# ligengen/EgoGen

Hardware: AMD Instinct MI355X
Metric: PPO env-steps/sec (512 parallel SMPL-X agents) (higher is better)
Workload: dtype f32 (blend GEMM: shape/template columns as 2-term bf16 splits, pose correctives as one fp16 product, fp32 accumulate); PPO update products on 2-term bf16 splits; rollout policy layers on 2-term bf16 splits

## Files before the change

egogen_amd/_lib.py:

```python
from __future__ import annotations

import ctypes as C
import os

_HERE = os.path.dirname(os.path.abspath(__file__))
LIB_PATH = os.path.join(_HERE, "libegogen_hip.so")

c_float_p = C.POINTER(C.c_float)
c_int_p = C.POINTER(C.c_int32)


class EgxError(RuntimeError):
    pass


class BodyModelHost(C.Structure):
    _fields_ = [
        ("num_verts", C.c_int),
        ("v_template_host", C.c_void_p), ("shapedirs_host", C.c_void_p), ("posedirs_host", C.c_void_p),
        ("J_regressor_host", C.c_void_p), ("parents_host", C.c_void_p), ("lbs_weights_host", C.c_void_p),
        ("hand_comps_l_host", C.c_void_p), ("hand_comps_r_host", C.c_void_p),
        ("hand_mean_l_host", C.c_void_p), ("hand_mean_r_host", C.c_void_p),
        ("extra_vids_host", C.c_void_p), ("lmk_vids_host", C.c_void_p), ("lmk_bary_host", C.c_void_p),
        ("num_markers", C.c_int), ("marker_vids_host", C.c_void_p),
        ("num_feet", C.c_int), ("feet_vids_host", C.c_void_p),
    ]


class SdfGrid(C.Structure):
    _fields_ = [("grid", C.c_void_p), ("d0", C.c_int), ("d1", C.c_int), ("d2", C.c_int),
                ("center", C.c_float * 3), ("scale", C.c_float), ("coarse_minmax", C.c_void_p)]


class LinearDesc(C.Structure):
    _fields_ = [("num_rows", C.c_int), ("out_features", C.c_int), ("num_segments", C.c_int),
                ("seg_ptr", C.c_void_p * 4), ("seg_width", C.c_int * 4), ("seg_ld", C.c_int * 4),
                ("weight", C.c_void_p), ("weight_ld", C.c_int), ("bias", C.c_void_p),
                ("residual", C.c_void_p), ("residual_ld", C.c_int),
                ("out", C.c_void_p), ("out_ld", C.c_int), ("activation", C.c_int), ("leaky_slope", C.c_float)]


class PriorPacked3(C.Structure):
    _fields_ = [("x_enc_w_ih", C.c_void_p), ("x_enc_w_hh", C.c_void_p), ("drnn_w", C.c_void_p * 3), ("d_rnn_w_hz", C.c_void_p),
                ("d_rnn_w_y", C.c_void_p), ("d_rnn_w_hh", C.c_void_p), ("d_comb_w", C.c_void_p), ("d_mlp_w", C.c_void_p * 2),
                ("d_out_w", C.c_void_p), ("reg_in_m", C.c_void_p), ("reg_in_xb", C.c_void_p), ("reg_in_betas", C.c_void_p),
                ("reg_blk", C.c_void_p), ("reg_out", C.c_void_p), ("reg_blk_b", C.c_void_p)]


class PriorWeights(C.Structure):
    _fields_ = [(n, C.c_void_p) for n in ("x_enc_w_ih", "x_enc_w_hh", "x_enc_b_ih", "x_enc_b_hh")] + \
               [("drnn_w", C.c_void_p * 3), ("drnn_b", C.c_void_p * 3)] + \
               [(n, C.c_void_p) for n in ("d_rnn_w_ih", "d_rnn_w_hh", "d_rnn_b_ih", "d_rnn_b_hh")] + \
               [("d_mlp_w", C.c_void_p * 2), ("d_mlp_b", C.c_void_p * 2), ("d_out_w", C.c_void_p), ("d_out_b", C.c_void_p),
                ("reg_in_w", C.c_void_p), ("reg_in_b", C.c_void_p), ("reg_blk_w", C.c_void_p * 20), ("reg_blk_b", C.c_void_p * 20),
                ("reg_out_w", C.c_void_p), ("reg_out_b", C.c_void_p), ("d_comb_w", C.c_void_p), ("d_comb_b", C.c_void_p),
                ("packed3", C.POINTER(PriorPacked3))]


class PolicyPacked3(C.Structure):
    _fields_ = [(n, C.c_void_p) for n in ("x_enc_w_ih", "x_enc_w_hh", "ego_enc_w_ih", "ego_enc_w_hh")] + \
               [("actor_w", C.c_void_p * 4), ("actor_out_w", C.c_void_p), ("critic_w", C.c_void_p * 4), ("critic_out_w", C.c_void_p)]


class PolicyWeights(C.Structure):
    _fields_ = [(n, C.c_void_p) for n in ("x_enc_w_ih", "x_enc_w_hh", "x_enc_b_ih", "x_enc_b_hh",
                                          "ego_enc_w_ih", "ego_enc_w_hh", "ego_enc_b_ih", "ego_enc_b_hh")] + \
               [("actor_w", C.c_void_p * 4), ("actor_b", C.c_void_p * 4), ("actor_out_w", C.c_void_p), ("actor_out_b", C.c_void_p),
                ("critic_w", C.c_void_p * 4), ("critic_b", C.c_void_p * 4), ("critic_out_w", C.c_void_p), ("critic_out_b", C.c_void_p),
                ("packed3", C.POINTER(PolicyPacked3))]


class PolicyGrads(C.Structure):
    _fields_ = [(n, C.c_void_p) for n in ("x_enc_w_ih", "x_enc_w_hh", "x_enc_b_ih", "x_enc_b_hh",
                                          "ego_enc_w_ih", "ego_enc_w_hh", "ego_enc_b_ih", "ego_enc_b_hh")] + \
               [("actor_w", C.c_void_p * 4), ("actor_b", C.c_void_p * 4), ("actor_out_w", C.c_void_p), ("actor_out_b", C.c_void_p),
                ("critic_w", C.c_void_p * 4), ("critic_b", C.c_void_p * 4), ("critic_out_w", C.c_void_p), ("critic_out_b", C.c_void_p)]


class VposerWeights(C.Structure):
    _fields_ = [(n, C.c_void_p) for n in ("fc1_w", "fc1_b", "fc2_w", "fc2_b", "mu_w", "mu_b", "fc1_w3", "fc2_w3", "mu_w3")]


class EnvConfig(C.Structure):
    _fields_ = [(n, C.c_float) for n in ("reproj_factor", "goal_thresh", "pene_thres", "weight_skate", "weight_floor",
                                         "weight_face_target", "weight_look_target", "weight_success", "weight_target_dist",
                                         "weight_pene", "weight_vp")] + \
               [(n, C.c_int) for n in ("max_depth", "scene_kind", "terminate_on_penetration", "pene_type_body")] + \
               [("ray_len", C.c_float), ("vp_thresh", C.c_float), ("no_goal_termination", C.c_int)]


class EnvScenes(C.Structure):
    _fields_ = [("edges", C.c_void_p), ("edge_off", C.c_void_p), ("tris", C.c_void_p), ("tri_off", C.c_void_p),
                ("floor_height", C.c_void_p), ("map_lin", C.c_void_p), ("map_res", C.c_int),
                ("crowd_bbox", C.c_void_p), ("crowd_group", C.c_int), ("crowd_scenes", C.c_int), ("crowd_member", C.c_int),
                ("crowd_floor_half", C.c_float), ("crowd_polygon", C.c_int), ("crowd_static", C.c_int)]


class EnvState(C.Structure):
    _fields_ = [(n, C.c_void_p) for n in ("state", "seed", "R0", "T0", "dist", "steps", "wpath", "scene_idx")]


class EnvStepIO(C.Structure):
    _fields_ = [(n, C.c_void_p) for n in ("Y_gen", "pred_params", "joints", "markers_proj", "pene_count", "vp_emb",
                                          "feet_marker_idx", "reward", "terminated", "reward_terms", "obs_ego", "obs_dist",
                                          "obs_time", "out_marker_b", "out_prev_frame", "nonfinite_count", "invalid_flags")]


class EnvResetIO(C.Structure):
    _fields_ = [("num_candidates", C.c_int)] + \
               [(n, C.c_void_p) for n in ("mask", "cand_pairs", "cand_yaw", "cand_variant", "cand_scene", "cand_valid", "tab_joints",
                                          "tab_markers", "tab_glorot", "tab_transl", "tab_pose", "obs_ego", "obs_dist",
                                          "obs_time", "out_choice", "out_pending", "forced_count")]


SIGNATURES = {
    "egx_last_error": (C.c_char_p, []),
    "egx_version": (C.c_int, []),
    "egx_body_model_create": (C.c_int, [C.POINTER(BodyModelHost), C.POINTER(C.c_void_p)]),
    "egx_body_model_destroy": (None, [C.c_void_p]),
    "egx_body_model_num_verts": (C.c_int, [C.c_void_p]),
    "egx_body_model_nnz": (C.c_int, [C.c_void_p]),
    "egx_body_model_lbs_vertices": (C.c_int, [C.c_void_p, C.c_int]),
    "egx_lbs_workspace_bytes": (C.c_size_t, [C.c_void_p, C.c_int]),
    "egx_body_model_culls": (C.c_int, [C.c_void_p, C.POINTER(C.c_float)]),
    "egx_lbs_set_culling": (C.c_int, [C.c_int]),
    "egx_lbs_get_culling": (C.c_int, []),
    "egx_lbs_cull_stats": (C.c_int, [C.c_void_p, C.c_void_p, C.c_int, C.POINTER(C.c_int32), C.POINTER(C.c_int32)]),
    "egx_lbs_forward": (C.c_int, [C.c_void_p, C.c_void_p, C.c_void_p, C.c_int, C.c_int, C.c_void_p, C.c_void_p,
                                  C.c_void_p, C.POINTER(SdfGrid), C.c_void_p, C.c_void_p, C.c_void_p,
                                  C.c_void_p, C.c_size_t, C.c_void_p]),
    "egx_sdf_scene_set_create": (C.c_int, [C.POINTER(SdfGrid), C.c_int, C.POINTER(C.c_void_p)]),
    "egx_sdf_scene_set_destroy": (None, [C.c_void_p]),
    "egx_sdf_scene_set_size": (C.c_int, [C.c_void_p]),
    "egx_lbs_forward_scenes": (C.c_int, [C.c_void_p, C.c_void_p, C.c_void_p, C.c_int, C.c_int, C.c_void_p, C.c_void_p,
                                         C.c_void_p, C.c_void_p, C.c_void_p, C.c_void_p, C.c_void_p, C.c_void_p,
                                         C.c_void_p, C.c_size_t, C.c_void_p]),
    "egx_point_set_create": (C.c_int, [C.POINTER(BodyModelHost), C.c_void_p, C.c_int, C.POINTER(C.c_void_p)]),
    "egx_point_set_destroy": (None, [C.c_void_p]),
    "egx_point_set_size": (C.c_int, [C.c_void_p]),
    "egx_points_forward": (C.c_int, [C.c_void_p, C.c_void_p, C.c_void_p, C.c_int, C.c_int, C.c_void_p, C.c_void_p, C.c_void_p]),
    "egx_points_backward": (C.c_int, [C.c_void_p, C.c_void_p, C.c_void_p, C.c_int, C.c_int, C.c_void_p, C.c_void_p, C.c_void_p,
                                      C.c_void_p, C.c_void_p]),
    "egx_lbs_joints": (C.c_int, [C.c_void_p, C.c_void_p, C.c_void_p, C.c_int, C.c_int, C.c_void_p, C.c_void_p, C.c_size_t, C.c_void_p]),
    "egx_canonical_frame": (C.c_int, [C.c_void_p, C.c_int, C.c_int, C.c_void_p, C.c_void_p, C.c_void_p]),
    "egx_update_transl_glorot": (C.c_int, [C.c_void_p, C.c_void_p, C.c_int, C.c_void_p, C.c_void_p, C.c_int, C.c_void_p, C.c_void_p]),
    "egx_sdf_sample": (C.c_int, [C.POINTER(SdfGrid), C.c_void_p, C.c_int64, C.c_void_p, C.c_void_p]),
    "egx_mesh_sdf": (C.c_int, [C.c_void_p, C.c_int, C.POINTER(C.c_float), C.c_float, C.c_int, C.c_int, C.c_int, C.c_int, C.c_void_p, C.c_void_p]),
    "egx_sdf_boxes": (C.c_int, [C.c_void_p, C.POINTER(C.c_float), C.POINTER(C.c_float), C.c_int, C.POINTER(C.c_float), C.c_float,
                                C.c_int, C.c_int, C.c_int, C.c_void_p, C.c_void_p]),
    "egx_scan_sdf": (C.c_int, [C.c_void_p, C.c_int, C.c_void_p, C.c_void_p, C.c_int, C.c_int, C.POINTER(C.c_float), C.c_float,
                               C.c_int, C.c_int, C.c_int, C.c_void_p, C.c_void_p]),
    "egx_walkable_raster": (C.c_int, [C.c_void_p, C.c_int, C.c_float, C.c_float, C.c_float, C.c_int, C.c_int] + [C.c_float] * 5 +
                            [C.c_void_p, C.c_void_p, C.c_void_p]),
    "egx_sdf_coarse_bytes": (C.c_size_t, [C.c_int, C.c_int, C.c_int]),
    "egx_sdf_build_coarse": (C.c_int, [C.POINTER(SdfGrid), C.c_void_p, C.c_void_p]),
    "egx_linear": (C.c_int, [C.POINTER(LinearDesc), C.c_void_p]),
    "egx_gru_pointwise": (C.c_int, [C.c_void_p, C.c_void_p, C.c_void_p, C.c_int, C.c_void_p, C.c_int, C.c_int, C.c_int, C.c_void_p]),
    "egx_cont6d_to_aa": (C.c_int, [C.c_void_p, C.c_int, C.c_void_p, C.c_int, C.c_void_p]),
    "egx_posenc": (C.c_int, [C.c_void_p, C.c_void_p, C.c_int, C.c_void_p, C.c_void_p]),
    "egx_sample_prior_workspace_bytes": (C.c_size_t, [C.c_int]),
    "egx_sample_prior": (C.c_int, [C.POINTER(PriorWeights), C.c_void_p, C.c_void_p, C.c_int, C.c_void_p, C.c_void_p, C.c_int,
                                   C.c_void_p, C.c_void_p, C.c_void_p, C.c_size_t, C.c_void_p]),
    "egx_policy_workspace_bytes": (C.c_size_t, [C.c_int]),
    "egx_policy_forward": (C.c_int, [C.POINTER(PolicyWeights), C.c_void_p, C.c_void_p, C.c_void_p, C.c_void_p, C.c_int,
                                     C.c_void_p, C.c_void_p, C.c_void_p, C.c_void_p, C.c_size_t, C.c_void_p]),
    "egx_assemble_params": (C.c_int, [C.c_void_p, C.c_void_p, C.c_int, C.c_void_p, C.c_void_p]),
    "egx_env_step_post": (C.c_int, [C.POINTER(EnvConfig), C.POINTER(EnvScenes), C.POINTER(EnvState), C.POINTER(EnvStepIO),
                                    C.c_int, C.c_void_p]),
    "egx_env_reset": (C.c_int, [C.POINTER(EnvConfig), C.POINTER(EnvScenes), C.POINTER(EnvState), C.POINTER(EnvResetIO),
                                C.c_int, C.c_void_p]),
    "egx_env_get_feature": (C.c_int, [C.c_void_p] * 5 + [C.c_int] * 4 + [C.c_void_p] * 3),
    "egx_env_get_map": (C.c_int, [C.c_void_p, C.c_int, C.c_float, C.c_void_p, C.c_int, C.c_void_p, C.c_void_p, C.c_int, C.c_void_p,
                                  C.c_void_p, C.c_void_p]),
    "egx_sample_action": (C.c_int, [C.c_void_p, C.c_void_p, C.c_void_p, C.c_float, C.c_float, C.c_int, C.c_int, C.c_void_p,
                                    C.c_void_p, C.c_void_p]),
    "egx_gae": (C.c_int, [C.c_void_p, C.c_void_p, C.c_void_p, C.c_int, C.c_int, C.c_double, C.c_double, C.c_void_p,
                          C.c_void_p, C.c_void_p]),
    "egx_ppo_loss": (C.c_int, [C.c_void_p] * 9 + [C.c_float] * 6 + [C.c_int] + [C.c_void_p] * 5),
    "egx_gru_pointwise_bwd": (C.c_int, [C.c_void_p, C.c_void_p, C.c_void_p, C.c_void_p, C.c_int, C.c_int, C.c_void_p, C.c_void_p,
                                        C.c_void_p, C.c_void_p]),
    "egx_ppo_loss_packed": (C.c_int, [C.c_void_p] * 8 + [C.c_float] * 6 + [C.c_int] + [C.c_void_p] * 4),
    "egx_lbs_set_blend_mode": (C.c_int, [C.c_int]),
    "egx_lbs_get_blend_mode": (C.c_int, []),
    "egx_lbs_set_wave_tile": (C.c_int, [C.c_int]),
    "egx_lbs_get_wave_tile": (C.c_int, []),
    "egx_lbs_set_fix_queue_capacity": (C.c_int, [C.c_int]),
    "egx_lbs_fix_stats": (C.c_int, [C.c_void_p, C.c_void_p, C.c_int, C.POINTER(C.c_int32)]),
    "egx_gather_rows": (C.c_int, [C.c_void_p, C.c_int, C.c_int, C.c_void_p, C.c_void_p, C.c_void_p, C.c_void_p]),
    "egx_adv_stats": (C.c_int, [C.c_void_p, C.c_int, C.c_void_p, C.c_void_p]),
    "egx_track_episode": (C.c_int, [C.c_void_p, C.c_void_p, C.c_int, C.c_void_p, C.c_void_p, C.c_void_p, C.c_void_p]),
    "egx_rollout_store": (C.c_int, [C.c_void_p] * 6 + [C.c_int] + [C.c_void_p] * 10),
    "egx_adamw_workspace_floats": (C.c_size_t, []),
    "egx_adamw_clip_step": (C.c_int, [C.c_void_p, C.c_void_p, C.c_void_p, C.c_void_p, C.c_size_t, C.c_size_t, C.c_float] + [C.c_double] * 5 +
                            [C.c_void_p, C.c_void_p, C.c_void_p]),
    "egx_policy_set_precision": (C.c_int, [C.c_int]),
    "egx_policy_get_precision": (C.c_int, []),
    "egx_act_fwd": (C.c_int, [C.c_void_p, C.c_void_p, C.c_void_p, C.c_int, C.c_int, C.c_int, C.c_float, C.c_void_p]),
    "egx_act_bwd_colsum": (C.c_int, [C.c_void_p, C.c_void_p, C.c_void_p, C.c_void_p, C.c_int, C.c_int, C.c_int, C.c_float,
                                     C.c_void_p]),
    "egx_profile_next_lbs": (C.c_int, [C.c_void_p, C.c_void_p]),
    "egx_event_create": (C.c_int, [C.POINTER(C.c_void_p)]),
    "egx_event_destroy": (C.c_int, [C.c_void_p]),
    "egx_event_elapsed_ms": (C.c_int, [C.c_void_p, C.c_void_p, C.POINTER(C.c_float)]),
    "egx_policy_train_create": (C.c_int, [C.POINTER(PolicyWeights), C.POINTER(PolicyGrads), C.c_int, C.POINTER(C.c_void_p)]),
    "egx_policy_train_destroy": (None, [C.c_void_p]),
    "egx_policy_train_refresh": (C.c_int, [C.c_void_p, C.c_void_p]),
    "egx_policy_train_packed": (C.c_int, [C.c_void_p, C.POINTER(PolicyPacked3)]),
    "egx_policy_train_bind": (C.c_int, [C.c_void_p, C.c_void_p, C.c_void_p]),
    "egx_policy_train_step": (C.c_int, [C.c_void_p] * 9 + [C.c_float] * 6 + [C.c_void_p, C.c_void_p]),
    "egx_policy_train_step_heads": (C.c_int, [C.c_void_p] * 9 + [C.c_float] * 6 + [C.c_void_p, C.c_void_p]),
    "egx_policy_train_step_encoders": (C.c_int, [C.c_void_p, C.c_void_p]),
    "egx_policy_train_set_precision": (C.c_int, [C.c_void_p, C.c_int]),
    "egx_pack3_bytes": (C.c_size_t, [C.c_int, C.c_int]),
    "egx_pack3": (C.c_int, [C.c_void_p, C.c_int, C.c_int, C.c_int, C.c_int, C.c_void_p, C.c_int, C.c_int, C.c_void_p]),
    "egx_gemm3_workspace_bytes": (C.c_size_t, [C.c_int, C.c_int, C.c_int]),
    "egx_gemm3": (C.c_int, [C.c_void_p, C.c_int, C.c_int, C.c_void_p, C.c_int, C.c_int, C.c_int, C.c_int, C.c_int, C.c_void_p, C.c_int,
                            C.c_float, C.c_void_p, C.c_int, C.c_void_p, C.c_int, C.c_void_p, C.c_int, C.c_void_p, C.c_size_t, C.c_void_p]),
    "egx_vposer_workspace_bytes": (C.c_size_t, [C.c_int]),
    "egx_vposer_encode": (C.c_int, [C.POINTER(VposerWeights), C.c_void_p, C.c_int, C.c_int, C.c_void_p, C.c_void_p,
                                    C.c_size_t, C.c_void_p]),
}

_lib = None


def load():
    global _lib
    if _lib is not None:
        return _lib
    if not os.path.exists(LIB_PATH):
        raise EgxError(f"{LIB_PATH} not found - build it with `python -c 'import __graft_entry__ as g; g.build()'` "
                       f"or `make -C egogen_amd/csrc`; there is no CPU fallback")
    lib = C.CDLL(LIB_PATH)
    for name, (res, args) in SIGNATURES.items():
        fn = getattr(lib, name)
        fn.restype = res
        fn.argtypes = args
    _lib = lib
    return lib


def check(rc: int, what: str):
    if rc != 0:
        msg = load().egx_last_error()
        raise EgxError(f"{what} failed (code {rc}): {msg.decode() if msg else ''}")


def ptr(t):
    if t is None:
        return None
    assert t.is_contiguous(), "tensor must be contiguous"
    return C.c_void_p(t.data_ptr())


def current_stream_ptr():
    import torch
    return C.c_void_p(torch.cuda.current_stream().cuda_stream)
```

egogen_amd/csrc/dense3.hip:

```cpp
#include <cstddef>
#include <cstdlib>
#include <mutex>
#include "egx_nets.h"

namespace {

typedef __bf16 bf16v8 __attribute__((ext_vector_type(8)));
typedef float f32x4a1 __attribute__((ext_vector_type(4), aligned(4)));

__host__ __device__ constexpr int d3_planes(int prec) { return prec == 0 ? 3 : (prec == 2 ? 2 : 1); }

template <int NP = 3>
__device__ __forceinline__ void d3_split(const float (&x)[8], bf16x8 (&pl)[NP]) {
  float r[8];
#pragma unroll
  for (int p = 0; p < NP; ++p) {
    bf16v8 h;
#pragma unroll
    for (int e = 0; e < 8; ++e) {
      const float v = (p == 0) ? x[e] : r[e];
      h[e] = (__bf16)v;
      r[e] = v - (float)h[e];
    }
    pl[p] = __builtin_bit_cast(bf16x8, h);
// ... 314 lines not shown
struct D3Gru2 {
  D3Gru g0, g1;
  int blocks0;
  int rowmap;
};
static_assert(offsetof(D3Gru2, g0) == 0 && offsetof(D3Gru2, g1) == sizeof(D3Gru), "layout");
template <int TRIP, int NPL>
__global__ __launch_bounds__(512) void egx_gru3_kernel(D3Gru2 two) {
  const bool second = (int)blockIdx.x >= two.blocks0;
  const D3Gru a = d3_kernarg<D3Gru>(second ? 1 : 0);
  const int gru_bid = second ? (int)blockIdx.x - two.blocks0 : (int)blockIdx.x;
  extern __shared__ __attribute__((aligned(16))) float gsm[];
  float* red = gsm;
  float* tile = gsm + 8 * 24 * 64;
  const int lane = threadIdx.x & 63, wave = threadIdx.x >> 6;
  const int MT = (a.M + 31) >> 5, CT = a.H >> 4;
  int mt, ct;
  if (!d3_tile(gru_bid, MT, CT, mt, ct, d3_rowmap(two.rowmap, a.M, 3 * a.H))) return;
  const int sd = wave >> 2, w4 = wave & 3;
  constexpr bool EARLY = NPL == 3;
  const int e_mi = wave >> 2, e_r = wave & 3;
  const int e_col = lane & 15, e_c = ct * 16 + e_col;
  const int e_row = 16 * e_mi + 4 * (lane >> 4) + e_r, e_m = mt * 32 + e_row;
  float pre_gi[3] = {0.f, 0.f, 0.f}, pre_bi[3] = {0.f, 0.f, 0.f}, pre_bh[3] = {0.f, 0.f, 0.f}, pre_hp = 0.f;
  auto prefetch = [&]() __attribute__((always_inline)) {
    if (e_m >= a.M) return;
#pragma unroll
    for (int g = 0; g < 3; ++g) {
      const int n = g * a.H + e_c;
      if (a.gi_in) pre_gi[g] = d3_g(a.gi_in)[(size_t)e_m * 3 * a.H + n];
      if (a.bias_i) pre_bi[g] = d3_g(a.bias_i)[n];
      pre_bh[g] = d3_g(a.bias_h)[n];
    }
    if (a.h_prev) pre_hp = d3_g(a.h_prev)[(size_t)e_m * a.ldh + e_c];
  };
  if (EARLY) prefetch();
  f32x4 acc[2][3];
#pragma unroll
  for (int mi = 0; mi < 2; ++mi)
#pragma unroll
    for (int g = 0; g < 3; ++g) acc[mi][g] = f32x4{0.f, 0.f, 0.f, 0.f};
  {
    const D3_GLOBAL bf16x8* A = d3_g(sd ? a.Ah : a.Ai);
    const D3_GLOBAL bf16x8* B = d3_g(sd ? a.Bh : a.Bi);
    const int S = A ? (sd ? a.Sh : a.Si) : 0, SA = sd ? a.SAh : a.SAi, sa0 = sd ? a.sah0 : a.sai0;
    const int per = (S + 3) >> 2;
    const int s_lo = w4 * per, s_hi = min(S, s_lo + per);
    const D3_GLOBAL bf16x8* pa[2];
    const D3_GLOBAL bf16x8* pb[3];
#pragma unroll
    for (int mi = 0; mi < 2; ++mi) pa[mi] = A + ((size_t)(2 * mt + mi) * SA + sa0) * 3 * 64 + lane;
#pragma unroll
    for (int g = 0; g < 3; ++g) pb[g] = B + (size_t)(g * CT + ct) * S * 3 * 64 + lane;
    for (int s = s_lo; s < s_hi; s += TRIP) {
      bf16x8 fa[TRIP][2][NPL], fb[TRIP][3][NPL];
#pragma unroll
      for (int u = 0; u < TRIP; ++u) {
        const int su = min(s + u, s_hi - 1);
#pragma unroll
        for (int p = 0; p < NPL; ++p) {
#pragma unroll
          for (int mi = 0; mi < 2; ++mi) fa[u][mi][p] = pa[mi][(size_t)(su * 3 + p) * 64];
#pragma unroll
          for (int g = 0; g < 3; ++g) fb[u][g][p] = pb[g][(size_t)(su * 3 + p) * 64];
        }
      }
      __builtin_amdgcn_sched_barrier(0);
      asm volatile("s_waitcnt vmcnt(0)" ::: "memory");
      __builtin_amdgcn_sched_barrier(0);
#pragma unroll
      for (int u = 0; u < TRIP; ++u) {
        if (s + u >= s_hi) break;
        d3_mma_tiles<2, 3, NPL>(fa[u], fb[u], acc);
      }
      __builtin_amdgcn_sched_barrier(0);
    }
  }
#pragma unroll
  for (int g = 0; g < 3; ++g)
#pragma unroll
    for (int mi = 0; mi < 2; ++mi)
#pragma unroll
      for (int r = 0; r < 4; ++r) red[(wave * 24 + (g * 2 + mi) * 4 + r) * 64 + lane] = acc[mi][g][r];
  if (!EARLY) prefetch();
  __syncthreads();
  {
    const int mi = e_mi, r = e_r, col = e_col, c = e_c, row = e_row, m = e_m;
    float gv[2][3];
#pragma unroll
    for (int s2 = 0; s2 < 2; ++s2)
#pragma unroll
      for (int g = 0; g < 3; ++g) {
        const int q = (g * 2 + mi) * 4 + r;
        gv[s2][g] = ((red[((s2 * 4 + 0) * 24 + q) * 64 + lane] + red[((s2 * 4 + 1) * 24 + q) * 64 + lane]) +
                     red[((s2 * 4 + 2) * 24 + q) * 64 + lane]) + red[((s2 * 4 + 3) * 24 + q) * 64 + lane];
      }
    float hv = 0.f;
    if (m < a.M) {
      float gi[3], gh[3];
#pragma unroll
      for (int g = 0; g < 3; ++g) {
        gi[g] = pre_gi[g] + gv[0][g] + pre_bi[g];
        gh[g] = gv[1][g] + pre_bh[g];
      }
      const float rg = 1.f / (1.f + expf(-(gi[0] + gh[0])));
      const float zg = 1.f / (1.f + expf(-(gi[1] + gh[1])));
      const float ng = tanhf(gi[2] + rg * gh[2]);
      const float hp = pre_hp;
      {
#pragma clang fp contract(off)
        const float keep = (1.f - zg) * ng, carry = zg * hp;
        hv = keep + carry;
      }
#pragma unroll
      for (int g = 0; g < 3; ++g) {
        const int n = g * a.H + c;
        if (a.gi_out) d3_g(a.gi_out)[(size_t)m * 3 * a.H + n] = gi[g];
        if (a.gh_out) d3_g(a.gh_out)[(size_t)m * 3 * a.H + n] = gh[g];
      }
      if (a.h_out) d3_g(a.h_out)[(size_t)m * a.ldo + c] = hv;
    }
    tile[row * 20 + col] = hv;
  }
  if (a.h_out3 || a.h_out3T) __syncthreads();
  if (a.h_out3T && wave == 2) {
    const int c = lane & 15, kg = lane >> 4;
    float x[8];
#pragma unroll
    for (int e = 0; e < 8; ++e) x[e] = tile[(8 * kg + e) * 20 + c];
    bf16x8 pl[NPL];
    d3_split<NPL>(x, pl);
    D3_GLOBAL bf16x8* o = d3_g(a.h_out3T) + ((size_t)((a.col0T >> 4) + ct) * a.S3T + a.s3T0 + mt) * 3 * 64 + lane;
#pragma unroll
    for (int p = 0; p < NPL; ++p) o[p * 64] = pl[p];
  }
  if (a.h_out3) {
    if (wave < 2 && lane < 32) {
      const int row = 16 * wave + (lane & 15), g = lane >> 4;
      const f32x4 x0 = *reinterpret_cast<const f32x4*>(&tile[row * 20 + 8 * g]), x1 = *reinterpret_cast<const f32x4*>(&tile[row * 20 + 8 * g + 4]);
      const float x[8] = {x0[0], x0[1], x0[2], x0[3], x1[0], x1[1], x1[2], x1[3]};
      bf16x8 pl[NPL];
      d3_split<NPL>(x, pl);
      D3_GLOBAL bf16x8* o = d3_g(a.h_out3) + ((size_t)(2 * mt + wave) * a.S3 + a.s30 + (ct >> 1)) * 3 * 64 + 32 * (ct & 1) + lane;
#pragma unroll
      for (int p = 0; p < NPL; ++p) o[p * 64] = pl[p];
    }
  }
}

__global__ __launch_bounds__(256) void egx_posenc3_kernel(const float* __restrict__ dist, const float* __restrict__ time, int n,
                                                          float* __restrict__ out, int ld, bf16x8* __restrict__ out3, int S3, int s0,
                                                          bf16x8* __restrict__ out3T, int S3T, int col0T, float* __restrict__ zero6) {
  if (zero6 && blockIdx.x == 0 && threadIdx.x < 6) zero6[threadIdx.x] = 0.f;
  int frag = blockIdx.x * 4 + (threadIdx.x >> 6);
  const int lane = threadIdx.x & 63;
  const int RT = 2 * ((n + 31) >> 5);
  if (frag >= RT * 4) {
    frag -= RT * 4;
    const int Sn = (n + 31) >> 5;
    if (!out3T || frag >= 8 * Sn) return;
    const int t = frag / Sn, s = frag % Sn;
    const int c = 16 * t + (lane & 15), m0 = 32 * s + 8 * (lane >> 4);
    float x[8];
#pragma unroll
    for (int e = 0; e < 8; ++e) {
      const int m = m0 + e;
      float v = 0.f;
      if (m < n) {
        const float f = ((c < 64) ? dist[m] : time[m]) * exp2f((float)((c & 63) >> 1));
        v = (c & 1) ? cosf(f) : sinf(f);
      }
      x[e] = v;
    }
    bf16x8 pl[3];
    d3_split(x, pl);
    bf16x8* o = out3T + ((size_t)((col0T >> 4) + t) * S3T + s) * 3 * 64 + lane;
#pragma unroll
    for (int p = 0; p < 3; ++p) o[p * 64] = pl[p];
    return;
  }
  const int rt = frag >> 2, s = frag & 3;
  const int row = rt * 16 + (lane & 15), c0 = s * 32 + 8 * (lane >> 4);
  float x[8];
#pragma unroll
  for (int e = 0; e < 8; ++e) {
    const int c = c0 + e;
    float v = 0.f;
    if (row < n) {
      const float f = ((c < 64) ? dist[row] : time[row]) * exp2f((float)((c & 63) >> 1));
      v = (c & 1) ? cosf(f) : sinf(f);
      out[(size_t)row * ld + c] = v;
    }
    x[e] = v;
  }
  bf16x8 pl[3];
  d3_split(x, pl);
  bf16x8* o = out3 + ((size_t)rt * S3 + s0 + s) * 3 * 64 + lane;
#pragma unroll
  for (int p = 0; p < 3; ++p) o[p * 64] = pl[p];
}
void egx_launch_posenc3(hipStream_t st, const float* dist, const float* time, int n, float* out, int ld, void* out3, int S3, int s0,
                        void* out3T, int S3T, int col0T, float* zero6) {
  const int frags = 2 * egx_ceil_div(n, 32) * 4 + (out3T ? 8 * egx_ceil_div(n, 32) : 0);
  hipLaunchKernelGGL(egx_posenc3_kernel, dim3(egx_ceil_div(frags, 4)), dim3(256), 0, st, dist, time, n, out, ld,
                     static_cast<bf16x8*>(out3), S3, s0, static_cast<bf16x8*>(out3T), S3T, col0T, zero6);
}

namespace {
constexpr int R3_XBP = 164, R3_NOUT = 159;
constexpr int r3_act_frags(int nrt) { return nrt * 4 * 3 * 64; }
constexpr size_t r3_lds(int nrt) { return (size_t)16 * nrt * R3_XBP * 4 + 2 * (size_t)r3_act_frags(nrt) * 16; }

__device__ __forceinline__ void r3_load_w(const bf16x8* P, int tile, int S, int lane, bf16x8 (&wf)[4][3]) {
  const bf16x8* p = P + (size_t)tile * S * 3 * 64 + lane;
#pragma unroll
  for (int s = 0; s < 4; ++s)
#pragma unroll
    for (int pl = 0; pl < 3; ++pl) wf[s][pl] = p[(s * 3 + pl) * 64];
}
template <int NRT>
__device__ __forceinline__ void r3_mma3(const bf16x8 (&a)[NRT][3], const bf16x8 (&wf)[3], f32x4 (&acc)[NRT]) {
#pragma unroll
  for (int pr = 0; pr < 6; ++pr) {
    const int pa = (pr == 0) ? 1 : (pr == 1) ? 0 : (pr == 2) ? 2 : (pr == 3) ? 0 : (pr == 4) ? 1 : 0;
    const int pb = (pr == 0) ? 1 : (pr == 1) ? 2 : (pr == 2) ? 0 : (pr == 3) ? 1 : (pr == 4) ? 0 : 0;
#pragma unroll
    for (int rt = 0; rt < NRT; ++rt) acc[rt] = __builtin_amdgcn_mfma_f32_16x16x32_bf16(wf[pb], a[rt][pa], acc[rt], 0, 0, 0);
  }
}
template <int NRT>
__device__ __forceinline__ void r3_mma128(const bf16x8* act, int lane, const bf16x8 (&wf)[4][3], f32x4 (&acc)[NRT]) {
#pragma unroll
  for (int s = 0; s < 4; ++s) {
    bf16x8 a[NRT][3];
#pragma unroll
    for (int rt = 0; rt < NRT; ++rt)
#pragma unroll
      for (int pl = 0; pl < 3; ++pl) a[rt][pl] = act[((rt * 4 + s) * 3 + pl) * 64 + lane];
    r3_mma3<NRT>(a, wf[s], acc);
  }
}
template <int NRT>
__device__ __forceinline__ void r3_store_packed(const float (&v)[NRT][4], bf16x8* dst, int wave, int lane) {
  typedef __bf16 bf16v4 __attribute__((ext_vector_type(4)));
  const int g = lane >> 4;
  char* o = reinterpret_cast<char*>(dst + (size_t)((wave >> 1) * 3) * 64 + 16 * (2 * (wave & 1) + (g >> 1)) + (lane & 15)) + 8 * (g & 1);
#pragma unroll
  for (int rt = 0; rt < NRT; ++rt) {
    float r[4];
#pragma unroll
    for (int p = 0; p < 3; ++p) {
      bf16v4 h;
#pragma unroll
      for (int e = 0; e < 4; ++e) {
        const float x = (p == 0) ? v[rt][e] : r[e];
        h[e] = (__bf16)x;
        r[e] = x - (float)h[e];
      }
      *reinterpret_cast<bf16v4*>(o + (size_t)((rt * 4) * 3 + p) * 64 * sizeof(bf16x8)) = h;
    }
  }
}
}

template <int NRT>
__global__ __launch_bounds__(512) void egx_regressor3_kernel(RegWeights3 w, const float* __restrict__ Y,
                                                                const float* __restrict__ betas, int A, int M,
                                                                float* __restrict__ out_Yb) {
  constexpr int ROWS = 16 * NRT;
  extern __shared__ __attribute__((aligned(16))) char r3_smem[];
  float* xb = reinterpret_cast<float*>(r3_smem);
  bf16x8* hb3 = reinterpret_cast<bf16x8*>(r3_smem + (size_t)ROWS * R3_XBP * 4);
  bf16x8* tb3 = hb3 + r3_act_frags(NRT);
  const int tid = threadIdx.x, lane = tid & 63, wave = tid >> 6;
  const int m0 = blockIdx.x * ROWS;
  const int col4 = 16 * wave + 4 * (lane >> 4);
  for (int i = tid; i < ROWS * R3_XBP; i += 512) xb[i] = 0.f;
  bf16x8* in3 = hb3;
  for (int f = wave; f < NRT * 8; f += 8) {
    const int rt = f >> 3, s = f & 7;
    const int row = min(m0 + 16 * rt + (lane & 15), M - 1), k0 = 8 * (lane >> 4);
    float x[8];
#pragma unroll
    for (int e = 0; e < 8; ++e) {
      const int k = 32 * s + k0 + e;
      x[e] = (s < 7) ? (k < 201 ? Y[(size_t)row * 201 + k] : 0.f) : (k0 + e < 10 ? betas[(size_t)(row % A) * 10 + k0 + e] : 0.f);
    }
    bf16x8 pl[3];
    d3_split(x, pl);
#pragma unroll
    for (int p = 0; p < 3; ++p) in3[((rt * 8 + s) * 3 + p) * 64 + lane] = pl[p];
  }
  __syncthreads();
  f32x4 base[NRT];
  {
    const f32x4 b = *reinterpret_cast<const f32x4a1*>(w.in_b + col4);
#pragma unroll
    for (int rt = 0; rt < NRT; ++rt) base[rt] = b;
    for (int s = 0; s < 8; ++s) {
      bf16x8 wf[3];
      const bf16x8* pw = (s < 7) ? w.in_m + ((size_t)(wave * 7 + s) * 3) * 64 + lane : w.in_b3 + ((size_t)wave * 3) * 64 + lane;
#pragma unroll
      for (int pl = 0; pl < 3; ++pl) wf[pl] = pw[pl * 64];
      bf16x8 a[NRT][3];
#pragma unroll
      for (int rt = 0; rt < NRT; ++rt)
#pragma unroll
        for (int pl = 0; pl < 3; ++pl) a[rt][pl] = in3[((rt * 8 + s) * 3 + pl) * 64 + lane];
      r3_mma3<NRT>(a, wf, base);
    }
  }
  __syncthreads();
  bf16x8 wA[4][3], wB[4][3];
  float hres[NRT][4];
  f32x4 acc[NRT];
  auto layer = [&](int l, const bf16x8 (&cur)[4][3], bf16x8 (&nxt)[4][3]) __attribute__((always_inline)) {
    const bf16x8* src = (l & 1) ? tb3 : hb3;
    const f32x4 b = *reinterpret_cast<const f32x4a1*>(w.blk_b + l * 128 + col4);
    if (l + 1 < 20) r3_load_w(w.blk + (size_t)(l + 1) * 8 * 4 * 3 * 64, wave, 4, lane, nxt);
    else r3_load_w(w.out, wave, 4, lane, nxt);
#pragma unroll
    for (int rt = 0; rt < NRT; ++rt) acc[rt] = f32x4{0.f, 0.f, 0.f, 0.f};
    __builtin_amdgcn_sched_barrier(0);
    r3_mma128<NRT>(src, lane, cur, acc);
    __builtin_amdgcn_sched_barrier(0);
    float v[NRT][4];
#pragma unroll
    for (int rt = 0; rt < NRT; ++rt)
#pragma unroll
      for (int r = 0; r < 4; ++r) {
        float y = fmaxf(acc[rt][r] + b[r], 0.f);
        if (l & 1) { y += hres[rt][r]; hres[rt][r] = y; }
        v[rt][r] = y;
      }
    r3_store_packed<NRT>(v, (l & 1) ? hb3 : tb3, wave, lane);
    __syncthreads();
  };
  r3_load_w(w.blk, wave, 4, lane, wA);
  for (int rc = 0; rc < 3; ++rc) {
#pragma unroll
    for (int rt = 0; rt < NRT; ++rt) acc[rt] = base[rt];
    if (rc > 0) {
      bf16x8* xb3 = hb3;
      for (int f = wave; f < NRT * 5; f += 8) {
        const int rt = f / 5, s = f % 5;
        const float* sp = xb + (16 * rt + (lane & 15)) * R3_XBP + 32 * s + 8 * (lane >> 4);
        const f32x4 x0 = *reinterpret_cast<const f32x4*>(sp), x1 = *reinterpret_cast<const f32x4*>(sp + 4);
        const float x[8] = {x0[0], x0[1], x0[2], x0[3], x1[0], x1[1], x1[2], x1[3]};
        bf16x8 pl[3];
        d3_split(x, pl);
#pragma unroll
        for (int p = 0; p < 3; ++p) xb3[((rt * 5 + s) * 3 + p) * 64 + lane] = pl[p];
// ... 446 lines not shown
```

egogen_amd/csrc/egx_nets.h:

```cpp
#pragma once
#include "egx_common.h"

struct EgxSeg {
  const float* p;
  int w, ld;
};

int egx_launch_linear(hipStream_t st, int M, int N, const EgxSeg* segs, int nseg, const float* W, const float* b,
                      int act, float slope, const float* res, int ldr, float* out, int ldo);
int egx_launch_gru_pointwise(hipStream_t st, const float* gi, const float* gh, const float* hprev, int ldh, float* hout,
                             int ldo, int M, int H);
int egx_launch_cont6d_to_aa(hipStream_t st, const float* xb6, int n, float* out, int ldo);
int egx_launch_posenc(hipStream_t st, const float* dist, const float* time, int A, float* out);

void egx_launch_frame_scan(hipStream_t st, float* y, const float* x_last, int x_ld, int A, int width, int T);

struct D3Pack {
  const float* src;
  int R, K, ld, col0;
  void* dst;
  int S_total, s0;
  int transpose = 0;
};
void egx_launch_pack3(hipStream_t st, const D3Pack* jobs, int njobs);

struct D3Plain {
  const bf16x8* A = nullptr;
  int SA = 0, sa0 = 0;
  const bf16x8* B = nullptr;
  int S = 0;
  const float* bias = nullptr;
  const float* res = nullptr;
  int ldr = 0;
  float* out = nullptr;
  int ldo = 0;
  bf16x8* out3 = nullptr;
  int S3 = 0, s30 = 0;
  int M = 0, N = 0, act = 0;
  float slope = 0.f;
  int batches = 1;
  size_t batch_strideA = 0, batch_stride3 = 0;
  int batch_rows_out = 0;
  int prec = 0;
  float* out_act = nullptr;
  int ldact = 0;
  const float* dact = nullptr;
  int lddact = 0, dact_code = 0;
  float dact_slope = 0.f;
  bf16x8* out3T = nullptr;
  int S3T = 0, s3T0 = 0;
  float* bias_out = nullptr;
  int n_split = 0;
};
void egx_launch_dense3_n(hipStream_t st, const D3Plain* ps, int n);
void egx_launch_dense3(hipStream_t st, const D3Plain& p);
void egx_launch_dense3_pair(hipStream_t st, const D3Plain& p, const D3Plain& q);
void egx_launch_dense3_triple(hipStream_t st, const D3Plain& p, const D3Plain& q, const D3Plain& r);
int egx_ppo_loss_packed_precleared(const float* zp, const float* value, const float* act, const float* adv, const float* ret,
                                   const float* logp_old, const float* adv_stats, const float* scale, float adv_eps, float min_logvar,
                                   float max_logvar, float eps_clip, float vf_coef, float ent_coef, int num_rows, float* g_zp,
                                   float* g_value, float* out_terms, void* stream_);
void egx_launch_posenc3(hipStream_t st, const float* dist, const float* time, int n, float* out, int ld, void* out3, int S3, int s0,
                        void* out3T = nullptr, int S3T = 0, int col0T = 0, float* zero6 = nullptr );

struct D3Gru {
  const bf16x8* Ai = nullptr;
  int SAi = 0, sai0 = 0;
  const bf16x8* Bi = nullptr;
  int Si = 0;
  const float* bias_i = nullptr;
  const float* gi_in = nullptr;
  float* gi_out = nullptr;
  const bf16x8* Ah = nullptr;
  int SAh = 0, sah0 = 0;
  const bf16x8* Bh = nullptr;
  int Sh = 0;
  const float* bias_h = nullptr;
  const float* h_prev = nullptr;
  int ldh = 0;
  float* h_out = nullptr;
  int ldo = 0;
  bf16x8* h_out3 = nullptr;
  int S3 = 0, s30 = 0;
  int M = 0, H = 0;
  int prec = 0;
  float* gh_out = nullptr;
  bf16x8* h_out3T = nullptr;
  int S3T = 0, s3T0 = 0, col0T = 0;
};
int egx_launch_gru3(hipStream_t st, const D3Gru& g);
int egx_launch_gru3_pair(hipStream_t st, const D3Gru& g0, const D3Gru& g1);

struct RegWeights3 {
  const bf16x8 *in_m, *in_xb, *in_b3;
  const float* in_b;
  const bf16x8* blk;
  const float* blk_b;
  const bf16x8* out;
  const float* out_b;
};
int egx_launch_regressor3(hipStream_t st, const RegWeights3& w, const float* Y, const float* betas, int A, int M, float* out_Yb);

struct VpWeights3 {
  const bf16x8 *fc1, *fc2, *mu;
  const float *b1, *b2, *bmu;
};
int egx_launch_vposer3(hipStream_t st, const VpWeights3& w, const float* x, int x_ld, int n, float* out);

__device__ __forceinline__ void egx_cont6d_item(const float* src, float* dst, int j) {
  if (j == 22) {
    dst[0] = src[0]; dst[1] = src[1]; dst[2] = src[2];
    for (int e = 0; e < 24; ++e) dst[69 + e] = src[135 + e];
    return;
  }
  const float* a = src + 3 + 6 * j;
  float b1[3] = {a[0], a[2], a[4]}, a2[3] = {a[1], a[3], a[5]};
  const float n1 = fmaxf(sqrtf(b1[0] * b1[0] + b1[1] * b1[1] + b1[2] * b1[2]), 1e-12f);
  b1[0] /= n1; b1[1] /= n1; b1[2] /= n1;
  const float d = b1[0] * a2[0] + b1[1] * a2[1] + b1[2] * a2[2];
  float b2[3] = {a2[0] - d * b1[0], a2[1] - d * b1[1], a2[2] - d * b1[2]};
  const float n2 = fmaxf(sqrtf(b2[0] * b2[0] + b2[1] * b2[1] + b2[2] * b2[2]), 1e-12f);
  b2[0] /= n2; b2[1] /= n2; b2[2] /= n2;
  const float b3[3] = {b1[1] * b2[2] - b1[2] * b2[1], b1[2] * b2[0] - b1[0] * b2[2], b1[0] * b2[1] - b1[1] * b2[0]};
  const float R[9] = {b1[0], b2[0], b3[0], b1[1], b2[1], b3[1], b1[2], b2[2], b3[2]};
  float aa[3];
  egx_tgm_rotmat_to_aa(R, aa);
  dst[3 + 3 * j + 0] = aa[0]; dst[3 + 3 * j + 1] = aa[1]; dst[3 + 3 * j + 2] = aa[2];
}
```

egogen_amd/csrc/ppo.hip:

```cpp
#include <algorithm>
#include <cstring>
#include "egx_common.h"

namespace {
constexpr float LOG_SQRT_2PI = 0.91893853320467274178f;

}

__device__ __forceinline__ float egx_wave_sum(float v) {
#pragma unroll
  for (int o = 32; o > 0; o >>= 1) v += __shfl_xor(v, o);
  return v;
}

__global__ __launch_bounds__(256) void egx_ppo_loss_kernel(const float* __restrict__ mu, const float* __restrict__ logvar,
                                                          const float* __restrict__ value, const float* __restrict__ act,
                                                          const float* __restrict__ adv, const float* __restrict__ ret,
                                                          const float* __restrict__ logp_old, const float* __restrict__ adv_stats,
                                                          const float* __restrict__ scale_ptr, float adv_eps, float min_lv,
                                                          float max_lv, float eps_clip, float vf_coef, float ent_coef, int n,
                                                          int stride ,
                                                          float* __restrict__ g_mu, float* __restrict__ g_logvar,
                                                          float* __restrict__ g_value, float* __restrict__ out_terms) {
  __shared__ float sh[4][6];
  const int lane = threadIdx.x & 63, wave = threadIdx.x >> 6;
  const float scale = scale_ptr[0];
  float acc[6] = {0.f, 0.f, 0.f, 0.f, 0.f, 0.f};
  for (int row = blockIdx.x * 4 + wave; row < n; row += gridDim.x * 4) {
    float lv[2], inv_var[2], diff[2], lp_d = 0.f, ent_d = 0.f, musq_d = 0.f;
    bool pass[2];
#pragma unroll
    for (int h = 0; h < 2; ++h) {
      const int d = lane + 64 * h;
      const size_t i = (size_t)row * stride + d;
      const float lv_raw = logvar[i], m = mu[i];
      lv[h] = fminf(fmaxf(lv_raw, min_lv), max_lv);
      pass[h] = (lv_raw >= min_lv) && (lv_raw <= max_lv);
      inv_var[h] = expf(-lv[h]);
      diff[h] = act[(size_t)row * 128 + d] - m;
      lp_d += -0.5f * diff[h] * diff[h] * inv_var[h] - 0.5f * lv[h] - LOG_SQRT_2PI;
      ent_d += 0.5f + LOG_SQRT_2PI + 0.5f * lv[h];
      musq_d += m * m;
    }
    const float lp = egx_wave_sum(lp_d), ent = egx_wave_sum(ent_d), musq = egx_wave_sum(musq_d);
    float A = adv[row];
    if (adv_stats) A = (A - adv_stats[0]) / (adv_stats[1] + adv_eps);
    const float ratio = expf(lp - logp_old[row]);
    const float s1 = ratio * A;
    const float rc = fminf(fmaxf(ratio, 1.f - eps_clip), 1.f + eps_clip);
    const float s2 = rc * A;
    const bool in_range = (ratio >= 1.f - eps_clip) && (ratio <= 1.f + eps_clip);
    float dclip_dlp;
    if (s1 < s2) dclip_dlp = -A * ratio;
    else if (s1 > s2) dclip_dlp = in_range ? -A * ratio : 0.f;
    else dclip_dlp = in_range ? -A * ratio : -0.5f * A * ratio;
    const float v = value[row];
    const float dv = ret[row] - v;
#pragma unroll
    for (int h = 0; h < 2; ++h) {
      const size_t i = (size_t)row * stride + lane + 64 * h;
      g_mu[i] = scale * dclip_dlp * (diff[h] * inv_var[h]);
      const float dlp_dlv = 0.5f * (diff[h] * diff[h] * inv_var[h] - 1.f);
      g_logvar[i] = pass[h] ? scale * (dclip_dlp * dlp_dlv - ent_coef * 0.5f) : 0.f;
    }
    if (lane == 0) g_value[row] = scale * vf_coef * (-2.f) * dv;
    const float clip_l = -fminf(s1, s2), vf_l = dv * dv;
    acc[0] += scale * (clip_l + vf_coef * vf_l - ent_coef * ent);
    acc[1] += scale * clip_l;
    acc[2] += scale * vf_l;
    acc[3] += scale * ent;
    acc[4] += scale * 0.5f * musq / 128.f;
    acc[5] += scale * (logp_old[row] - lp);
  }
  if (lane == 0) {
#pragma unroll
    for (int k = 0; k < 6; ++k) sh[wave][k] = acc[k];
  }
  __syncthreads();
  if (threadIdx.x < 6) atomicAdd(out_terms + threadIdx.x, (sh[0][threadIdx.x] + sh[1][threadIdx.x]) + (sh[2][threadIdx.x] + sh[3][threadIdx.x]));
}

__global__ void egx_gru_pointwise_bwd_kernel(const float* __restrict__ gi, const float* __restrict__ gh,
                                             const float* __restrict__ hprev, const float* __restrict__ dh, int M, int H,
                                             float* __restrict__ dgi, float* __restrict__ dgh, float* __restrict__ dhprev) {
  const int idx = blockIdx.x * blockDim.x + threadIdx.x;
  if (idx >= M * H) return;
  const int m = idx / H, c = idx % H;
  const size_t b3 = (size_t)m * 3 * H;
  const float r = 1.f / (1.f + expf(-(gi[b3 + c] + gh[b3 + c])));
  const float z = 1.f / (1.f + expf(-(gi[b3 + H + c] + gh[b3 + H + c])));
  const float ghn = gh[b3 + 2 * H + c];
  const float nn = tanhf(gi[b3 + 2 * H + c] + r * ghn);
  const float hp = hprev ? hprev[idx] : 0.f;
  const float g = dh[idx];
  const float dn = g * (1.f - z), dz = g * (hp - nn);
  const float dan = dn * (1.f - nn * nn);
  const float dar = dan * ghn * r * (1.f - r);
  const float daz = dz * z * (1.f - z);
  dgi[b3 + c] = dar; dgh[b3 + c] = dar;
  dgi[b3 + H + c] = daz; dgh[b3 + H + c] = daz;
  dgi[b3 + 2 * H + c] = dan; dgh[b3 + 2 * H + c] = dan * r;
  if (dhprev) dhprev[idx] = g * z;
}

__global__ void egx_act_fwd_kernel(float* __restrict__ z, const float* __restrict__ res, float* __restrict__ out, size_t n4,
                                   int act, float slope) {
  const size_t i = (size_t)blockIdx.x * blockDim.x + threadIdx.x;
  if (i >= n4) return;
  float4 v = reinterpret_cast<float4*>(z)[i];
  float* e = reinterpret_cast<float*>(&v);
#pragma unroll
  for (int k = 0; k < 4; ++k) {
    const float x = e[k];
    e[k] = (act == 1) ? tanhf(x) : (act == 2) ? fmaxf(x, 0.f) : (act == 3) ? (x > 0.f ? x : x * slope) : x;
  }
  reinterpret_cast<float4*>(z)[i] = v;
  if (res) {
    const float4 r = reinterpret_cast<const float4*>(res)[i];
    reinterpret_cast<float4*>(out)[i] = make_float4(v.x + r.x, v.y + r.y, v.z + r.z, v.w + r.w);
  }
}

__global__ __launch_bounds__(256) void egx_act_bwd_colsum_kernel(const float* __restrict__ dy, const float* __restrict__ a,
                                                                 float* __restrict__ g, float* __restrict__ db, int M, int N,
                                                                 int rows_per_block, int act, float slope) {
  __shared__ float part[4][64];
  const int tx = threadIdx.x & 63, ty = threadIdx.x >> 6;
  const int n = blockIdx.x * 64 + tx;
  const int m0 = blockIdx.y * rows_per_block, m1 = min(M, m0 + rows_per_block);
  float s = 0.f;
  if (n < N) {
    for (int m = m0 + ty; m < m1; m += 4) {
      const size_t idx = (size_t)m * N + n;
      float v = dy[idx];
      if (act != 0) {
        const float y = a[idx];
        v *= (act == 1) ? (1.f - y * y) : (act == 2) ? (y > 0.f ? 1.f : 0.f) : (y > 0.f ? 1.f : slope);
      }
      if (g) g[idx] = v;
      s += v;
    }
  }
  part[ty][tx] = s;
  __syncthreads();
  if (ty == 0 && n < N && db) atomicAdd(db + n, part[0][tx] + part[1][tx] + part[2][tx] + part[3][tx]);
}

struct GatherArgs {
  const float *s0, *s1, *s2, *s3, *s4, *s5, *s6, *s7;
  float *d0, *d1, *d2, *d3, *d4, *d5, *d6, *d7;
  int w0, w1, w2, w3, w4, w5, w6, w7;
  const long long* idx;
  int n;
};
__device__ __forceinline__ void gather_seg(const float* __restrict__ s, float* __restrict__ d, int w, long long src_row, int dst_row) {
  if (!s || w <= 0) return;
  const float* sr = s + (size_t)src_row * w;
  float* dr = d + (size_t)dst_row * w;
  for (int c = threadIdx.x; c < w; c += blockDim.x) dr[c] = sr[c];
}
__global__ __launch_bounds__(256) void egx_gather_rows_kernel(GatherArgs a) {
  const int r = blockIdx.x;
  const long long src = a.idx[r];
  gather_seg(a.s0, a.d0, a.w0, src, r); gather_seg(a.s1, a.d1, a.w1, src, r);
  gather_seg(a.s2, a.d2, a.w2, src, r); gather_seg(a.s3, a.d3, a.w3, src, r);
  gather_seg(a.s4, a.d4, a.w4, src, r); gather_seg(a.s5, a.d5, a.w5, src, r);
  gather_seg(a.s6, a.d6, a.w6, src, r); gather_seg(a.s7, a.d7, a.w7, src, r);
}

__global__ __launch_bounds__(256) void egx_adv_stats_kernel(const float* __restrict__ adv, int n, float* __restrict__ out) {
  __shared__ double red[256];
  __shared__ double s_mean;
  double a = 0.0;
  for (int i = threadIdx.x; i < n; i += 256) a += adv[i];
  red[threadIdx.x] = a;
  __syncthreads();
  for (int st = 128; st > 0; st >>= 1) {
    if (threadIdx.x < st) red[threadIdx.x] += red[threadIdx.x + st];
    __syncthreads();
  }
  if (threadIdx.x == 0) s_mean = red[0] / n;
  __syncthreads();
  const double mean = s_mean;
  double b = 0.0;
  for (int i = threadIdx.x; i < n; i += 256) { const double d = adv[i] - mean; b += d * d; }
  red[threadIdx.x] = b;
  __syncthreads();
  for (int st = 128; st > 0; st >>= 1) {
    if (threadIdx.x < st) red[threadIdx.x] += red[threadIdx.x + st];
    __syncthreads();
  }
  if (threadIdx.x == 0) {
    out[0] = (float)mean;
    out[1] = (n > 1) ? (float)sqrt(red[0] / (n - 1)) : nanf("");
  }
}

__global__ __launch_bounds__(256) void egx_track_episode_kernel(const float* __restrict__ rew, const int* __restrict__ term, int A,
                                                                float* __restrict__ ep_ret, float* __restrict__ ep_len,
                                                                float* __restrict__ done_sums ) {
  __shared__ float s[3][256];
  float a = 0.f, b = 0.f, c = 0.f;
  for (int i = threadIdx.x; i < A; i += 256) {
    const float r = ep_ret[i] + rew[i], l = ep_len[i] + 1.f;
    const bool d = term[i] != 0;
    if (d) { a += r; b += l; c += 1.f; }
    ep_ret[i] = d ? 0.f : r;
    ep_len[i] = d ? 0.f : l;
  }
  s[0][threadIdx.x] = a; s[1][threadIdx.x] = b; s[2][threadIdx.x] = c;
  __syncthreads();
  for (int st = 128; st > 0; st >>= 1) {
    if (threadIdx.x < st)
      for (int k = 0; k < 3; ++k) s[k][threadIdx.x] += s[k][threadIdx.x + st];
    __syncthreads();
  }
  if (threadIdx.x < 3) done_sums[threadIdx.x] += s[threadIdx.x][0];
}

__global__ __launch_bounds__(256) void egx_rollout_store_kernel(const float* __restrict__ state, const float* __restrict__ ego,
                                                                const float* __restrict__ dist, const float* __restrict__ time,
                                                                const float* __restrict__ rew, const int* __restrict__ term, int A,
                                                                float* __restrict__ state_dst, float* __restrict__ ego_dst,
                                                                float* __restrict__ dist_dst, float* __restrict__ time_dst,
                                                                float* __restrict__ rew_dst, int* __restrict__ term_dst,
                                                                float* __restrict__ ep_ret, float* __restrict__ ep_len,
                                                                float* __restrict__ done_sums) {
  const int a = blockIdx.x;
  if (a < A) {
    const f32x4* s4 = reinterpret_cast<const f32x4*>(state + (size_t)a * 804);
    f32x4* d4 = reinterpret_cast<f32x4*>(state_dst + (size_t)a * 804);
    if (threadIdx.x < 201) d4[threadIdx.x] = s4[threadIdx.x];
    else if (threadIdx.x < 217) {
      const int e = threadIdx.x - 201;
      reinterpret_cast<f32x4*>(ego_dst + (size_t)a * 64)[e] = reinterpret_cast<const f32x4*>(ego + (size_t)a * 64)[e];
    } else if (threadIdx.x == 217) {
      dist_dst[a] = dist[a];
      time_dst[a] = time[a];
      if (rew_dst) { rew_dst[a] = rew[a]; term_dst[a] = term[a]; }
    }
    return;
  }
  if (!ep_ret) return;
  __shared__ float s[3][256];
  float x = 0.f, y = 0.f, c = 0.f;
  for (int i = threadIdx.x; i < A; i += 256) {
    const float r = ep_ret[i] + rew[i], l = ep_len[i] + 1.f;
    const bool d = term[i] != 0;
    if (d) { x += r; y += l; c += 1.f; }
    ep_ret[i] = d ? 0.f : r;
    ep_len[i] = d ? 0.f : l;
  }
  s[0][threadIdx.x] = x; s[1][threadIdx.x] = y; s[2][threadIdx.x] = c;
  __syncthreads();
  for (int st = 128; st > 0; st >>= 1) {
    if (threadIdx.x < st)
      for (int k = 0; k < 3; ++k) s[k][threadIdx.x] += s[k][threadIdx.x + st];
    __syncthreads();
  }
  if (threadIdx.x < 3) done_sums[threadIdx.x] += s[threadIdx.x][0];
}

__global__ __launch_bounds__(256) void egx_sumsq_partial_kernel(const float* __restrict__ g, size_t n, float* __restrict__ partials,
                                                                float* __restrict__ step) {
  __shared__ double red[256];
  double a = 0.0;
  const size_t stride = (size_t)gridDim.x * 256 * 4;
  for (size_t i = ((size_t)blockIdx.x * 256 + threadIdx.x) * 4; i + 3 < n; i += stride) {
    const float4 v = *reinterpret_cast<const float4*>(g + i);
    a += (double)v.x * v.x + (double)v.y * v.y + (double)v.z * v.z + (double)v.w * v.w;
  }
  if (blockIdx.x == 0 && threadIdx.x == 0) {
    for (size_t i = n & ~(size_t)3; i < n; ++i) a += (double)g[i] * g[i];
    *step += 1.f;
  }
  red[threadIdx.x] = a;
  __syncthreads();
  for (int st = 128; st > 0; st >>= 1) {
    if (threadIdx.x < st) red[threadIdx.x] += red[threadIdx.x + st];
    __syncthreads();
  }
  if (threadIdx.x == 0) partials[blockIdx.x] = (float)red[0];
}

__global__ __launch_bounds__(256) void egx_adamw_consts_kernel(const float* __restrict__ partials, int n_partials, int do_clip,
                                                               float max_norm, double lr, double b1, double b2,
                                                               const float* __restrict__ step, float* __restrict__ consts) {
  __shared__ double red[256];
  double a = 0.0;
  for (int i = threadIdx.x; i < n_partials; i += 256) a += partials[i];
  red[threadIdx.x] = a;
  __syncthreads();
  for (int st = 128; st > 0; st >>= 1) {
    if (threadIdx.x < st) red[threadIdx.x] += red[threadIdx.x + st];
    __syncthreads();
  }
  if (threadIdx.x == 0) {
    const double t = (double)*step;
    const float bc1 = (float)(1.0 - pow(b1, t)), bc2 = (float)(1.0 - pow(b2, t));
    float coef = 1.f;
    if (do_clip) coef = fminf(max_norm / ((float)sqrt(red[0]) + 1e-6f), 1.f);
    consts[0] = coef;
    consts[1] = (float)(lr / bc1);
    consts[2] = sqrtf(bc2);
  }
}

__global__ __launch_bounds__(256) void egx_adamw_flat_kernel(float* __restrict__ p, const float* __restrict__ g, float* __restrict__ m,
                                                             float* __restrict__ v, size_t n, size_t n_clip,
                                                             const float* __restrict__ consts ,
                                                             double lr, double b1, double b2, double eps, double wd) {
  const float coef = consts[0], step_size = consts[1], bc2s = consts[2];
  const size_t i0 = ((size_t)blockIdx.x * 256 + threadIdx.x) * 4;
  if (i0 >= n) return;
  const int cnt = (int)((n - i0 < 4) ? (n - i0) : 4);
  float gr[4], pv[4], mv[4], vv[4];
  if (cnt == 4) {
    *reinterpret_cast<float4*>(gr) = *reinterpret_cast<const float4*>(g + i0);
    *reinterpret_cast<float4*>(pv) = *reinterpret_cast<const float4*>(p + i0);
    *reinterpret_cast<float4*>(mv) = *reinterpret_cast<const float4*>(m + i0);
    *reinterpret_cast<float4*>(vv) = *reinterpret_cast<const float4*>(v + i0);
  } else {
    for (int e = 0; e < cnt; ++e) { gr[e] = g[i0 + e]; pv[e] = p[i0 + e]; mv[e] = m[i0 + e]; vv[e] = v[i0 + e]; }
  }
  const double omb1 = 1.0 - b1, omb2 = 1.0 - b2, lrwd = lr * wd;
#pragma unroll
  for (int e = 0; e < 4; ++e) {
    if (e < cnt) {
      float gg = gr[e];
      if (i0 + e < n_clip) gg *= coef;
      pv[e] = (float)((double)pv[e] - lrwd * (double)pv[e]);
      mv[e] = (float)((double)mv[e] + omb1 * ((double)gg - (double)mv[e]));
      vv[e] = (float)(b2 * (double)vv[e] + omb2 * (double)gg * (double)gg);
      const float denom = (float)((double)(sqrtf(vv[e]) / bc2s) + eps);
      pv[e] -= step_size * mv[e] / denom;
    }
  }
  if (cnt == 4) {
    *reinterpret_cast<float4*>(p + i0) = *reinterpret_cast<const float4*>(pv);
    *reinterpret_cast<float4*>(m + i0) = *reinterpret_cast<const float4*>(mv);
    *reinterpret_cast<float4*>(v + i0) = *reinterpret_cast<const float4*>(vv);
  } else {
    for (int e = 0; e < cnt; ++e) { p[i0 + e] = pv[e]; m[i0 + e] = mv[e]; v[i0 + e] = vv[e]; }
  }
}

__global__ void egx_zero_terms_kernel(float* __restrict__ t) {
  if (threadIdx.x < 6) t[threadIdx.x] = 0.f;
}

static int ppo_loss_blocks(int num_rows) { return std::max(1, std::min(256, egx_ceil_div(num_rows, 8))); }

extern "C" int egx_ppo_loss(const float* mu, const float* logvar, const float* value, const float* act, const float* adv,
                            const float* ret, const float* logp_old, const float* adv_stats, const float* scale,
                            float adv_eps, float min_logvar, float max_logvar, float eps_clip, float vf_coef, float ent_coef,
                            int num_rows, float* g_mu, float* g_logvar, float* g_value, float* out_terms, void* stream_) {
  EGX_REQUIRE(mu && logvar && value && act && adv && ret && logp_old && scale && g_mu && g_logvar && g_value && out_terms &&
                  num_rows > 0, "bad arguments");
  hipStream_t st = static_cast<hipStream_t>(stream_);
  hipLaunchKernelGGL(egx_zero_terms_kernel, dim3(1), dim3(64), 0, st, out_terms);
  hipLaunchKernelGGL(egx_ppo_loss_kernel, dim3(ppo_loss_blocks(num_rows)), dim3(256), 0, st, mu, logvar, value, act, adv, ret, logp_old,
                     adv_stats, scale, adv_eps, min_logvar, max_logvar, eps_clip, vf_coef, ent_coef, num_rows, 128, g_mu, g_logvar,
                     g_value, out_terms);
  EGX_HIP_CHECK(hipGetLastError());
  return EGX_OK;
}

int egx_ppo_loss_packed_precleared(const float* zp, const float* value, const float* act, const float* adv, const float* ret,
                                   const float* logp_old, const float* adv_stats, const float* scale, float adv_eps, float min_logvar,
                                   float max_logvar, float eps_clip, float vf_coef, float ent_coef, int num_rows, float* g_zp,
                                   float* g_value, float* out_terms, void* stream_) {
  EGX_REQUIRE(zp && value && act && adv && ret && logp_old && scale && g_zp && g_value && out_terms && num_rows > 0, "bad arguments");
  hipStream_t st = static_cast<hipStream_t>(stream_);
  hipLaunchKernelGGL(egx_ppo_loss_kernel, dim3(ppo_loss_blocks(num_rows)), dim3(256), 0, st, zp, zp + 128, value, act, adv, ret, logp_old, adv_stats,
                     scale, adv_eps, min_logvar, max_logvar, eps_clip, vf_coef, ent_coef, num_rows, 256, g_zp, g_zp + 128, g_value,
                     out_terms);
  EGX_HIP_CHECK(hipGetLastError());
  return EGX_OK;
}

extern "C" int egx_ppo_loss_packed(const float* zp, const float* value, const float* act, const float* adv, const float* ret,
                                   const float* logp_old, const float* adv_stats, const float* scale, float adv_eps, float min_logvar,
                                   float max_logvar, float eps_clip, float vf_coef, float ent_coef, int num_rows, float* g_zp,
                                   float* g_value, float* out_terms, void* stream_) {
  EGX_REQUIRE(zp && value && act && adv && ret && logp_old && scale && g_zp && g_value && out_terms && num_rows > 0, "bad arguments");
  hipStream_t st = static_cast<hipStream_t>(stream_);
  hipLaunchKernelGGL(egx_zero_terms_kernel, dim3(1), dim3(64), 0, st, out_terms);
  hipLaunchKernelGGL(egx_ppo_loss_kernel, dim3(ppo_loss_blocks(num_rows)), dim3(256), 0, st, zp, zp + 128, value, act, adv, ret, logp_old, adv_stats,
                     scale, adv_eps, min_logvar, max_logvar, eps_clip, vf_coef, ent_coef, num_rows, 256, g_zp, g_zp + 128, g_value,
                     out_terms);
  EGX_HIP_CHECK(hipGetLastError());
  return EGX_OK;
}

extern "C" int egx_gru_pointwise_bwd(const float* gi, const float* gh, const float* h_prev, const float* dh, int num_rows,
                                     int hidden, float* dgi, float* dgh, float* dh_prev, void* stream_) {
  EGX_REQUIRE(gi && gh && dh && dgi && dgh && num_rows > 0 && hidden > 0, "bad arguments");
  const int n = num_rows * hidden;
  hipLaunchKernelGGL(egx_gru_pointwise_bwd_kernel, dim3(egx_ceil_div(n, 256)), dim3(256), 0, static_cast<hipStream_t>(stream_),
                     gi, gh, h_prev, dh, num_rows, hidden, dgi, dgh, dh_prev);
  EGX_HIP_CHECK(hipGetLastError());
  return EGX_OK;
}

extern "C" int egx_act_fwd(float* z, const float* res, float* out, int num_rows, int width, int act, float slope, void* stream_) {
  EGX_REQUIRE(z && num_rows > 0 && width > 0 && (!res || out), "bad arguments");
  EGX_REQUIRE(((size_t)num_rows * width) % 4 == 0, "rows x width must be a multiple of 4");
  EGX_REQUIRE(act >= 0 && act <= 3, "unknown activation");
  const size_t n4 = (size_t)num_rows * width / 4;
  hipLaunchKernelGGL(egx_act_fwd_kernel, dim3((unsigned)((n4 + 255) / 256)), dim3(256), 0, static_cast<hipStream_t>(stream_), z,
                     res, out, n4, act, slope);
  EGX_HIP_CHECK(hipGetLastError());
  return EGX_OK;
}

extern "C" int egx_act_bwd_colsum(const float* dy, const float* a, float* g, float* db_accum, int num_rows, int width, int act,
                                  float slope, void* stream_) {
  EGX_REQUIRE(dy && num_rows > 0 && width > 0 && (act == 0 || a) && (g || db_accum), "bad arguments");
  EGX_REQUIRE(act >= 0 && act <= 3, "unknown activation");
  const int strips = egx_ceil_div(width, 64);
  int splits = std::max(1, std::min(egx_ceil_div(num_rows, 32), 512 / strips));
  const int rpb = egx_ceil_div(num_rows, splits);
  splits = egx_ceil_div(num_rows, rpb);
  hipLaunchKernelGGL(egx_act_bwd_colsum_kernel, dim3(strips, splits), dim3(256), 0, static_cast<hipStream_t>(stream_), dy, a, g,
                     db_accum, num_rows, width, rpb, act, slope);
  EGX_HIP_CHECK(hipGetLastError());
  return EGX_OK;
}

extern "C" int egx_gather_rows(const int64_t* idx, int num_rows, int num_tensors, const float* const* src, const int* width,
                               float* const* dst, void* stream_) {
  EGX_REQUIRE(idx && src && width && dst && num_rows > 0 && num_tensors > 0 && num_tensors <= 8, "bad arguments");
  GatherArgs a;
  std::memset(&a, 0, sizeof(a));
  const float** sp[8] = {&a.s0, &a.s1, &a.s2, &a.s3, &a.s4, &a.s5, &a.s6, &a.s7};
  float** dp[8] = {&a.d0, &a.d1, &a.d2, &a.d3, &a.d4, &a.d5, &a.d6, &a.d7};
  int* wp[8] = {&a.w0, &a.w1, &a.w2, &a.w3, &a.w4, &a.w5, &a.w6, &a.w7};
  for (int t = 0; t < num_tensors; ++t) {
    EGX_REQUIRE(src[t] && dst[t] && width[t] > 0, "null tensor or non-positive width");
    *sp[t] = src[t]; *dp[t] = dst[t]; *wp[t] = width[t];
  }
  a.idx = reinterpret_cast<const long long*>(idx);
  a.n = num_rows;
  hipLaunchKernelGGL(egx_gather_rows_kernel, dim3(num_rows), dim3(256), 0, static_cast<hipStream_t>(stream_), a);
  EGX_HIP_CHECK(hipGetLastError());
  return EGX_OK;
}

extern "C" int egx_adv_stats(const float* adv, int n, float* out_mean_std, void* stream_) {
  EGX_REQUIRE(adv && out_mean_std && n > 0, "bad arguments");
  hipLaunchKernelGGL(egx_adv_stats_kernel, dim3(1), dim3(256), 0, static_cast<hipStream_t>(stream_), adv, n, out_mean_std);
  EGX_HIP_CHECK(hipGetLastError());
  return EGX_OK;
}

extern "C" int egx_track_episode(const float* rew, const int32_t* term, int num_agents, float* ep_ret, float* ep_len,
                                 float* done_sums, void* stream_) {
  EGX_REQUIRE(rew && term && ep_ret && ep_len && done_sums && num_agents > 0, "bad arguments");
  hipLaunchKernelGGL(egx_track_episode_kernel, dim3(1), dim3(256), 0, static_cast<hipStream_t>(stream_), rew, term, num_agents,
                     ep_ret, ep_len, done_sums);
  EGX_HIP_CHECK(hipGetLastError());
  return EGX_OK;
}

extern "C" int egx_rollout_store(const float* state, const float* egosensing, const float* dist, const float* time, const float* rew,
                                 const int32_t* term, int num_agents, float* state_dst, float* ego_dst, float* dist_dst, float* time_dst,
                                 float* rew_dst, int32_t* term_dst, float* ep_ret, float* ep_len, float* done_sums, void* stream_) {
  EGX_REQUIRE(state && egosensing && dist && time && state_dst && ego_dst && dist_dst && time_dst && num_agents > 0, "bad arguments");
  EGX_REQUIRE((!rew_dst && !term_dst && !ep_ret) || (rew && term && rew_dst && term_dst), "reward / termination source or slot missing");
  EGX_REQUIRE(!ep_ret || (ep_len && done_sums && rew && term), "episode bookkeeping needs ep_len, done_sums, rew, term");
  hipLaunchKernelGGL(egx_rollout_store_kernel, dim3(num_agents + (ep_ret ? 1 : 0)), dim3(256), 0, static_cast<hipStream_t>(stream_), state,
                     egosensing, dist, time, rew, term, num_agents, state_dst, ego_dst, dist_dst, time_dst, rew_dst, term_dst, ep_ret, ep_len,
                     done_sums);
  EGX_HIP_CHECK(hipGetLastError());
  return EGX_OK;
}

extern "C" size_t egx_adamw_workspace_floats(void) { return 1024 + 8; }

extern "C" int egx_adamw_clip_step(float* param, const float* grad, float* exp_avg, float* exp_avg_sq, size_t n, size_t n_clip,
                                   float max_norm, double lr, double beta1, double beta2, double eps, double weight_decay,
                                   float* step, float* workspace, void* stream_) {
  EGX_REQUIRE(param && grad && exp_avg && exp_avg_sq && step && workspace && n > 0 && n_clip <= n, "bad arguments");
  hipStream_t st = static_cast<hipStream_t>(stream_);
  const int nb = 1024;
  const bool do_clip = max_norm > 0.f && n_clip > 0;
  hipLaunchKernelGGL(egx_sumsq_partial_kernel, dim3(nb), dim3(256), 0, st, grad, do_clip ? n_clip : (size_t)0, workspace, step);
  hipLaunchKernelGGL(egx_adamw_consts_kernel, dim3(1), dim3(256), 0, st, workspace, nb, do_clip ? 1 : 0, max_norm, lr, beta1, beta2,
                     step, workspace + nb);
  const size_t blocks = (n + 1023) / 1024;
  hipLaunchKernelGGL(egx_adamw_flat_kernel, dim3((unsigned)blocks), dim3(256), 0, st, param, grad, exp_avg, exp_avg_sq, n, n_clip,
                     workspace + nb, lr, beta1, beta2, eps, weight_decay);
  EGX_HIP_CHECK(hipGetLastError());
  return EGX_OK;
}
```

egogen_amd/csrc/update3.hip:

```cpp
#include <algorithm>
#include <cstring>
#include <vector>
#include "egx_nets.h"

namespace {

typedef __bf16 bf16v8 __attribute__((ext_vector_type(8)));
__device__ __forceinline__ void u3_split(const float (&x)[8], bf16x8 (&pl)[3]) {
  float r[8];
#pragma unroll
  for (int p = 0; p < 3; ++p) {
    bf16v8 h;
#pragma unroll
    for (int e = 0; e < 8; ++e) {
      const float v = (p == 0) ? x[e] : r[e];
      h[e] = (__bf16)v;
      r[e] = v - (float)h[e];
    }
    pl[p] = __builtin_bit_cast(bf16x8, h);
  }
}

struct PackEntry {
  const float* src;
  int red, cols, ld, col0;
  bf16x8* dst;
  int S_total, s0;
  int transpose;
  int ones_row;
  int frag_end;
  bf16x8* dst2;
  int S_total2;
};

__global__ __launch_bounds__(256) void egx_pack3_table_kernel(const PackEntry* __restrict__ tab, int n, int nplanes) {
  int frag = blockIdx.x * 4 + (threadIdx.x >> 6);
  const int lane = threadIdx.x & 63;
  if (n <= 0 || frag >= tab[n - 1].frag_end) return;
  int lo = 0, hi = n - 1;
  while (lo < hi) {
    const int mid = (lo + hi) >> 1;
    if (frag >= tab[mid].frag_end) lo = mid + 1; else hi = mid;
  }
  const PackEntry e = tab[lo];
  frag -= lo > 0 ? tab[lo - 1].frag_end : 0;
  float x[8];
  int rt, s;
  if (e.transpose == 2) {
    __shared__ float sblk[4][32][33];
    float (*sb)[33] = sblk[threadIdx.x >> 6];
    const int BJ = (e.cols + 31) >> 5;
    const int bi = frag / BJ, bj = frag % BJ;
    const int r = lane & 15, kg = lane >> 4;
#pragma unroll
    for (int t = 0; t < 2; ++t) {
      const int row = 32 * bi + 16 * t + r, k0 = 32 * bj + 8 * kg;
      const float* sp = e.src + (size_t)row * e.ld + e.col0 + k0;
      if (row < e.red && k0 + 7 < e.cols && (reinterpret_cast<uintptr_t>(sp) & 15) == 0) {
        const f32x4 x0 = *reinterpret_cast<const f32x4*>(sp), x1 = *reinterpret_cast<const f32x4*>(sp + 4);
        x[0] = x0[0]; x[1] = x0[1]; x[2] = x0[2]; x[3] = x0[3]; x[4] = x1[0]; x[5] = x1[1]; x[6] = x1[2]; x[7] = x1[3];
      } else {
#pragma unroll
        for (int q = 0; q < 8; ++q) x[q] = (row < e.red && k0 + q < e.cols) ? sp[q] : 0.f;
      }
#pragma unroll
      for (int q = 0; q < 8; ++q) sb[16 * t + r][8 * kg + q] = x[q];
      bf16x8 pl[3];
      u3_split(x, pl);
      bf16x8* o = e.dst + ((size_t)(2 * bi + t) * e.S_total + e.s0 + bj) * 3 * 64 + lane;
#pragma unroll
      for (int p = 0; p < 3; ++p)
        if (p < nplanes) o[p * 64] = pl[p];
    }
    __builtin_amdgcn_wave_barrier();
#pragma unroll
    for (int t = 0; t < 2; ++t) {
#pragma unroll
      for (int q = 0; q < 8; ++q) x[q] = sb[8 * kg + q][16 * t + r];
      bf16x8 pl[3];
      u3_split(x, pl);
      bf16x8* o = e.dst2 + ((size_t)(2 * bj + t) * e.S_total2 + bi) * 3 * 64 + lane;
#pragma unroll
      for (int p = 0; p < 3; ++p)
        if (p < nplanes) o[p * 64] = pl[p];
    }
    return;
  }
  if (!e.transpose) {
    const int S = (e.cols + 31) >> 5;
    rt = frag / S; s = frag % S;
    const int row = rt * 16 + (lane & 15), k0 = s * 32 + 8 * (lane >> 4);
#pragma unroll
    for (int q = 0; q < 8; ++q) x[q] = (row < e.red && k0 + q < e.cols) ? e.src[(size_t)row * e.ld + e.col0 + k0 + q] : 0.f;
  } else {
    const int S = (e.red + 31) >> 5;
    rt = frag / S; s = frag % S;
    const int irow = rt * 16 + (lane & 15), k0 = s * 32 + 8 * (lane >> 4);
#pragma unroll
    for (int q = 0; q < 8; ++q) {
      float v = 0.f;
      if (k0 + q < e.red) {
        if (irow < e.cols) v = e.src[(size_t)(k0 + q) * e.ld + e.col0 + irow];
        else if (irow == e.ones_row) v = 1.f;
      }
      x[q] = v;
    }
  }
  bf16x8 pl[3];
  u3_split(x, pl);
  bf16x8* o = e.dst + ((size_t)rt * e.S_total + e.s0 + s) * 3 * 64 + lane;
#pragma unroll
  for (int p = 0; p < 3; ++p)
    if (p < nplanes) o[p * 64] = pl[p];
}

inline int img_tiles(int rows) { return 2 * egx_ceil_div(rows, 32); }
inline size_t img_frags(int rows, int red) { return (size_t)img_tiles(rows) * egx_ceil_div(red, 32); }
constexpr size_t FRAG_BYTES = 3 * 64 * 16;

struct GruBwd {
  const float* gi;
  const float* gh;
  const float* bias_h;
  const float* h_prev;
  const float* dh0;
  const float* dh1;
  int ld0, ld1;
  bf16x8* dgiT;
  bf16x8* dghT;
  int ST, s0T;
  bf16x8* dgh_r;
  float* dhp;
  int M, H;
};
struct GruBwd2 {
  GruBwd a, b;
  int blocks0;
};

__global__ __launch_bounds__(256) void egx_gru_bwd3_kernel(GruBwd2 two) {
  const bool second = (int)blockIdx.x >= two.blocks0;
  const GruBwd& a = second ? two.b : two.a;
  const int bid = second ? (int)blockIdx.x - two.blocks0 : (int)blockIdx.x;
  __shared__ __attribute__((aligned(16))) float tile[6][32 * 36];
  const int CT = a.H >> 5;
  const int mt = bid / CT, ct = bid % CT;
  const int lane = threadIdx.x & 63, wave = threadIdx.x >> 6;
  const int H = a.H;
  const int cl = threadIdx.x & 31, c = ct * 32 + cl;
#pragma unroll
  for (int j = 0; j < 4; ++j) {
    const int rl = (threadIdx.x >> 5) + 8 * j, m = mt * 32 + rl;
    float o[6] = {0.f, 0.f, 0.f, 0.f, 0.f, 0.f};
    if (m < a.M) {
      const float* gim = a.gi + (size_t)m * 3 * H;
      const float* ghm = a.gh ? a.gh + (size_t)m * 3 * H : a.bias_h;
      const float ghn = ghm[2 * H + c];
      const float r = 1.f / (1.f + expf(-(gim[c] + ghm[c])));
      const float z = 1.f / (1.f + expf(-(gim[H + c] + ghm[H + c])));
      const float nn = tanhf(gim[2 * H + c] + r * ghn);
      const float hp = a.h_prev ? a.h_prev[(size_t)m * H + c] : 0.f;
      float dh = a.dh0[(size_t)m * a.ld0 + c];
      if (a.dh1) dh += a.dh1[(size_t)m * a.ld1 + c];
      const float dnn = dh * (1.f - z), dz = dh * (hp - nn);
      const float dpn = dnn * (1.f - nn * nn);
      const float dpr = dpn * ghn * r * (1.f - r), dpz = dz * z * (1.f - z);
      o[0] = dpr; o[1] = dpz; o[2] = dpn; o[3] = dpr; o[4] = dpz; o[5] = dpn * r;
      if (a.dhp) a.dhp[(size_t)m * H + c] = dh * z;
    }
#pragma unroll
    for (int q = 0; q < 6; ++q) tile[q][rl * 36 + cl] = o[q];
  }
  __syncthreads();
  const int ntask = 12 + (a.dgh_r ? 6 : 0);
  for (int task = wave; task < ntask; task += 4) {
    float x[8];
    bf16x8* o;
    if (task < 12) {
      const int q = task >> 1, half = task & 1;
      const int cc = 16 * half + (lane & 15), kg = lane >> 4;
#pragma unroll
      for (int e = 0; e < 8; ++e) x[e] = tile[q][(8 * kg + e) * 36 + cc];
      bf16x8* img = q < 3 ? a.dgiT : a.dghT;
      const int row_tile = ((q % 3) * H + ct * 32) / 16 + half;
      o = img + ((size_t)row_tile * a.ST + a.s0T + mt) * 3 * 64 + lane;
    } else {
      const int g = (task - 12) >> 1, half = (task - 12) & 1;
      const int row = 16 * half + (lane & 15), kg = lane >> 4;
      const f32x4 x0 = *reinterpret_cast<const f32x4*>(&tile[3 + g][row * 36 + 8 * kg]), x1 = *reinterpret_cast<const f32x4*>(&tile[3 + g][row * 36 + 8 * kg + 4]);
      x[0] = x0[0]; x[1] = x0[1]; x[2] = x0[2]; x[3] = x0[3]; x[4] = x1[0]; x[5] = x1[1]; x[6] = x1[2]; x[7] = x1[3];
      const int S = (3 * H) >> 5;
      o = a.dgh_r + ((size_t)(2 * mt + half) * S + (g * H) / 32 + ct) * 3 * 64 + lane;
    }
    bf16x8 pl[3];
    u3_split(x, pl);
#pragma unroll
    for (int p = 0; p < 3; ++p) o[p * 64] = pl[p];
  }
}

struct Arena {
  char* base = nullptr;
  size_t off = 0, cap = 0;
  void* take(size_t bytes) {
    void* p = base ? base + off : nullptr;
    off = egx_align_up(off + bytes, 256);
    return p;
  }
};

constexpr int HD = 512, CAT = 1152, ZP = 256, ST_DIM = 402, EGO_DIM = 32;

struct Branch {
  const float* W[4]; const float* b[4]; const float* Wout; const float* bout;
  float* gW[4]; float* gb[4]; float* gWout; float* gbout;
  int nout;
  bf16x8 *W_r[4], *W_t[4], *Wout_r, *Wout_t;
  float *a[4], *u1f, *du2, *du1, *dhx;
  bf16x8 *a1_r, *u1_r, *a3_r, *u2_r, *a1T, *u1T, *a3T, *u2T;
  bf16x8 *g_r[4], *gT[4];
  float* head;
  float* ghead;
  bf16x8 *ghead_r, *gheadT;
};
struct Encoder {
  const float *Wih, *Whh, *bih, *bhh;
  float *gWih, *gWhh, *gbih, *gbhh;
  int in_dim, cat_off;
  bf16x8 *Wih_r, *Whh_r, *Whh_t;
  bf16x8 *x0_r, *x1_r, *xT;
  float *gi1, *gi2, *gh2, *h1f;
  bf16x8 *h1_r, *hprevT;
  bf16x8 *dgiT, *dghT, *dgh_r;
  float *dhp, *dh1;
};

}

struct egx_policy_train {
  int n = 0, Sn = 0;
  Arena ar;
  Encoder enc[2];
  Branch br[2];
  float* catf = nullptr;
  bf16x8 *cat_r = nullptr, *catT = nullptr;
  PackEntry* tab_weights = nullptr; int n_weights = 0, frags_weights = 0;
  PackEntry* tab_inputs = nullptr; int n_inputs = 0, frags_inputs = 0;
  PackEntry* tab_loss = nullptr; int n_loss = 0, frags_loss = 0;
  std::vector<PackEntry> h_inputs;
  const float* bound_state = nullptr; const float* bound_ego = nullptr;
  int prec = 0;
};

namespace {

int upload_table(std::vector<PackEntry>& v, PackEntry** dev, int* frags) {
  int run = 0;
  for (PackEntry& e : v) {
    if (e.transpose == 2) {
      run += egx_ceil_div(e.red, 32) * egx_ceil_div(e.cols, 32);
    } else {
      const int rows = e.transpose ? e.cols + (e.ones_row >= 0 ? 1 : 0) : e.red;
      const int red = e.transpose ? e.red : e.cols;
      run += (int)img_frags(rows, red);
    }
    e.frag_end = run;
  }
  *frags = run;
  if (!*dev) EGX_HIP_CHECK(hipMalloc(reinterpret_cast<void**>(dev), v.size() * sizeof(PackEntry)));
  EGX_HIP_CHECK(hipMemcpy(*dev, v.data(), v.size() * sizeof(PackEntry), hipMemcpyHostToDevice));
  return EGX_OK;
}
void run_table(hipStream_t st, const PackEntry* tab, int n, int frags, int nplanes = 3) {
  hipLaunchKernelGGL(egx_pack3_table_kernel, dim3(egx_ceil_div(frags, 4)), dim3(256), 0, st, tab, n, nplanes);
}
inline int planes_of(int prec) { return prec == 0 ? 3 : (prec == 2 ? 2 : 1); }

void layout(egx_policy_train* h) {
  const int n = h->n, Sn = h->Sn;
  Arena& ar = h->ar;
  ar.off = 0;
  auto img = [&](int rows, int red) { return static_cast<bf16x8*>(ar.take(img_frags(rows, red) * FRAG_BYTES)); };
  auto f32 = [&](size_t count) { return static_cast<float*>(ar.take(count * sizeof(float))); };
  for (int e = 0; e < 2; ++e) {
    Encoder& E = h->enc[e];
    E.Wih_r = img(3 * HD, E.in_dim); E.Whh_r = img(3 * HD, HD); E.Whh_t = img(HD, 3 * HD);
    E.x0_r = img(n, E.in_dim); E.x1_r = img(n, E.in_dim); E.xT = img(E.in_dim + 1, 2 * n);
    E.gi1 = f32((size_t)n * 3 * HD); E.gi2 = f32((size_t)n * 3 * HD); E.gh2 = f32((size_t)n * 3 * HD); E.h1f = f32((size_t)n * HD);
    E.h1_r = img(n, HD); E.hprevT = img(HD + 1, 2 * n);
    E.dgiT = img(3 * HD, 2 * n); E.dghT = img(3 * HD, 2 * n); E.dgh_r = img(n, 3 * HD);
    E.dhp = f32((size_t)n * HD); E.dh1 = f32((size_t)n * HD);
  }
  h->catf = f32((size_t)n * CAT); h->cat_r = img(n, CAT); h->catT = img(CAT + 1, n);
  for (int b = 0; b < 2; ++b) {
    Branch& B = h->br[b];
    for (int l = 0; l < 4; ++l) { B.W_r[l] = img(CAT, CAT); B.W_t[l] = img(CAT, CAT); B.a[l] = f32((size_t)n * CAT); }
    B.Wout_r = img(B.nout, CAT); B.Wout_t = img(CAT, B.nout);
    B.u1f = f32((size_t)n * CAT); B.du2 = f32((size_t)n * CAT); B.du1 = f32((size_t)n * CAT); B.dhx = f32((size_t)n * CAT);
    B.a1_r = img(n, CAT); B.u1_r = img(n, CAT); B.a3_r = img(n, CAT); B.u2_r = img(n, CAT);
    B.a1T = img(CAT + 1, n); B.u1T = img(CAT + 1, n); B.a3T = img(CAT + 1, n); B.u2T = img(CAT + 1, n);
    for (int l = 0; l < 4; ++l) { B.g_r[l] = img(n, CAT); B.gT[l] = img(CAT, n); }
    B.head = f32((size_t)n * B.nout); B.ghead = f32((size_t)n * B.nout);
    B.ghead_r = img(n, B.nout); B.gheadT = img(B.nout, n);
  }
  (void)Sn;
}

__global__ void egx_ones_row_kernel(bf16x8* img, int row, int S_total, int s_lo, int s_hi) {
  const int s = s_lo + blockIdx.x, kg = threadIdx.x;
  if (s >= s_hi) return;
  const int lane = (row & 15) + 16 * kg;
  bf16x8 one;
#pragma unroll
  for (int e = 0; e < 8; ++e) one[e] = (short)0x3F80;
  img[((size_t)(row >> 4) * S_total + s) * 3 * 64 + lane] = one;
}

}

extern "C" int egx_policy_train_create(const egx_policy_weights* w, const egx_policy_grads* g, int num_rows, egx_policy_train** out) {
  EGX_REQUIRE(w && g && out, "null argument");
  EGX_REQUIRE(num_rows > 0 && num_rows % 32 == 0, "the minibatch must be a multiple of 32 rows");
  auto* h = new egx_policy_train();
  h->n = num_rows; h->Sn = num_rows / 32;
  Encoder& X = h->enc[0];
  X.Wih = w->x_enc_w_ih; X.Whh = w->x_enc_w_hh; X.bih = w->x_enc_b_ih; X.bhh = w->x_enc_b_hh;
  X.gWih = g->x_enc_w_ih; X.gWhh = g->x_enc_w_hh; X.gbih = g->x_enc_b_ih; X.gbhh = g->x_enc_b_hh;
  X.in_dim = ST_DIM; X.cat_off = 0;
  Encoder& E = h->enc[1];
  E.Wih = w->ego_enc_w_ih; E.Whh = w->ego_enc_w_hh; E.bih = w->ego_enc_b_ih; E.bhh = w->ego_enc_b_hh;
  E.gWih = g->ego_enc_w_ih; E.gWhh = g->ego_enc_w_hh; E.gbih = g->ego_enc_b_ih; E.gbhh = g->ego_enc_b_hh;
  E.in_dim = EGO_DIM; E.cat_off = HD;
  for (int l = 0; l < 4; ++l) {
    h->br[0].W[l] = w->actor_w[l]; h->br[0].b[l] = w->actor_b[l]; h->br[0].gW[l] = g->actor_w[l]; h->br[0].gb[l] = g->actor_b[l];
    h->br[1].W[l] = w->critic_w[l]; h->br[1].b[l] = w->critic_b[l]; h->br[1].gW[l] = g->critic_w[l]; h->br[1].gb[l] = g->critic_b[l];
  }
  h->br[0].Wout = w->actor_out_w; h->br[0].bout = w->actor_out_b; h->br[0].gWout = g->actor_out_w; h->br[0].gbout = g->actor_out_b;
  h->br[0].nout = ZP;
  h->br[1].Wout = w->critic_out_w; h->br[1].bout = w->critic_out_b; h->br[1].gWout = g->critic_out_w; h->br[1].gbout = g->critic_out_b;
  h->br[1].nout = 1;
  layout(h);
  h->ar.cap = h->ar.off;
  if (hipMalloc(reinterpret_cast<void**>(&h->ar.base), h->ar.cap) != hipSuccess) {
    delete h;
    egx_set_error("egx_policy_train_create: device allocation failed");
    return EGX_ERR_HIP;
  }
  auto fail = [&](int rc_) { egx_policy_train_destroy(h); return rc_; };
#define U3_CHECK(expr) do { hipError_t e_ = (expr); if (e_ != hipSuccess) { egx_set_error(std::string("egx_policy_train_create: ") + hipGetErrorString(e_)); return fail(EGX_ERR_HIP); } } while (0)
  U3_CHECK(hipMemset(h->ar.base, 0, h->ar.cap));
  layout(h);
  const int n = h->n, Sn = h->Sn;
  auto ones = [&](bf16x8* img, int row, int S_total, int s_lo, int s_hi) {
    hipLaunchKernelGGL(egx_ones_row_kernel, dim3(s_hi - s_lo), dim3(4), 0, nullptr, img, row, S_total, s_lo, s_hi);
  };
  for (int e = 0; e < 2; ++e) ones(h->enc[e].hprevT, HD, 2 * Sn, 0, 2 * Sn);
  ones(h->catT, CAT, Sn, 0, Sn);
  for (int b = 0; b < 2; ++b)
    for (bf16x8* img : {h->br[b].a1T, h->br[b].u1T, h->br[b].a3T, h->br[b].u2T}) ones(img, CAT, Sn, 0, Sn);
  U3_CHECK(hipGetLastError());
  std::vector<PackEntry> tw;
  auto add = [](std::vector<PackEntry>& v, const float* src, int red, int cols, int ld, int col0, bf16x8* dst, int S_total, int s0,
                int transpose, int ones_row) {
    PackEntry e;
    e.src = src; e.red = red; e.cols = cols; e.ld = ld; e.col0 = col0; e.dst = dst; e.S_total = S_total; e.s0 = s0;
    e.transpose = transpose; e.ones_row = ones_row; e.frag_end = 0; e.dst2 = nullptr; e.S_total2 = 0;
    v.push_back(e);
  };
  auto add_both = [](std::vector<PackEntry>& v, const float* src, int rows, int cols, bf16x8* img, bf16x8* imgT) {
    PackEntry e;
    e.src = src; e.red = rows; e.cols = cols; e.ld = cols; e.col0 = 0; e.dst = img; e.S_total = egx_ceil_div(cols, 32); e.s0 = 0;
    e.transpose = 2; e.ones_row = -1; e.frag_end = 0; e.dst2 = imgT; e.S_total2 = egx_ceil_div(rows, 32);
    v.push_back(e);
  };
  for (int e = 0; e < 2; ++e) {
    Encoder& En = h->enc[e];
    add(tw, En.Wih, 3 * HD, En.in_dim, En.in_dim, 0, En.Wih_r, egx_ceil_div(En.in_dim, 32), 0, 0, -1);
    add_both(tw, En.Whh, 3 * HD, HD, En.Whh_r, En.Whh_t);
  }
  for (int b = 0; b < 2; ++b) {
    Branch& B = h->br[b];
    for (int l = 0; l < 4; ++l) {
      add_both(tw, B.W[l], CAT, CAT, B.W_r[l], B.W_t[l]);
    }
    add_both(tw, B.Wout, B.nout, CAT, B.Wout_r, B.Wout_t);
  }
  h->n_weights = (int)tw.size();
  int rc = upload_table(tw, &h->tab_weights, &h->frags_weights);
  if (rc) return fail(rc);
  for (int e = 0; e < 2; ++e) {
    Encoder& En = h->enc[e];
    const int d = En.in_dim, S = egx_ceil_div(d, 32);
    add(h->h_inputs, nullptr, n, d, 2 * d, 0, En.x0_r, S, 0, 0, -1);
    add(h->h_inputs, nullptr, n, d, 2 * d, d, En.x1_r, S, 0, 0, -1);
    add(h->h_inputs, nullptr, n, d, 2 * d, 0, En.xT, 2 * Sn, 0, 1, d);
    add(h->h_inputs, nullptr, n, d, 2 * d, d, En.xT, 2 * Sn, Sn, 1, d);
  }
  h->n_inputs = (int)h->h_inputs.size();
  std::vector<PackEntry> tl;
  for (int b = 0; b < 2; ++b) {
    Branch& B = h->br[b];
    add(tl, B.ghead, n, B.nout, B.nout, 0, B.ghead_r, egx_ceil_div(B.nout, 32), 0, 0, -1);
    add(tl, B.ghead, n, B.nout, B.nout, 0, B.gheadT, Sn, 0, 1, -1);
  }
  h->n_loss = (int)tl.size();
  if ((rc = upload_table(tl, &h->tab_loss, &h->frags_loss))) return fail(rc);
  U3_CHECK(hipDeviceSynchronize());
#undef U3_CHECK
  *out = h;
  return EGX_OK;
}

extern "C" void egx_policy_train_destroy(egx_policy_train* h) {
  if (!h) return;
  (void)hipFree(h->ar.base); (void)hipFree(h->tab_weights); (void)hipFree(h->tab_inputs); (void)hipFree(h->tab_loss);
  delete h;
}

extern "C" int egx_policy_train_refresh(egx_policy_train* h, void* stream) {
  EGX_REQUIRE(h, "null handle");
  const int planes = std::max(planes_of(h->prec), planes_of(egx_policy_get_precision()));
  run_table(static_cast<hipStream_t>(stream), h->tab_weights, h->n_weights, h->frags_weights, planes);
  EGX_HIP_CHECK(hipGetLastError());
  return EGX_OK;
}

extern "C" int egx_policy_train_set_precision(egx_policy_train* h, int prec) {
  EGX_REQUIRE(h, "null handle");
  EGX_REQUIRE(prec == 0 || prec == 1 || prec == 2, "precision must be 0 (three bf16 planes: fp32-equivalent), 2 (two planes) or 1 (bf16)");
  h->prec = prec;
  return EGX_OK;
}

extern "C" int egx_policy_train_packed(const egx_policy_train* h, egx_policy_packed3* out) {
  EGX_REQUIRE(h && out, "null argument");
  out->x_enc_w_ih = h->enc[0].Wih_r; out->x_enc_w_hh = h->enc[0].Whh_r;
  out->ego_enc_w_ih = h->enc[1].Wih_r; out->ego_enc_w_hh = h->enc[1].Whh_r;
  for (int l = 0; l < 4; ++l) { out->actor_w[l] = h->br[0].W_r[l]; out->critic_w[l] = h->br[1].W_r[l]; }
  out->actor_out_w = h->br[0].Wout_r; out->critic_out_w = h->br[1].Wout_r;
  return EGX_OK;
}

extern "C" int egx_policy_train_bind(egx_policy_train* h, const float* state, const float* egosensing) {
  EGX_REQUIRE(h && state && egosensing, "null argument");
  if (h->bound_state == state && h->bound_ego == egosensing && h->tab_inputs) return EGX_OK;
  for (int i = 0; i < 4; ++i) h->h_inputs[i].src = state;
  for (int i = 4; i < 8; ++i) h->h_inputs[i].src = egosensing;
  int rc = upload_table(h->h_inputs, &h->tab_inputs, &h->frags_inputs);
  if (rc) return rc;
  h->bound_state = state; h->bound_ego = egosensing;
  return EGX_OK;
}

static int train_step_parts(egx_policy_train* h, const float* dist, const float* time, const float* act, const float* adv,
                            const float* ret, const float* logp_old, const float* adv_stats, const float* scale, float adv_eps,
                            float min_logvar, float max_logvar, float eps_clip, float vf_coef, float ent_coef, float* out_terms,
                            void* stream_, int parts);

extern "C" int egx_policy_train_step(egx_policy_train* h, const float* dist, const float* time, const float* act, const float* adv,
                                     const float* ret, const float* logp_old, const float* adv_stats, const float* scale,
                                     float adv_eps, float min_logvar, float max_logvar, float eps_clip, float vf_coef, float ent_coef,
                                     float* out_terms, void* stream_) {
  return train_step_parts(h, dist, time, act, adv, ret, logp_old, adv_stats, scale, adv_eps, min_logvar, max_logvar, eps_clip, vf_coef,
                          ent_coef, out_terms, stream_, 3);
}

extern "C" int egx_policy_train_step_heads(egx_policy_train* h, const float* dist, const float* time, const float* act, const float* adv,
                                           const float* ret, const float* logp_old, const float* adv_stats, const float* scale,
                                           float adv_eps, float min_logvar, float max_logvar, float eps_clip, float vf_coef,
                                           float ent_coef, float* out_terms, void* stream_) {
  return train_step_parts(h, dist, time, act, adv, ret, logp_old, adv_stats, scale, adv_eps, min_logvar, max_logvar, eps_clip, vf_coef,
                          ent_coef, out_terms, stream_, 1);
}
extern "C" int egx_policy_train_step_encoders(egx_policy_train* h, void* stream_) {
  EGX_REQUIRE(h, "null handle");
  return train_step_parts(h, nullptr, nullptr, nullptr, nullptr, nullptr, nullptr, nullptr, nullptr, 0.f, 0.f, 0.f, 0.f, 0.f, 0.f, nullptr,
                          stream_, 2);
}

static int train_step_parts(egx_policy_train* h, const float* dist, const float* time, const float* act, const float* adv,
                            const float* ret, const float* logp_old, const float* adv_stats, const float* scale, float adv_eps,
                            float min_logvar, float max_logvar, float eps_clip, float vf_coef, float ent_coef, float* out_terms,
                            void* stream_, int parts) {
  EGX_REQUIRE(h && (!(parts & 1) || (dist && time && act && adv && ret && logp_old && scale && out_terms)), "null argument");
  EGX_REQUIRE(h->tab_inputs, "egx_policy_train_bind has not been called");
  hipStream_t st = static_cast<hipStream_t>(stream_);
  const int n = h->n, Sn = h->Sn;
  constexpr int S_HD = HD / 32, S_CAT = CAT / 32, S_G = 3 * HD / 32;
  const float slope = 0.01f;
  const int prec = h->prec;
  auto launch_n = [prec](hipStream_t s_, D3Plain* ps, int cnt) {
    for (int i = 0; i < cnt; ++i) ps[i].prec = prec;
    egx_launch_dense3_n(s_, ps, cnt);
  };
  auto launch_gru = [prec](hipStream_t s_, D3Gru& g0, D3Gru& g1) {
    g0.prec = g1.prec = prec;
    return egx_launch_gru3_pair(s_, g0, g1);
  };

  int rc = EGX_OK;
  if (parts & 1) {
  run_table(st, h->tab_inputs, h->n_inputs, h->frags_inputs, planes_of(h->prec));
  egx_launch_posenc3(st, dist, time, n, h->catf + 2 * HD, CAT, h->cat_r, S_CAT, 2 * S_HD, h->catT, Sn, 2 * HD, out_terms);
  {
    D3Gru g[2];
    for (int e = 0; e < 2; ++e) {
      Encoder& E = h->enc[e];
      const int Sx = egx_ceil_div(E.in_dim, 32);
      D3Gru& q = g[e];
      q.M = n; q.H = HD;
      q.Ai = E.x0_r; q.SAi = Sx; q.Bi = E.Wih_r; q.Si = Sx; q.bias_i = E.bih; q.bias_h = E.bhh;
      q.gi_out = E.gi1; q.h_out = E.h1f; q.ldo = HD; q.h_out3 = E.h1_r; q.S3 = S_HD;
      q.h_out3T = E.hprevT; q.S3T = 2 * Sn; q.s3T0 = Sn; q.col0T = 0;
    }
    launch_gru(st, g[0], g[1]);
    for (int e = 0; e < 2; ++e) {
      Encoder& E = h->enc[e];
      D3Gru& q = g[e];
      q.Ai = E.x1_r; q.gi_out = E.gi2; q.gh_out = E.gh2;
      q.Ah = E.h1_r; q.SAh = S_HD; q.Bh = E.Whh_r; q.Sh = S_HD; q.h_prev = E.h1f; q.ldh = HD;
      q.h_out = h->catf + E.cat_off; q.ldo = CAT; q.h_out3 = h->cat_r; q.S3 = S_CAT; q.s30 = E.cat_off / 32;
      q.h_out3T = h->catT; q.S3T = Sn; q.s3T0 = 0; q.col0T = E.cat_off;
    }
    launch_gru(st, g[0], g[1]);
  }
  {
    D3Plain L[2];
    auto fwd = [&](int l, const bf16x8* in_a, const bf16x8* in_c, const float* res_a, const float* res_c, float* outf_a, float* outf_c,
                   bf16x8* o3_a, bf16x8* o3_c, bf16x8* o3T_a, bf16x8* o3T_c) {
      const bf16x8* in[2] = {in_a, in_c};
      const float* res[2] = {res_a, res_c};
      float* outf[2] = {outf_a, outf_c};
      bf16x8* o3[2] = {o3_a, o3_c};
      bf16x8* o3T[2] = {o3T_a, o3T_c};
      for (int b = 0; b < 2; ++b) {
        Branch& B = h->br[b];
        D3Plain& q = L[b];
        q = D3Plain();
        q.M = n; q.N = CAT; q.A = in[b]; q.SA = S_CAT; q.S = S_CAT; q.B = B.W_r[l]; q.bias = B.b[l]; q.act = 3; q.slope = slope;
        q.out_act = B.a[l]; q.ldact = CAT;
        q.res = res[b]; q.ldr = CAT; q.out = outf[b]; q.ldo = CAT;
        q.out3 = o3[b]; q.S3 = S_CAT; q.out3T = o3T[b]; q.S3T = Sn;
      }
      launch_n(st, L, 2);
    };
    Branch &Ba = h->br[0], &Bc = h->br[1];
    fwd(0, h->cat_r, h->cat_r, nullptr, nullptr, nullptr, nullptr, Ba.a1_r, Bc.a1_r, Ba.a1T, Bc.a1T);
    fwd(1, Ba.a1_r, Bc.a1_r, h->catf, h->catf, Ba.u1f, Bc.u1f, Ba.u1_r, Bc.u1_r, Ba.u1T, Bc.u1T);
    fwd(2, Ba.u1_r, Bc.u1_r, nullptr, nullptr, nullptr, nullptr, Ba.a3_r, Bc.a3_r, Ba.a3T, Bc.a3T);
    fwd(3, Ba.a3_r, Bc.a3_r, Ba.u1f, Bc.u1f, nullptr, nullptr, Ba.u2_r, Bc.u2_r, Ba.u2T, Bc.u2T);
    for (int b = 0; b < 2; ++b) {
      Branch& B = h->br[b];
      D3Plain& q = L[b];
      q = D3Plain();
      q.M = n; q.N = B.nout; q.A = B.u2_r; q.SA = S_CAT; q.S = S_CAT; q.B = B.Wout_r; q.bias = B.bout; q.out = B.head; q.ldo = B.nout;
    }
    launch_n(st, L, 2);
  }
  rc = egx_ppo_loss_packed_precleared(h->br[0].head, h->br[1].head, act, adv, ret, logp_old, adv_stats, scale, adv_eps, min_logvar, max_logvar,
                               eps_clip, vf_coef, ent_coef, n, h->br[0].ghead, h->br[1].ghead, out_terms, st);
  if (rc) return rc;
  run_table(st, h->tab_loss, h->n_loss, h->frags_loss, planes_of(h->prec));
  hipStream_t sw = st;
  auto wgrad = [&](D3Plain& q, const bf16x8* gT, const bf16x8* xT, int rows, float* gW, float* gb) {
    q = D3Plain();
    q.M = rows; q.N = CAT + 1; q.A = gT; q.SA = Sn; q.S = Sn; q.B = xT; q.out = gW; q.ldo = CAT; q.n_split = CAT; q.bias_out = gb;
  };
  Branch &Ba = h->br[0], &Bc = h->br[1];
  D3Plain W[4], D[2];
  for (int b = 0; b < 2; ++b) wgrad(W[b], h->br[b].gheadT, h->br[b].u2T, h->br[b].nout, h->br[b].gWout, h->br[b].gbout);
  launch_n(sw, W, 2);
  auto dgrad = [&](const bf16x8* const (&gin)[2], const int (&S_in)[2], const bf16x8* const (&Wt)[2], float* const (&res)[2],
                   float* const (&outf)[2], int gate, int lout) {
    for (int b = 0; b < 2; ++b) {
      Branch& B = h->br[b];
      D3Plain& d = D[b];
      d = D3Plain();
      d.M = n; d.N = CAT; d.A = gin[b]; d.SA = S_in[b]; d.S = S_in[b]; d.B = Wt[b];
      d.res = res[b]; d.ldr = CAT; d.out = outf[b]; d.ldo = CAT;
      if (gate >= 0) {
        d.dact = B.a[gate]; d.lddact = CAT; d.dact_code = 3; d.dact_slope = slope;
        d.out3 = B.g_r[lout]; d.S3 = S_CAT; d.out3T = B.gT[lout]; d.S3T = Sn;
      }
    }
    launch_n(st, D, 2);
  };
  const int S_head[2] = {egx_ceil_div(Ba.nout, 32), egx_ceil_div(Bc.nout, 32)}, S_full[2] = {S_CAT, S_CAT};
  float* const none[2] = {nullptr, nullptr};
  {
    const bf16x8* const gin[2] = {Ba.ghead_r, Bc.ghead_r};
    const bf16x8* const Wt[2] = {Ba.Wout_t, Bc.Wout_t};
    float* const outf[2] = {Ba.du2, Bc.du2};
    dgrad(gin, S_head, Wt, none, outf, 3, 3);
  }
  D3Plain WL[8];
  auto layer_bwd = [&](int l, bf16x8* const (&xT)[2], float* const (&res)[2], float* const (&outf)[2], int gate) {
    for (int b = 0; b < 2; ++b) wgrad(WL[2 * l + b], h->br[b].gT[l], xT[b], CAT, h->br[b].gW[l], h->br[b].gb[l]);
    const bf16x8* const gin[2] = {Ba.g_r[l], Bc.g_r[l]};
    const bf16x8* const Wt[2] = {Ba.W_t[l], Bc.W_t[l]};
    dgrad(gin, S_full, Wt, res, outf, gate, gate);
    return EGX_OK;
  };
  {
    bf16x8* const x3[2] = {Ba.a3T, Bc.a3T};
    if ((rc = layer_bwd(3, x3, none, none, 2))) return rc;
    bf16x8* const x2[2] = {Ba.u1T, Bc.u1T};
    float* const du2[2] = {Ba.du2, Bc.du2};
    float* const du1[2] = {Ba.du1, Bc.du1};
    if ((rc = layer_bwd(2, x2, du2, du1, 1))) return rc;
    bf16x8* const x1[2] = {Ba.a1T, Bc.a1T};
    if ((rc = layer_bwd(1, x1, none, none, 0))) return rc;
    bf16x8* const x0[2] = {h->catT, h->catT};
    float* const dhx[2] = {Ba.dhx, Bc.dhx};
    if ((rc = layer_bwd(0, x0, du1, dhx, -1))) return rc;
    launch_n(sw, WL, 4);
    launch_n(sw, WL + 4, 4);
  }
  }
  if (parts & 2) {
    hipStream_t sw = st;
    GruBwd2 two;
    const int blocks = (n / 32) * (HD / 32);
    two.blocks0 = blocks;
    GruBwd* gb[2] = {&two.a, &two.b};
    for (int e = 0; e < 2; ++e) {
      Encoder& E = h->enc[e];
      GruBwd& q = *gb[e];
      q.gi = E.gi2; q.gh = E.gh2; q.bias_h = E.bhh; q.h_prev = E.h1f;
      q.dh0 = h->br[0].dhx + E.cat_off; q.ld0 = CAT; q.dh1 = h->br[1].dhx + E.cat_off; q.ld1 = CAT;
      q.dgiT = E.dgiT; q.dghT = E.dghT; q.ST = 2 * Sn; q.s0T = Sn; q.dgh_r = E.dgh_r; q.dhp = E.dhp; q.M = n; q.H = HD;
    }
    hipLaunchKernelGGL(egx_gru_bwd3_kernel, dim3(2 * blocks), dim3(256), 0, st, two);
    D3Plain P[4];
    for (int e = 0; e < 2; ++e) {
      Encoder& E = h->enc[e];
      D3Plain& d = P[e];
      d = D3Plain();
      d.M = n; d.N = HD; d.A = E.dgh_r; d.SA = S_G; d.S = S_G; d.B = E.Whh_t; d.res = E.dhp; d.ldr = HD; d.out = E.dh1; d.ldo = HD;
    }
    launch_n(st, P, 2);
    for (int e = 0; e < 2; ++e) {
      Encoder& E = h->enc[e];
      GruBwd& q = *gb[e];
      q.gi = E.gi1; q.gh = nullptr; q.h_prev = nullptr; q.dh0 = E.dh1; q.ld0 = HD; q.dh1 = nullptr; q.ld1 = 0;
      q.s0T = 0; q.dgh_r = nullptr; q.dhp = nullptr;
    }
    hipLaunchKernelGGL(egx_gru_bwd3_kernel, dim3(2 * blocks), dim3(256), 0, st, two);
      for (int e = 0; e < 2; ++e) {
      Encoder& E = h->enc[e];
      D3Plain& a = P[2 * e];
      a = D3Plain();
      a.M = 3 * HD; a.N = E.in_dim + 1; a.A = E.dgiT; a.SA = 2 * Sn; a.S = 2 * Sn; a.B = E.xT; a.out = E.gWih; a.ldo = E.in_dim;
      a.n_split = E.in_dim; a.bias_out = E.gbih;
      D3Plain& c = P[2 * e + 1];
      c = D3Plain();
      c.M = 3 * HD; c.N = HD + 1; c.A = E.dghT; c.SA = 2 * Sn; c.S = 2 * Sn; c.B = E.hprevT; c.out = E.gWhh; c.ldo = HD;
      c.n_split = HD; c.bias_out = E.gbhh;
    }
    launch_n(sw, P, 4);
  }
  EGX_HIP_CHECK(hipGetLastError());
  return EGX_OK;
}
```

egogen_amd/ppo_policy.py:

```python
from __future__ import annotations

import ctypes as C
import math
import os
from typing import Dict, List, Optional

import numpy as np
import torch
import torch.distributed as dist
from torch import nn

from . import _lib
from .models import ActorCritic, GAMMAActor, GAMMACritic, GAMMAPolicyBase, PolicyHipRunner

_EPS = float(np.finfo(np.float32).eps)
_LOG_SQRT_2PI = math.log(math.sqrt(2 * math.pi))
_UPDATE_PREC = {"f32": 0, "bf16x2": 2, "bf16": 1}


class RunningMeanStd:

    def __init__(self):
        self.mean, self.var, self.count = 0.0, 1.0, 0

    def update(self, x) -> None:
        x = np.asarray(x, np.float64).reshape(-1)
        self.update_from_moments(float(x.mean()), float(x.var()), x.size)

    def update_from_moments(self, bm: float, bv: float, bc) -> None:
        delta = bm - self.mean
        tot = self.count + bc
        new_mean = self.mean + delta * bc / tot
        m2 = self.var * self.count + bv * bc + delta ** 2 * self.count * bc / tot
        self.mean, self.var, self.count = new_mean, m2 / tot, tot


class RolloutBatch:

    def __init__(self, n: int, A: int, device):
        f = dict(dtype=torch.float32, device=device)
        self.n, self.A = n, A
        self.state = torch.zeros(n + 1, A, 2, 402, **f)
        self.ego = torch.zeros(n + 1, A, 2, 32, **f)
        self.dist = torch.zeros(n + 1, A, **f)
        self.time = torch.zeros(n + 1, A, **f)
        self.act = torch.zeros(n, A, 128, **f)
        self.mu = torch.zeros(n, A, 128, **f)
        self.logvar = torch.zeros(n, A, 128, **f)
        self.logp_old = torch.zeros(n, A, **f)
        self.rew = torch.zeros(n, A, **f)
        self.term = torch.zeros(n, A, dtype=torch.int32, device=device)
        self.values = torch.zeros(n + 1, A, **f)
        self.returns = torch.zeros(n, A, **f)
        self.adv = torch.zeros(n, A, **f)

    def store_obs(self, t: int, obs: Dict[str, torch.Tensor]):
        self.state[t].copy_(obs["state"])
        self.ego[t].copy_(obs["egosensing"])
        self.dist[t].copy_(obs["dist"].reshape(-1))
        self.time[t].copy_(obs["time"].reshape(-1))

    def obs_flat(self, upto: Optional[int] = None) -> Dict[str, torch.Tensor]:
        k = self.n if upto is None else upto
        return {"state": self.state[:k].reshape(-1, 2, 402), "egosensing": self.ego[:k].reshape(-1, 2, 32),
                "dist": self.dist[:k].reshape(-1), "time": self.time[:k].reshape(-1)}


class GAMMAPPOPolicy(nn.Module):
    def __init__(self, actor: GAMMAActor, critic: GAMMACritic, shared_net: GAMMAPolicyBase, optim: torch.optim.Optimizer,
                 dist_fn=None, discount_factor: float = 0.99, gae_lambda: float = 0.95, max_grad_norm: Optional[float] = None,
                 vf_coef: float = 0.5, ent_coef: float = 0.01, weight_kld: float = 1.0, reward_normalization: bool = False,
                 eps_clip: float = 0.2, dual_clip: Optional[float] = None, value_clip: bool = False,
                 advantage_normalization: bool = True, recompute_advantage: bool = False,
                 deterministic_eval: bool = False, max_batchsize: int = 256, seed: int = 0, **_ignored):
        super().__init__()
        assert dual_clip is None or dual_clip > 1.0, "Dual-clip PPO parameter should greater than 1.0."
        self._dual_clip = dual_clip
        self._value_clip = bool(value_clip)
        self._rew_norm = bool(reward_normalization)
        self._recompute_adv = bool(recompute_advantage)
        self.ret_rms = RunningMeanStd()
        self.actor, self.critic, self.shared_net = actor, critic, shared_net
        self._actor_critic = ActorCritic(actor, critic)
        self.optim = optim
        self._gamma, self._lambda = discount_factor, gae_lambda
        self._grad_norm = max_grad_norm
        self._weight_vf, self._weight_ent, self._weight_kld = vf_coef, ent_coef, weight_kld
        self._eps_clip = eps_clip
        self._norm_adv = bool(advantage_normalization)
        self._deterministic_eval = deterministic_eval
        self._batch = max_batchsize
        self._runner = PolicyHipRunner(shared_net, actor, critic)
        self._noise_gen: Optional[torch.Generator] = None
        self._seed = seed
        self._perm_gen = torch.Generator().manual_seed(seed)
        self._flat_grad: Optional[torch.Tensor] = None
        self._after_minibatch = None
        self._layout = None
        self._graph_cache: dict = {}
        self.use_update_graph = bool(_ignored.get("use_update_graph", False))
        self.overlap_allreduce = os.environ.get("EGX_DP_OVERLAP", "0") == "1"
        self.use_fused_loss = bool(_ignored.get("use_fused_loss", True))
        self._scale_cache = {}
        self.use_train_step = bool(_ignored.get("use_train_step", os.environ.get("EGX_TRAIN_STEP", "1") != "0"))
        self._train_handles: dict = {}
        self.update_precision = str(_ignored.get("update_precision", os.environ.get("EGX_UPDATE_PREC", "f32")))
        if self.update_precision not in _UPDATE_PREC:
            raise ValueError(f"update_precision must be one of {sorted(_UPDATE_PREC)}, got {self.update_precision!r}")
        self.use_fused_linear = bool(_ignored.get("use_fused_linear", True))
        self.use_flat_optimizer = bool(_ignored.get("use_flat_optimizer", os.environ.get("EGX_FLAT_OPTIMIZER", "1") != "0"))
        self._flat_opt_state = None
        self.world_size = dist.get_world_size() if dist.is_available() and dist.is_initialized() else 1
        self._dp = self.world_size > 1 or (os.environ.get("EGX_FORCE_DP_PATH") == "1" and dist.is_available() and dist.is_initialized())
        self.update_paths: dict = {}
        self.allreduce_events: list = []
        self._allreduce_done: list = []

    @torch.no_grad()
    def forward(self, obs: Dict[str, torch.Tensor], noise: Optional[torch.Tensor] = None, out: Optional[dict] = None):
        lib = _lib.load()
        out = self._runner.forward(obs, want_actor=True, want_critic=True, out=out)
        n = out["mu"].shape[0]
        dev = out["mu"].device
        deterministic = self._deterministic_eval and not self.training
        if not deterministic and noise is None:
            if self._noise_gen is None:
                self._noise_gen = torch.Generator(device=dev)
                rank = dist.get_rank() if self.world_size > 1 else 0
                self._noise_gen.manual_seed(self._seed + 1 + 9973 * rank)
            noise = torch.randn(n, 128, generator=self._noise_gen, device=dev)
        if "act" not in out:
            out["act"] = torch.empty(n, 128, dtype=torch.float32, device=dev)
            out["logp"] = torch.empty(n, dtype=torch.float32, device=dev)
        rc = lib.egx_sample_action(_lib.ptr(out["mu"]), _lib.ptr(out["logvar"]), _lib.ptr(noise) if noise is not None else None,
                                   float(self.actor.min_logvar), float(self.actor.max_logvar), 1 if deterministic else 0, n,
                                   _lib.ptr(out["act"]), _lib.ptr(out["logp"]), _lib.current_stream_ptr())
        _lib.check(rc, "egx_sample_action")
        return out

    @torch.no_grad()
    def values(self, obs: Dict[str, torch.Tensor]) -> torch.Tensor:
        return self._runner.forward(obs, want_actor=False, want_critic=True)["value"]

    @torch.no_grad()
    def process_fn(self, batch: RolloutBatch):
        lib = _lib.load()
        n, A = batch.n, batch.A
        if getattr(batch, "rollout_values_valid", False) and not getattr(self, "_recomputing", False):
            last = {k: v[n * A:(n + 1) * A] for k, v in batch.obs_flat(n + 1).items()}
            batch.values[n].copy_(self.values(last))
        else:
            v = self.values(batch.obs_flat(n + 1))
            batch.values.copy_(v.reshape(n + 1, A))
        values = batch.values
        scale = 1.0
        if self._rew_norm:
            scale = float(np.sqrt(self.ret_rms.var + _EPS))
            values = (batch.values * scale).contiguous()
        rc = lib.egx_gae(_lib.ptr(values), _lib.ptr(batch.rew), _lib.ptr(batch.term), n, A, float(self._gamma),
                         float(self._lambda), _lib.ptr(batch.returns), _lib.ptr(batch.adv), _lib.current_stream_ptr())
        _lib.check(rc, "egx_gae")
        if self._rew_norm:
            unnorm = batch.returns.detach().double()
            batch.returns.div_(scale)
            if self._dp:
                mom = torch.stack([unnorm.sum(), (unnorm * unnorm).sum(), torch.tensor(float(unnorm.numel()), dtype=torch.float64,
                                                                                       device=unnorm.device)])
                dist.all_reduce(mom)
                s1, s2, cnt = (float(v) for v in mom.cpu())
                mean = s1 / cnt
                self.ret_rms.update_from_moments(mean, max(0.0, s2 / cnt - mean * mean), cnt)
            else:
                self.ret_rms.update(unnorm.cpu().numpy())
        return batch

    def _dist_params(self, obs):
        hx = self.shared_net(obs)
        (mu, logvar), _ = self.actor(hx)
        logvar = logvar.clamp(self.actor.min_logvar, self.actor.max_logvar)
        sigma = torch.exp(logvar) ** 0.5
        return hx, mu, sigma

    @staticmethod
    def log_prob(mu, sigma, act):
        return (-((act - mu) ** 2) / (2 * sigma ** 2) - torch.log(sigma) - _LOG_SQRT_2PI).sum(-1)

    @staticmethod
    def entropy(sigma):
        return (0.5 + _LOG_SQRT_2PI + torch.log(sigma)).sum(-1)

    def _flat_layout(self):
        if self._layout is None:
            params = [p for g in self.optim.param_groups for p in g["params"]]
            off, lay = 0, []
            for p in params:
                lay.append((p, off, p.numel()))
                off += (p.numel() + 63) // 64 * 64
            self._layout, self._layout_total = lay, off
        return self._layout

    def _ensure_flat_grads(self):
        lay = self._flat_layout()
        if self._flat_grad is None:
            self._flat_grad = torch.zeros(self._layout_total, dtype=torch.float32, device=lay[0][0].device)
        base = self._flat_grad.data_ptr()
        for p, off, n in lay:
            if p.grad is None or p.grad.data_ptr() != base + 4 * off:
                p.grad = self._flat_grad[off:off + n].view_as(p)

    def _loss_options(self) -> bool:
        return self._dual_clip is not None or self._value_clip

    def minibatch_loss(self, obs, act, adv, returns, logp_old, global_stats=None, v_s=None):
        n_local = adv.shape[0]
        if adv.is_cuda and self.use_fused_loss and not self._loss_options():
            return self._minibatch_loss_fused(obs, act, adv, returns, logp_old, global_stats)
        hx, mu, sigma = self._dist_params(obs)
        if self._norm_adv:
            if global_stats is None:
                mean, std = adv.mean(), adv.std()
            else:
                mean, std = global_stats[0], global_stats[1]
            adv = (adv - mean) / (std + _EPS)
        scale = 1.0 / n_local if global_stats is None else 1.0 / global_stats[2]
        lp = self.log_prob(mu, sigma, act)
        ratio = (lp - logp_old).exp().float()
        surr1 = ratio * adv
        surr2 = ratio.clamp(1.0 - self._eps_clip, 1.0 + self._eps_clip) * adv
        if self._dual_clip:
            clip1 = torch.min(surr1, surr2)
            clip2 = torch.max(clip1, self._dual_clip * adv)
            clip_loss = -torch.where(adv < 0, clip2, clip1).sum() * scale
        else:
            clip_loss = -torch.min(surr1, surr2).sum() * scale
        value = self.critic(hx).flatten()
        if self._value_clip:
            if v_s is None:
                raise ValueError("value_clip needs the old values v_s of the minibatch")
            v_clip = v_s + (value - v_s).clamp(-self._eps_clip, self._eps_clip)
            vf_loss = torch.max((returns - value).pow(2), (returns - v_clip).pow(2)).sum() * scale
        else:
            vf_loss = (returns - value).pow(2).sum() * scale
        ent_loss = self.entropy(sigma).sum() * scale
        kld_loss = 0.5 * mu.pow(2).sum() * scale / mu.shape[1]
        loss = clip_loss + self._weight_vf * vf_loss - self._weight_ent * ent_loss
        return loss, {"loss": loss, "loss/clip": clip_loss, "loss/vf": vf_loss, "loss/ent": ent_loss, "loss/kld": kld_loss,
                      "approx_kl": (logp_old - lp).sum() * scale}

    def _gather(self, batch: RolloutBatch, idx: torch.Tensor):
        N = batch.n * batch.A
        obs_all = batch.obs_flat()
        if idx.is_cuda and self.use_fused_loss and all(v.dtype == torch.float32 for v in obs_all.values()):
            from .fused_ops import gather_rows
            st, ego, di, ti, act, adv, ret, lpo = gather_rows(idx, [
                obs_all["state"].reshape(N, 804), obs_all["egosensing"].reshape(N, 64), obs_all["dist"].reshape(N, 1),
                obs_all["time"].reshape(N, 1), batch.act.reshape(N, 128), batch.adv.reshape(N, 1), batch.returns.reshape(N, 1),
                batch.logp_old.reshape(N, 1)])
            n = idx.shape[0]
            obs = {"state": st.reshape(n, 2, 402), "egosensing": ego.reshape(n, 2, 32), "dist": di.reshape(n), "time": ti.reshape(n)}
            return obs, act, adv.reshape(n), ret.reshape(n), lpo.reshape(n)
        obs = {k: v.index_select(0, idx) for k, v in obs_all.items()}
        return (obs, batch.act.reshape(N, 128).index_select(0, idx), batch.adv.reshape(N).index_select(0, idx),
                batch.returns.reshape(N).index_select(0, idx), batch.logp_old.reshape(N).index_select(0, idx))

    def _train_handle(self, n: int):
        if not (self.use_train_step and self.use_fused_loss and self.use_fused_linear and n % 32 == 0 and self.actor.z_dim == 128
                and self._flat_opt_state == "ready" and self._flat_grad is not None and self._flat_grad.is_cuda and self._norm_adv
                and self._chain_shapes_ok() and not self._loss_options()):
            return None
        hs = self._train_handles.get(n)
        if hs is not None:
            return hs
        if self._graph_cache:
            self._graph_cache.clear()
        lib = _lib.load()
        self._ensure_flat_grads()
        w = self._runner._weights()
        g = _lib.PolicyGrads()
        s, a, c = self.shared_net, self.actor.pnet, self.critic.vnet
        gp = lambda t: t.grad.data_ptr()
        g.x_enc_w_ih, g.x_enc_w_hh, g.x_enc_b_ih, g.x_enc_b_hh = gp(s.x_enc.weight_ih_l0), gp(s.x_enc.weight_hh_l0), gp(s.x_enc.bias_ih_l0), gp(s.x_enc.bias_hh_l0)
        g.ego_enc_w_ih, g.ego_enc_w_hh, g.ego_enc_b_ih, g.ego_enc_b_hh = (gp(s.ego_enc.weight_ih_l0), gp(s.ego_enc.weight_hh_l0),
                                                                            gp(s.ego_enc.bias_ih_l0), gp(s.ego_enc.bias_hh_l0))
        for b in range(2):
            for k in range(2):
                g.actor_w[2 * b + k], g.actor_b[2 * b + k] = gp(a.layers[b].layers[k].weight), gp(a.layers[b].layers[k].bias)
                g.critic_w[2 * b + k], g.critic_b[2 * b + k] = gp(c.layers[b].layers[k].weight), gp(c.layers[b].layers[k].bias)
        g.actor_out_w, g.actor_out_b = gp(a.out_fc.weight), gp(a.out_fc.bias)
        g.critic_out_w, g.critic_out_b = gp(c.out_fc.weight), gp(c.out_fc.bias)
        h = C.c_void_p()
        _lib.check(lib.egx_policy_train_create(C.byref(w), C.byref(g), int(n), C.byref(h)), "egx_policy_train_create")
        _lib.check(lib.egx_policy_train_set_precision(h, _UPDATE_PREC[self.update_precision]), "egx_policy_train_set_precision")
        dev = self._flat_grad.device
        f = dict(dtype=torch.float32, device=dev)
        bufs = [torch.empty(n, 804, **f), torch.empty(n, 64, **f), torch.empty(n, 1, **f), torch.empty(n, 1, **f),
                torch.empty(n, 128, **f), torch.empty(n, 1, **f), torch.empty(n, 1, **f), torch.empty(n, 1, **f)]
        _lib.check(lib.egx_policy_train_bind(h, _lib.ptr(bufs[0]), _lib.ptr(bufs[1])), "egx_policy_train_bind")
        packed = _lib.PolicyPacked3()
        _lib.check(lib.egx_policy_train_packed(h, C.byref(packed)), "egx_policy_train_packed")
        hs = {"h": h, "bufs": bufs, "stats": torch.zeros(2, **f), "key": (w.x_enc_w_ih, g.x_enc_w_ih), "packed": packed}
        self._train_handles[n] = hs
        if len(self._train_handles) == 1:
            self._runner.adopt_packed(packed, refresh=self._refresh_images)
            self._images_owner = n
        self._refresh_images()
        return hs

    def _chain_shapes_ok(self) -> bool:
        ok = getattr(self, "_chain_ok", None)
        if ok is None:
            a, c, s = self.actor.pnet, self.critic.vnet, self.shared_net
            def block_ok(blk, nout):
                return (blk.residual and len(blk.layers) == 2 and blk.out_fc.out_features == nout and blk.out_fc.in_features == 1152
                        and all(m.act_name == "lrelu" and len(m.layers) == 2 and
                                all(fc.in_features == 1152 and fc.out_features == 1152 for fc in m.layers) for m in blk.layers))
            ok = (s.h_dim == 512 and s.x_enc.input_size == 402 and s.ego_enc.input_size == 32 and block_ok(a, 256) and block_ok(c, 1))
            self._chain_ok = ok
        return ok

    def _drop_train_handles(self):
        lib = _lib.load() if self._train_handles else None
        for hs in self._train_handles.values():
            lib.egx_policy_train_destroy(hs["h"])
        self._train_handles = {}
        self._runner._wstruct = None

    def __del__(self):
        try:
            self._drop_train_handles()
        except Exception:
            pass

    def _refresh_images(self):
        if not self._train_handles:
            return
        lib, st = _lib.load(), _lib.current_stream_ptr()
        for hs in self._train_handles.values():
            _lib.check(lib.egx_policy_train_refresh(hs["h"], st), "egx_policy_train_refresh")

    def _fwd_bwd_train_step(self, hs, batch, idx, gstats, log_out, part: str = "all"):
        from .fused_ops import gather_rows
        lib, st = _lib.load(), _lib.current_stream_ptr()
        if part == "encoders":
            _lib.check(lib.egx_policy_train_step_encoders(hs["h"], st), "egx_policy_train_step_encoders")
            return
        N = batch.n * batch.A
        obs_all = batch.obs_flat()
        b = hs["bufs"]
        gather_rows(idx, [obs_all["state"].reshape(N, 804), obs_all["egosensing"].reshape(N, 64), obs_all["dist"].reshape(N, 1),
                          obs_all["time"].reshape(N, 1), batch.act.reshape(N, 128), batch.adv.reshape(N, 1), batch.returns.reshape(N, 1),
                          batch.logp_old.reshape(N, 1)], out=b)
        n = int(idx.shape[0])
        dev = b[0].device
        if gstats is None:
            _lib.check(lib.egx_adv_stats(_lib.ptr(b[5]), n, _lib.ptr(hs["stats"]), st), "egx_adv_stats")
            scale = self._scale_cache.get((n, dev))
            if scale is None:
                scale = torch.full((1,), 1.0 / n, dtype=torch.float32, device=dev)
                self._scale_cache[(n, dev)] = scale
        else:
            hs["stats"].copy_(torch.stack([gstats[0], gstats[1]]).float())
            scale = (1.0 / gstats[2]).reshape(1).float()
        fn = lib.egx_policy_train_step_heads if part == "heads" else lib.egx_policy_train_step
        rc = fn(hs["h"], _lib.ptr(b[2]), _lib.ptr(b[3]), _lib.ptr(b[4]), _lib.ptr(b[5]), _lib.ptr(b[6]), _lib.ptr(b[7]),
                _lib.ptr(hs["stats"]), _lib.ptr(scale), float(_EPS), float(self.actor.min_logvar),
                float(self.actor.max_logvar), float(self._eps_clip), float(self._weight_vf), float(self._weight_ent),
                _lib.ptr(log_out), st)
        _lib.check(rc, "egx_policy_train_step")

    def _fwd_bwd(self, batch, idx, gstats, log_out) -> str:
        hs = self._train_handle(int(idx.shape[0])) if idx.is_cuda else None
        if hs is not None:
            self._fwd_bwd_train_step(hs, batch, idx, gstats, log_out)
            return "chain"
        obs, act, adv, ret, lpo = self._gather(batch, idx)
        v_s = batch.values[:batch.n].reshape(-1).index_select(0, idx) if self._value_clip else None
        loss, terms = self.minibatch_loss(obs, act, adv, ret, lpo, gstats, v_s=v_s)
        self._flat_grad.zero_()
        loss.backward()
        if adv.is_cuda and self.use_fused_loss and self.use_fused_linear:
            from . import models as _m
            if _m._TWO_STREAM_UPDATE:
                torch.cuda.current_stream().wait_stream(_m._side_stream(adv.device))
        packed = terms.get("_packed")
        if packed is not None:
            log_out.copy_(packed)
        else:
            log_out.copy_(torch.stack([terms[k].detach() for k in ("loss", "loss/clip", "loss/vf", "loss/ent", "loss/kld", "approx_kl")]))
        return "autograd"

    def _clip_and_step(self):
        if self.use_flat_optimizer and self._flat_opt_state == "ready":
            g = self.optim.param_groups[0]
            lib = _lib.load()
            b1, b2 = g["betas"]
            rc = lib.egx_adamw_clip_step(_lib.ptr(self._flat_p), _lib.ptr(self._flat_grad), _lib.ptr(self._flat_m), _lib.ptr(self._flat_v),
                                         self._flat_p.numel(), self._n_clip, float(self._grad_norm or 0.0), float(g["lr"]), float(b1),
                                         float(b2), float(g["eps"]), float(g["weight_decay"]), _lib.ptr(self._step_t),
                                         _lib.ptr(self._adamw_ws), _lib.current_stream_ptr())
            _lib.check(rc, "egx_adamw_clip_step")
            self._runner.mark_dirty()
            self._refresh_images()
            return
        if self._grad_norm:
            nn.utils.clip_grad_norm_(self._actor_critic.parameters(), max_norm=self._grad_norm)
        self.optim.step()
        self._refresh_images()

    def _flat_optimizer_ready(self) -> bool:
        if self._flat_opt_state == "unsupported":
            return False
        opt = self.optim
        params = [p for g in opt.param_groups for p in g["params"]]
        if self._flat_opt_state is None:
            ok = (isinstance(opt, torch.optim.AdamW) and len(opt.param_groups) == 1 and not opt.param_groups[0].get("amsgrad", False)
                  and not opt.param_groups[0].get("maximize", False) and all(p.is_cuda and p.dtype == torch.float32 for p in params))
            clip = list(self._actor_critic.parameters())
            ok = ok and len(clip) <= len(params) and all(a is b for a, b in zip(clip, params))
            if not ok:
                self._flat_opt_state = "unsupported"
                return False
            dev = params[0].device
            lay = self._flat_layout()
            total = self._layout_total
            self._flat_p = torch.zeros(total, dtype=torch.float32, device=dev)
            self._flat_m = torch.zeros(total, dtype=torch.float32, device=dev)
            self._flat_v = torch.zeros(total, dtype=torch.float32, device=dev)
            self._step_t = torch.zeros((), dtype=torch.float32, device=dev)
            self._adamw_ws = torch.zeros(int(_lib.load().egx_adamw_workspace_floats()), dtype=torch.float32, device=dev)
            self._n_clip = lay[len(clip)][1] if len(clip) < len(lay) else total
            with torch.no_grad():
                for p, off, n in lay:
                    self._flat_p[off:off + n].copy_(p.detach().reshape(-1))
                    p.data = self._flat_p[off:off + n].view_as(p)
            self._flat_opt_state = "ready"
            self._graph_cache.clear()
            self._drop_train_handles()
        st0 = opt.state.get(params[0], {})
        if st0.get("exp_avg") is None or st0["exp_avg"].data_ptr() != self._flat_m.data_ptr():
            with torch.no_grad():
                for p, off, n in self._flat_layout():
                    st = opt.state[p]
                    mv, vv = self._flat_m[off:off + n].view_as(p), self._flat_v[off:off + n].view_as(p)
                    if torch.is_tensor(st.get("exp_avg")):
                        mv.copy_(st["exp_avg"]); vv.copy_(st["exp_avg_sq"])
                    else:
                        mv.zero_(); vv.zero_()
                    if "step" in st and p is params[0]:
                        self._step_t.fill_(float(st["step"]))
                    st["exp_avg"], st["exp_avg_sq"], st["step"] = mv, vv, self._step_t
            self._graph_cache.clear()
        return True

    def optim_state_dict(self) -> dict:
        sd = self.optim.state_dict()
        out_state = {}
        for k, st in sd["state"].items():
            ns = {}
            for name, v in st.items():
                if name == "step":
                    ns[name] = torch.tensor(float(v), dtype=torch.float32)
                elif torch.is_tensor(v):
                    ns[name] = v.detach().clone()
                else:
                    ns[name] = v
            out_state[k] = ns
        return {"state": out_state, "param_groups": sd["param_groups"]}

    def _global_adv_stats(self, batch: RolloutBatch, perm: torch.Tensor, spans) -> torch.Tensor:
        adv = batch.adv.reshape(-1).double()
        sizes = {e - s for s, e in spans}
        if len(sizes) == 1:
            a = adv.index_select(0, perm[spans[0][0]:spans[-1][1]]).reshape(len(spans), -1)
            mom = torch.stack([a.sum(1), (a * a).sum(1), torch.full_like(a[:, 0], float(a.shape[1]))], dim=1)
        else:
            rows = []
            for s, e in spans:
                a = adv.index_select(0, perm[s:e])
                rows.append(torch.stack([a.sum(), (a * a).sum(), torch.full_like(a[0], float(e - s))]))
            mom = torch.stack(rows)
        mom = mom.contiguous()
        dist.all_reduce(mom)
        ng = mom[:, 2]
        mean = mom[:, 0] / ng
        var = (mom[:, 1] - ng * mean * mean) / (ng - 1)
        return torch.stack([mean, var.clamp(min=0).sqrt(), ng], dim=1).float()

    def _grad_buckets(self):
        n = getattr(self, "_n_clip", None)
        g = self._flat_grad
        if n is None or n <= 0 or n >= g.numel():
            return [g]
        return [g[:n], g[n:]]

    def _all_reduce_grad(self, bucket=None):
        ev = self.allreduce_events.pop() if self.allreduce_events else None
        if ev is not None:
            ev[0].record()
        dist.all_reduce(self._flat_grad if bucket is None else bucket)
        if ev is not None:
            ev[1].record()
            self._allreduce_done.append(ev)

    def _comm_stream(self):
        s = getattr(self, "_comm_s", None)
        if s is None:
            s = self._comm_s = torch.cuda.Stream()
        return s

    def _graphs_for(self, batch: RolloutBatch, local_bs: int):
        key = (id(batch), local_bs)
        g = self._graph_cache.get(key)
        if g is not None:
            return g
        dev = batch.act.device
        st = {"idx": torch.zeros(local_bs, dtype=torch.long, device=dev), "log": torch.zeros(6, device=dev),
              "gstats": torch.tensor([0.0, 1.0, float(local_bs * self.world_size)], device=dev), "use_gstats": self._dp}
        gs = (lambda: (st["gstats"][0], st["gstats"][1], st["gstats"][2])) if st["use_gstats"] else (lambda: None)
        try:
            snap = {k: v.clone() for k, v in self.state_dict().items()}
            params = [p_ for g_ in self.optim.param_groups for p_ in g_["params"]]
            osnap = {id(p_): {k: v.clone() for k, v in self.optim.state.get(p_, {}).items() if torch.is_tensor(v)} for p_ in params}
            side = torch.cuda.Stream()
            side.wait_stream(torch.cuda.current_stream())
            with torch.cuda.stream(side):
                for _ in range(3):
                    self._fwd_bwd(batch, st["idx"], gs(), st["log"])
                    self._clip_and_step()
            torch.cuda.current_stream().wait_stream(side)
            torch.cuda.synchronize()
            g1 = torch.cuda.CUDAGraph()
            g2 = None
            if not self._dp:
                with torch.cuda.graph(g1):
                    st["path"] = self._fwd_bwd(batch, st["idx"], gs(), st["log"])
                    self._clip_and_step()
            else:
                hs = self._train_handle(local_bs) if st["idx"].is_cuda else None
                if hs is not None and len(self._grad_buckets()) == 2 and self.overlap_allreduce:
                    with torch.cuda.graph(g1):
                        self._fwd_bwd_train_step(hs, batch, st["idx"], gs(), st["log"], part="heads")
                    g1b = torch.cuda.CUDAGraph()
                    with torch.cuda.graph(g1b, pool=g1.pool()):
                        self._fwd_bwd_train_step(hs, batch, st["idx"], gs(), st["log"], part="encoders")
                    st["g1b"], st["path"] = g1b, "chain"
                else:
                    with torch.cuda.graph(g1):
                        st["path"] = self._fwd_bwd(batch, st["idx"], gs(), st["log"])
                g2 = torch.cuda.CUDAGraph()
                with torch.cuda.graph(g2, pool=g1.pool()):
                    self._clip_and_step()
            self.load_state_dict(snap)
            for p_ in params:
                for k, v in self.optim.state.get(p_, {}).items():
                    if torch.is_tensor(v):
                        old_v = osnap[id(p_)].get(k)
                        v.copy_(old_v) if old_v is not None else v.zero_()
            st["g1"], st["g2"] = g1, g2
            self._refresh_images()
        except Exception as e:
            import warnings
            warnings.warn(f"PPO update graph capture failed ({type(e).__name__}: {e}); running the update eagerly")
            st["g1"] = st["g2"] = None
            st["failed"] = True
        self._graph_cache[key] = st
        return st

    def _minibatch_loss_fused(self, obs, act, adv, returns, logp_old, global_stats):
        from .fused_ops import PPOLossFn, PPOLossPackedFn
        zp = None
        if self.use_fused_linear:
            from .models import fused_update_forward
            self._ensure_flat_grads()
            if self.actor.z_dim == 128:
                zp, value = fused_update_forward(self.shared_net, self.actor, self.critic, obs, packed=True)
            else:
                mu, logvar, value = fused_update_forward(self.shared_net, self.actor, self.critic, obs)
        else:
            hx = self.shared_net(obs)
            (mu, logvar), _ = self.actor(hx)
            value = self.critic(hx).flatten()
        n_local = adv.shape[0]
        dev = adv.device
        stats = None
        if self._norm_adv:
            if global_stats is None:
                from .fused_ops import adv_stats
                stats = adv_stats(adv)
            else:
                stats = torch.stack([global_stats[0], global_stats[1]]).float()
        if global_stats is None:
            scale = self._scale_cache.get((n_local, dev))
            if scale is None:
                scale = torch.full((1,), 1.0 / n_local, dtype=torch.float32, device=dev)
                self._scale_cache[(n_local, dev)] = scale
        else:
            scale = (1.0 / global_stats[2]).reshape(1).float()
        if zp is not None:
            loss, terms = PPOLossPackedFn.apply(zp, value, act, adv, returns, logp_old, stats, scale, _EPS, self.actor.min_logvar,
                                                self.actor.max_logvar, self._eps_clip, self._weight_vf, self._weight_ent)
        else:
            loss, terms = PPOLossFn.apply(mu, logvar, value, act, adv, returns, logp_old, stats, scale, _EPS, self.actor.min_logvar,
                                          self.actor.max_logvar, self._eps_clip, self._weight_vf, self._weight_ent)
        return loss, {"loss": terms[0], "loss/clip": terms[1], "loss/vf": terms[2], "loss/ent": terms[3], "loss/kld": terms[4],
                      "approx_kl": terms[5], "_packed": terms}

    def learn(self, batch: RolloutBatch, batch_size: int, repeat: int) -> Dict[str, List[float]]:
        self.train()
        self._ensure_flat_grads()
        if self.use_flat_optimizer and batch.act.is_cuda:
            self._flat_optimizer_ready()
        self._refresh_images()
        ws = self.world_size
        dp = self._dp
        N = batch.n * batch.A
        dev = batch.act.device
        local_bs = max(1, batch_size // ws)
        names = ("loss", "loss/clip", "loss/vf", "loss/ent", "loss/kld")
        stats = {k: [] for k in names}
        logs = []
        use_graph = self.use_update_graph and dev.type == "cuda"
        kld_rows = []
        for step in range(repeat):
            if self._recompute_adv and step > 0:
                self._recomputing = True
                try:
                    self._runner.mark_dirty()
                    self._refresh_images()
                    self.process_fn(batch)
                finally:
                    self._recomputing = False
            if getattr(self, "_perm_queue", None):
                perm = torch.as_tensor(self._perm_queue.pop(0), dtype=torch.long).to(dev)
            else:
                perm = torch.randperm(N, generator=self._perm_gen).to(dev)
            bounds = list(range(0, N, local_bs))
            if len(bounds) > 1 and N - bounds[-1] < local_bs:
                bounds.pop()
            last_log = None
            spans = [(s, bounds[i + 1] if i + 1 < len(bounds) else N) for i, s in enumerate(bounds)]
            gstats_all = self._global_adv_stats(batch, perm, spans) if dp else None
            for i, (s, e) in enumerate(spans):
                idx = perm[s:e]
                st = self._graphs_for(batch, local_bs) if (use_graph and e - s == local_bs) else None
                if st is not None and st.get("g1") is not None:
                    st["idx"].copy_(idx)
                    if dp:
                        st["gstats"].copy_(gstats_all[i])
                    st["g1"].replay()
                    if dp:
                        if st.get("g1b") is not None:
                            main, comm = torch.cuda.current_stream(), self._comm_stream()
                            b0, b1 = self._grad_buckets()
                            comm.wait_stream(main)
                            with torch.cuda.stream(comm):
                                self._all_reduce_grad(b0)
                            st["g1b"].replay()
                            comm.wait_stream(main)
                            with torch.cuda.stream(comm):
                                self._all_reduce_grad(b1)
                            main.wait_stream(comm)
                        else:
                            self._all_reduce_grad()
                        st["g2"].replay()
                    last_log = st["log"].clone()
                    self.update_paths[st["path"] + "+graph"] = self.update_paths.get(st["path"] + "+graph", 0) + 1
                else:
                    gstats = None
                    if dp:
                        gstats = (gstats_all[i, 0], gstats_all[i, 1], gstats_all[i, 2])
                    log = torch.zeros(6, device=dev)
                    path = self._fwd_bwd(batch, idx, gstats, log)
                    if dp:
                        self._all_reduce_grad()
                    self._clip_and_step()
                    last_log = log
                    self.update_paths[path] = self.update_paths.get(path, 0) + 1
                logs.append(last_log[:5])
                if self._after_minibatch is not None:
                    self._after_minibatch(len(logs) - 1)
                kld_rows.append(idx)
            if repeat > 1 and last_log is not None:
                kl = last_log[5].clone()
                if dp:
                    dist.all_reduce(kl)
                if float(kl.item()) >= 0.02:
                    break
        self._runner.mark_dirty()
        self._refresh_images()
        if logs:
            L = torch.stack(logs)
            mu2 = batch.mu.reshape(N, -1).pow(2).mean(1)
            if len({int(r.shape[0]) for r in kld_rows}) == 1:
                kld = 0.5 * mu2.index_select(0, torch.cat(kld_rows)).reshape(len(kld_rows), -1).mean(1)
            else:
                kld = torch.stack([0.5 * mu2.index_select(0, r).mean() for r in kld_rows])
            if dp:
                kld = kld / ws
            L[:, 4] = kld
            if dp:
                dist.all_reduce(L)
            for row in L.cpu().tolist():
                for k, v in zip(names, row):
                    stats[k].append(v)
        return stats
```

include/egogen_hip.h:

```cpp
#ifndef EGOGEN_HIP_H
#define EGOGEN_HIP_H

#include <stddef.h>
#include <stdint.h>

#ifdef __cplusplus
extern "C" {
#endif

#define EGX_OK 0
#define EGX_ERR_ARG (-1)
#define EGX_ERR_HIP (-2)
#define EGX_ERR_WORKSPACE (-3)

#define EGX_NUM_JOINTS 55
#define EGX_NUM_JOINTS_OUT 127
#define EGX_XB_DIM 93
#define EGX_NUM_BETAS 10
#define EGX_POSE_FEAT 486
#define EGX_BLEND_K 472

const char* egx_last_error(void);
int egx_version(void);

// ... 61 lines not shown
int egx_point_set_create(const egx_body_model_host* desc, const int32_t* vids_host, int num_points, egx_point_set** out);
void egx_point_set_destroy(egx_point_set* set);
int egx_point_set_size(const egx_point_set* set);
int egx_points_forward(const egx_point_set* set, const float* xb, const float* betas, int num_bodies, int frames_per_agent,
                       float* out_points, float* out_joints55, void* stream);
int egx_points_backward(const egx_point_set* set, const float* xb, const float* betas, int num_bodies, int frames_per_agent,
                        const float* grad_points, const float* grad_joints55, float* grad_xb, float* grad_betas_body, void* stream);

typedef struct egx_sdf_scene_set egx_sdf_scene_set;
int egx_sdf_scene_set_create(const egx_sdf_grid* scenes, int num_scenes, egx_sdf_scene_set** out);
void egx_sdf_scene_set_destroy(egx_sdf_scene_set* set);
int egx_sdf_scene_set_size(const egx_sdf_scene_set* set);

int egx_lbs_forward_scenes(const egx_body_model* m, const float* xb, const float* betas, int num_bodies, int frames_per_agent,
                           float* out_verts, float* out_joints, float* out_markers, const egx_sdf_scene_set* scenes,
                           const int32_t* agent_scene, const float* R0, const float* T0, int32_t* out_pene_count,
                           void* workspace, size_t workspace_bytes, void* stream);

int egx_lbs_joints(const egx_body_model* m, const float* xb, const float* betas, int num_bodies, int frames_per_agent,
                   float* out_joints55, void* workspace, size_t workspace_bytes, void* stream);

int egx_canonical_frame(const float* joints, int joints_per_body, int num_bodies, float* out_R, float* out_T, void* stream);

int egx_update_transl_glorot(const float* R, const float* T, int num_frames, const float* delta_T, const float* xb, int num_bodies,
                             float* out, void* stream);

int egx_sdf_sample(const egx_sdf_grid* sdf, const float* pts, int64_t n, float* out, void* stream);

int egx_mesh_sdf(const float* triangles, int num_triangles, const float* center_host, float scale, int d0, int d1, int d2,
                 int inside_positive, float* out_grid, void* stream);

#define EGX_SDF_MAX_BOXES 16
int egx_sdf_boxes(const float* base_grid, const float* room_lo_hi, const float* boxes, int num_boxes, const float* center_host,
                  float scale, int d0, int d1, int d2, float* out_grid, void* stream);

int egx_scan_sdf(const float* bvh_nodes, int bvh_levels, const float* triangles, const float* pseudo_normals, int num_triangles,
                 int leaf_size, const float* center_host, float scale, int d0, int d1, int d2, float* out_grid, void* stream);

int egx_walkable_raster(const float* triangles, int num_triangles, float origin_x, float origin_y, float cell, int nx, int ny,
                        float floor_height, float floor_tol, float min_up_nz, float z_lo, float z_hi, int* out_support,
                        float* out_clearance, void* stream);

#define EGX_ACT_NONE 0
#define EGX_ACT_TANH 1
#define EGX_ACT_RELU 2
#define EGX_ACT_LRELU 3

typedef struct egx_linear_desc {
  int num_rows;
  int out_features;
  int num_segments;
  const float* seg_ptr[4];
  int seg_width[4];
  int seg_ld[4];
  const float* weight;
  int weight_ld;
  const float* bias;
  const float* residual;
  int residual_ld;
  float* out;
  int out_ld;
  int activation;
  float leaky_slope;
} egx_linear_desc;

int egx_linear(const egx_linear_desc* d, void* stream);

int egx_gru_pointwise(const float* gi, const float* gh, const float* h_prev, int h_prev_ld, float* h_out,
                      int h_out_ld, int num_rows, int hidden, void* stream);

int egx_cont6d_to_aa(const float* xb6, int num_rows, float* out, int out_ld, void* stream);

int egx_posenc(const float* dist, const float* time, int num_agents, float* out, void* stream);

size_t egx_pack3_bytes(int num_rows, int num_cols);
int egx_pack3(const float* src, int num_rows, int num_cols, int src_ld, int src_col0, void* dst, int dst_ksteps,
              int dst_kstep0, void* stream);

size_t egx_gemm3_workspace_bytes(int M, int N, int K);
int egx_gemm3(const float* A, int lda, int trans_a, const float* B, int ldb, int trans_b, int M, int N, int K,
              const float* bias, int act, float slope, const float* res, int ldr, float* out, int ldo, float* out_act,
              int ldact, void* workspace, size_t workspace_bytes, void* stream);

typedef struct egx_prior_packed3 {
  const void *x_enc_w_ih, *x_enc_w_hh;
  const void *drnn_w[3];
  const void *d_rnn_w_hz;
  const void *d_rnn_w_y;
  const void *d_rnn_w_hh;
  const void *d_comb_w;
  const void *d_mlp_w[2];
  const void *d_out_w;
  const void *reg_in_m, *reg_in_xb, *reg_in_betas, *reg_blk, *reg_out;
  const float* reg_blk_b;
} egx_prior_packed3;

typedef struct egx_prior_weights {
  const float *x_enc_w_ih, *x_enc_w_hh, *x_enc_b_ih, *x_enc_b_hh;
  const float *drnn_w[3], *drnn_b[3];
  const float *d_rnn_w_ih, *d_rnn_w_hh, *d_rnn_b_ih, *d_rnn_b_hh;
  const float *d_mlp_w[2], *d_mlp_b[2];
  const float *d_out_w, *d_out_b;
  const float *reg_in_w, *reg_in_b;
  const float *reg_blk_w[20], *reg_blk_b[20];
  const float *reg_out_w, *reg_out_b;
  const float *d_comb_w, *d_comb_b;
  const egx_prior_packed3* packed3;
} egx_prior_weights;

size_t egx_sample_prior_workspace_bytes(int num_agents);

int egx_sample_prior(const egx_prior_weights* w, const float* x_hist0, const float* x_hist1, int x_ld,
                     const float* betas, const float* z, int num_agents, float* out_Y, float* out_Yb,
                     void* workspace, size_t workspace_bytes, void* stream);

typedef struct egx_policy_packed3 {
  const void *x_enc_w_ih, *x_enc_w_hh;
  const void *ego_enc_w_ih, *ego_enc_w_hh;
  const void *actor_w[4], *actor_out_w;
  const void *critic_w[4], *critic_out_w;
} egx_policy_packed3;

typedef struct egx_policy_weights {
  const float *x_enc_w_ih, *x_enc_w_hh, *x_enc_b_ih, *x_enc_b_hh;
  const float *ego_enc_w_ih, *ego_enc_w_hh, *ego_enc_b_ih, *ego_enc_b_hh;
  const float *actor_w[4], *actor_b[4];
  const float *actor_out_w, *actor_out_b;
  const float *critic_w[4], *critic_b[4];
  const float *critic_out_w, *critic_out_b;
  const egx_policy_packed3* packed3;
} egx_policy_weights;

typedef struct egx_policy_grads {
  float *x_enc_w_ih, *x_enc_w_hh, *x_enc_b_ih, *x_enc_b_hh;
  float *ego_enc_w_ih, *ego_enc_w_hh, *ego_enc_b_ih, *ego_enc_b_hh;
  float *actor_w[4], *actor_b[4], *actor_out_w, *actor_out_b;
  float *critic_w[4], *critic_b[4], *critic_out_w, *critic_out_b;
} egx_policy_grads;
typedef struct egx_policy_train egx_policy_train;
int egx_policy_train_create(const egx_policy_weights* w, const egx_policy_grads* g, int num_rows, egx_policy_train** out);
void egx_policy_train_destroy(egx_policy_train* h);
int egx_policy_train_refresh(egx_policy_train* h, void* stream);
int egx_policy_train_packed(const egx_policy_train* h, egx_policy_packed3* out);
int egx_policy_train_bind(egx_policy_train* h, const float* state, const float* egosensing);
int egx_policy_train_step(egx_policy_train* h, const float* dist, const float* time, const float* act, const float* adv,
                          const float* ret, const float* logp_old, const float* adv_stats, const float* scale, float adv_eps,
                          float min_logvar, float max_logvar, float eps_clip, float vf_coef, float ent_coef, float* out_terms,
                          void* stream);
int egx_policy_train_step_heads(egx_policy_train* h, const float* dist, const float* time, const float* act, const float* adv,
                                const float* ret, const float* logp_old, const float* adv_stats, const float* scale, float adv_eps,
                                float min_logvar, float max_logvar, float eps_clip, float vf_coef, float ent_coef, float* out_terms,
                                void* stream);
int egx_policy_train_step_encoders(egx_policy_train* h, void* stream);
int egx_policy_train_set_precision(egx_policy_train* h, int prec);

int egx_policy_set_precision(int bf16);
int egx_policy_get_precision(void);

size_t egx_policy_workspace_bytes(int num_rows);

int egx_policy_forward(const egx_policy_weights* w, const float* state, const float* egosensing, const float* dist,
                       const float* time, int num_rows, float* out_mu, float* out_logvar, float* out_value,
                       void* workspace, size_t workspace_bytes, void* stream);

typedef struct egx_vposer_weights {
  const float *fc1_w, *fc1_b;
  const float *fc2_w, *fc2_b;
  const float *mu_w, *mu_b;
  const void *fc1_w3, *fc2_w3, *mu_w3;
} egx_vposer_weights;

size_t egx_vposer_workspace_bytes(int num_rows);
int egx_vposer_encode(const egx_vposer_weights* w, const float* x, int x_ld, int num_rows, float* out,
                      void* workspace, size_t workspace_bytes, void* stream);

typedef struct egx_env_config {
  float reproj_factor, goal_thresh, pene_thres;
  float weight_skate, weight_floor, weight_face_target, weight_look_target, weight_success, weight_target_dist,
      weight_pene, weight_vp;
  int max_depth;
  int scene_kind;
  int terminate_on_penetration;
  int pene_type_body;
  float ray_len;
  float vp_thresh;
  int no_goal_termination;
} egx_env_config;

typedef struct egx_env_scenes {
  const float* edges;
  const int32_t* edge_off;
  const float* tris;
  const int32_t* tri_off;
  const float* floor_height;
  const float* map_lin;
  int map_res;
  float* crowd_bbox;
  int crowd_group;
  int crowd_scenes;
  int crowd_member;
  float crowd_floor_half;
  int crowd_polygon;
  int crowd_static;
} egx_env_scenes;

typedef struct egx_env_state {
  float* state;
  float* seed;
  float* R0;
  float* T0;
  float* dist;
  int32_t* steps;
  float* wpath;
  int32_t* scene_idx;
} egx_env_state;

typedef struct egx_env_step_io {
  const float* Y_gen;
  const float* pred_params;
  const float* joints;
  const float* markers_proj;
  const int32_t* pene_count;
  const float* vp_emb;
  const int32_t* feet_marker_idx;
  float* reward;
  int32_t* terminated;
  float* reward_terms;
  float* obs_ego;
  float* obs_dist;
  float* obs_time;
  float* out_marker_b;
  float* out_prev_frame;
  int32_t* nonfinite_count;
  int32_t* invalid_flags;
} egx_env_step_io;

typedef struct egx_env_reset_io {
  int num_candidates;
  const int32_t* mask;
  const float* cand_pairs;
  const float* cand_yaw;
  const int32_t* cand_variant;
  const int32_t* cand_scene;
  const int32_t* cand_valid;
  const float* tab_joints;
  const float* tab_markers;
  const float* tab_glorot;
  const float* tab_transl;
  const float* tab_pose;
  float* obs_ego;
  float* obs_dist;
  float* obs_time;
  int32_t* out_choice;
  int32_t* out_pending;
  int32_t* forced_count;
} egx_env_reset_io;

int egx_assemble_params(const float* seed, const float* Yb_gen, int num_agents, float* pred_params, void* stream);
int egx_env_step_post(const egx_env_config* cfg, const egx_env_scenes* scenes, const egx_env_state* st,
                      const egx_env_step_io* io, int num_agents, void* stream);
int egx_env_reset(const egx_env_config* cfg, const egx_env_scenes* scenes, const egx_env_state* st,
                  const egx_env_reset_io* io, int num_agents, void* stream);

int egx_env_get_feature(const float* Y_l, const float* pel, const float* R0, const float* T0, const float* wpath, int wpath_rows,
                        int num_bodies, int num_frames, int num_markers, float* out_dist_xyz, float* out_fea_marker, void* stream);

int egx_env_get_map(const float* tris, int num_tris, float floor_height, const float* map_lin, int res, const float* R, const float* T,
                    int num_bodies, float* out_points_scene, float* out_local_map, void* stream);

int egx_sample_action(const float* mu, float* logvar, const float* eps, float min_logvar, float max_logvar,
                      int deterministic, int num_rows, float* act, float* logp, void* stream);

int egx_gae(const float* values, const float* rew, const int32_t* terminated, int num_steps, int num_agents,
            double gamma, double gae_lambda, float* returns, float* adv, void* stream);

int egx_profile_next_lbs(void* start_event, void* stop_event);
int egx_event_create(void** out_event);
int egx_event_destroy(void* event);
int egx_event_elapsed_ms(void* start_event, void* stop_event, float* out_ms);


int egx_ppo_loss(const float* mu, const float* logvar, const float* value, const float* act, const float* adv,
                 const float* ret, const float* logp_old, const float* adv_stats, const float* scale, float adv_eps,
                 float min_logvar, float max_logvar, float eps_clip, float vf_coef, float ent_coef, int num_rows,
                 float* g_mu, float* g_logvar, float* g_value, float* out_terms, void* stream);
int egx_ppo_loss_packed(const float* zp, const float* value, const float* act, const float* adv, const float* ret,
                        const float* logp_old, const float* adv_stats, const float* scale, float adv_eps, float min_logvar,
                        float max_logvar, float eps_clip, float vf_coef, float ent_coef, int num_rows, float* g_zp, float* g_value,
                        float* out_terms, void* stream);

int egx_gru_pointwise_bwd(const float* gi, const float* gh, const float* h_prev, const float* dh, int num_rows, int hidden,
                          float* dgi, float* dgh, float* dh_prev, void* stream);

int egx_act_fwd(float* z, const float* res, float* out, int num_rows, int width, int act, float slope, void* stream);
int egx_act_bwd_colsum(const float* dy, const float* a, float* g, float* db_accum, int num_rows, int width, int act,
                       float slope, void* stream);

int egx_gather_rows(const int64_t* idx, int num_rows, int num_tensors, const float* const* src, const int* width,
                    float* const* dst, void* stream);

int egx_adv_stats(const float* adv, int n, float* out_mean_std, void* stream);

int egx_track_episode(const float* rew, const int32_t* term, int num_agents, float* ep_ret, float* ep_len, float* done_sums,
                      void* stream);
int egx_rollout_store(const float* state, const float* egosensing, const float* dist, const float* time, const float* rew,
                      const int32_t* term, int num_agents, float* state_dst, float* ego_dst, float* dist_dst, float* time_dst,
                      float* rew_dst, int32_t* term_dst, float* ep_ret, float* ep_len, float* done_sums, void* stream);

size_t egx_adamw_workspace_floats(void);
int egx_adamw_clip_step(float* param, const float* grad, float* exp_avg, float* exp_avg_sq, size_t n, size_t n_clip,
                        float max_norm, double lr, double beta1, double beta2, double eps, double weight_decay, float* step,
                        float* workspace, void* stream);

#ifdef __cplusplus
}
#endif
#endif
```

Measured before the change: 190,700.

## Drive PPO minibatch graphs from a device cursor with fused gather head

Adds a device-side cursor that the AdamW constants kernel increments and the PPO loss kernel uses to index per-minibatch log slots. A new update-head path gathers minibatch rows by permutation inside the captured graph, and posenc and advantage-stats are generalised to gathered rows. Each replay then needs no host index copy or log clone, and the logs are read back once after all replays. Image refreshes are also skipped when the cached key is unchanged. This removes per-minibatch host copies and syncs at the cost of extra graph state and indexing complexity.

```diff
diff --git a/egogen_amd/_lib.py b/egogen_amd/_lib.py
--- a/egogen_amd/_lib.py
+++ b/egogen_amd/_lib.py
@@ -75,6 +75,13 @@
                                           "ego_enc_w_ih", "ego_enc_w_hh", "ego_enc_b_ih", "ego_enc_b_hh")] + \
                [("actor_w", C.c_void_p * 4), ("actor_b", C.c_void_p * 4), ("actor_out_w", C.c_void_p), ("actor_out_b", C.c_void_p),
                 ("critic_w", C.c_void_p * 4), ("critic_b", C.c_void_p * 4), ("critic_out_w", C.c_void_p), ("critic_out_b", C.c_void_p)]
+
+
+class UpdateHead(C.Structure):
+    _fields_ = [("perm", C.c_void_p), ("cursor", C.c_void_p), ("max_cursor", C.c_int), ("num_src_rows", C.c_int)] + \
+               [(n, C.c_void_p) for n in ("state", "egosensing", "dist", "time", "act", "adv", "ret", "logp_old",
+                                          "act_c", "adv_c", "ret_c", "logp_old_c", "stats")] + \
+               [("compute_stats", C.c_int), ("log", C.c_void_p)]
 
 
 class VposerWeights(C.Structure):
@@ -211,6 +218,11 @@
     "egx_policy_train_step_heads": (C.c_int, [C.c_void_p] * 9 + [C.c_float] * 6 + [C.c_void_p, C.c_void_p]),
     "egx_policy_train_step_encoders": (C.c_int, [C.c_void_p, C.c_void_p]),
     "egx_policy_train_set_precision": (C.c_int, [C.c_void_p, C.c_int]),
+    "egx_policy_train_head": (C.c_int, [C.c_void_p, C.POINTER(UpdateHead), C.c_void_p]),
+    "egx_policy_train_step_cursor": (C.c_int, [C.c_void_p, C.POINTER(UpdateHead), C.c_void_p] + [C.c_float] * 6 + [C.c_void_p]),
+    "egx_policy_train_step_heads_cursor": (C.c_int, [C.c_void_p, C.POINTER(UpdateHead), C.c_void_p] + [C.c_float] * 6 + [C.c_void_p]),
+    "egx_adamw_clip_step_cursor": (C.c_int, [C.c_void_p, C.c_void_p, C.c_void_p, C.c_void_p, C.c_size_t, C.c_size_t, C.c_float] +
+                                   [C.c_double] * 5 + [C.c_void_p, C.c_void_p, C.c_void_p, C.c_void_p]),
     "egx_pack3_bytes": (C.c_size_t, [C.c_int, C.c_int]),
     "egx_pack3": (C.c_int, [C.c_void_p, C.c_int, C.c_int, C.c_int, C.c_int, C.c_void_p, C.c_int, C.c_int, C.c_void_p]),
     "egx_gemm3_workspace_bytes": (C.c_size_t, [C.c_int, C.c_int, C.c_int]),
diff --git a/egogen_amd/csrc/dense3.hip b/egogen_amd/csrc/dense3.hip
--- a/egogen_amd/csrc/dense3.hip
+++ b/egogen_amd/csrc/dense3.hip
@@ -490,52 +490,8 @@
                                                           float* __restrict__ out, int ld, bf16x8* __restrict__ out3, int S3, int s0,
                                                           bf16x8* __restrict__ out3T, int S3T, int col0T, float* __restrict__ zero6) {
   if (zero6 && blockIdx.x == 0 && threadIdx.x < 6) zero6[threadIdx.x] = 0.f;
-  int frag = blockIdx.x * 4 + (threadIdx.x >> 6);
-  const int lane = threadIdx.x & 63;
-  const int RT = 2 * ((n + 31) >> 5);
-  if (frag >= RT * 4) {
-    frag -= RT * 4;
-    const int Sn = (n + 31) >> 5;
-    if (!out3T || frag >= 8 * Sn) return;
-    const int t = frag / Sn, s = frag % Sn;
-    const int c = 16 * t + (lane & 15), m0 = 32 * s + 8 * (lane >> 4);
-    float x[8];
-#pragma unroll
-    for (int e = 0; e < 8; ++e) {
-      const int m = m0 + e;
-      float v = 0.f;
-      if (m < n) {
-        const float f = ((c < 64) ? dist[m] : time[m]) * exp2f((float)((c & 63) >> 1));
-        v = (c & 1) ? cosf(f) : sinf(f);
-      }
-      x[e] = v;
-    }
-    bf16x8 pl[3];
-    d3_split(x, pl);
-    bf16x8* o = out3T + ((size_t)((col0T >> 4) + t) * S3T + s) * 3 * 64 + lane;
-#pragma unroll
-    for (int p = 0; p < 3; ++p) o[p * 64] = pl[p];
-    return;
-  }
-  const int rt = frag >> 2, s = frag & 3;
-  const int row = rt * 16 + (lane & 15), c0 = s * 32 + 8 * (lane >> 4);
-  float x[8];
-#pragma unroll
-  for (int e = 0; e < 8; ++e) {
-    const int c = c0 + e;
-    float v = 0.f;
-    if (row < n) {
-      const float f = ((c < 64) ? dist[row] : time[row]) * exp2f((float)((c & 63) >> 1));
-      v = (c & 1) ? cosf(f) : sinf(f);
-      out[(size_t)row * ld + c] = v;
-    }
-    x[e] = v;
-  }
-  bf16x8 pl[3];
-  d3_split(x, pl);
-  bf16x8* o = out3 + ((size_t)rt * S3 + s0 + s) * 3 * 64 + lane;
-#pragma unroll
-  for (int p = 0; p < 3; ++p) o[p * 64] = pl[p];
+  egx_posenc3_role(dist, time, n, out, ld, out3, S3, s0, out3T, S3T, col0T, (int)blockIdx.x, EgxRowsIdentity(),
+                   [](const float (&x)[8], bf16x8 (&pl)[3]) { d3_split(x, pl); });
 }
 void egx_launch_posenc3(hipStream_t st, const float* dist, const float* time, int n, float* out, int ld, void* out3, int S3, int s0,
                         void* out3T, int S3T, int col0T, float* zero6) {
diff --git a/egogen_amd/csrc/egx_nets.h b/egogen_amd/csrc/egx_nets.h
--- a/egogen_amd/csrc/egx_nets.h
+++ b/egogen_amd/csrc/egx_nets.h
@@ -59,9 +59,107 @@
 int egx_ppo_loss_packed_precleared(const float* zp, const float* value, const float* act, const float* adv, const float* ret,
                                    const float* logp_old, const float* adv_stats, const float* scale, float adv_eps, float min_logvar,
                                    float max_logvar, float eps_clip, float vf_coef, float ent_coef, int num_rows, float* g_zp,
-                                   float* g_value, float* out_terms, void* stream_);
+                                   float* g_value, float* out_terms, void* stream_, const int* cursor = nullptr, int max_cursor = 0);
 void egx_launch_posenc3(hipStream_t st, const float* dist, const float* time, int n, float* out, int ld, void* out3, int S3, int s0,
                         void* out3T = nullptr, int S3T = 0, int col0T = 0, float* zero6 = nullptr );
+
+#if defined(__HIPCC__)
+struct EgxRowsIdentity {
+  __device__ __forceinline__ size_t operator()(int r) const { return (size_t)r; }
+};
+struct EgxRowsGathered {
+  const long long* __restrict__ idx;
+  int num_src;
+  __device__ __forceinline__ size_t operator()(int r) const {
+    const long long s = idx[r];
+    return (size_t)min(max(s, 0LL), (long long)num_src - 1);
+  }
+};
+
+template <class Rows, class Split>
+__device__ __forceinline__ void egx_posenc3_role(const float* __restrict__ dist, const float* __restrict__ time, int n,
+                                                 float* __restrict__ out, int ld, bf16x8* __restrict__ out3, int S3, int s0,
+                                                 bf16x8* __restrict__ out3T, int S3T, int col0T, int bid, const Rows& rows,
+                                                 const Split& split) {
+  int frag = bid * 4 + (threadIdx.x >> 6);
+  const int lane = threadIdx.x & 63;
+  const int RT = 2 * ((n + 31) >> 5);
+  if (frag >= RT * 4) {
+    frag -= RT * 4;
+    const int Sn = (n + 31) >> 5;
+    if (!out3T || frag >= 8 * Sn) return;
+    const int t = frag / Sn, s = frag % Sn;
+    const int c = 16 * t + (lane & 15), m0 = 32 * s + 8 * (lane >> 4);
+    float x[8];
+#pragma unroll
+    for (int e = 0; e < 8; ++e) {
+      const int m = m0 + e;
+      float v = 0.f;
+      if (m < n) {
+        const size_t sm = rows(m);
+        const float f = ((c < 64) ? dist[sm] : time[sm]) * exp2f((float)((c & 63) >> 1));
+        v = (c & 1) ? cosf(f) : sinf(f);
+      }
+      x[e] = v;
+    }
+    bf16x8 pl[3];
+    split(x, pl);
+    bf16x8* o = out3T + ((size_t)((col0T >> 4) + t) * S3T + s) * 3 * 64 + lane;
+#pragma unroll
+    for (int p = 0; p < 3; ++p) o[p * 64] = pl[p];
+    return;
+  }
+  const int rt = frag >> 2, s = frag & 3;
+  const int row = rt * 16 + (lane & 15), c0 = s * 32 + 8 * (lane >> 4);
+  const size_t srow = row < n ? rows(row) : 0;
+  float x[8];
+#pragma unroll
+  for (int e = 0; e < 8; ++e) {
+    const int c = c0 + e;
+    float v = 0.f;
+    if (row < n) {
+      const float f = ((c < 64) ? dist[srow] : time[srow]) * exp2f((float)((c & 63) >> 1));
+      v = (c & 1) ? cosf(f) : sinf(f);
+      out[(size_t)row * ld + c] = v;
+    }
+    x[e] = v;
+  }
+  bf16x8 pl[3];
+  split(x, pl);
+  bf16x8* o = out3 + ((size_t)rt * S3 + s0 + s) * 3 * 64 + lane;
+#pragma unroll
+  for (int p = 0; p < 3; ++p) o[p * 64] = pl[p];
+}
+
+template <class Rows>
+__device__ __forceinline__ void egx_adv_stats_role(const float* __restrict__ adv, int n, float* __restrict__ out, const Rows& rows) {
+  __shared__ double red[256];
+  __shared__ double s_mean;
+  double a = 0.0;
+  for (int i = threadIdx.x; i < n; i += 256) a += adv[rows(i)];
+  red[threadIdx.x] = a;
+  __syncthreads();
+  for (int st = 128; st > 0; st >>= 1) {
+    if (threadIdx.x < st) red[threadIdx.x] += red[threadIdx.x + st];
+    __syncthreads();
+  }
+  if (threadIdx.x == 0) s_mean = red[0] / n;
+  __syncthreads();
+  const double mean = s_mean;
+  double b = 0.0;
+  for (int i = threadIdx.x; i < n; i += 256) { const double d = adv[rows(i)] - mean; b += d * d; }
+  red[threadIdx.x] = b;
+  __syncthreads();
+  for (int st = 128; st > 0; st >>= 1) {
+    if (threadIdx.x < st) red[threadIdx.x] += red[threadIdx.x + st];
+    __syncthreads();
+  }
+  if (threadIdx.x == 0) {
+    out[0] = (float)mean;
+    out[1] = (n > 1) ? (float)sqrt(red[0] / (n - 1)) : nanf("");
+  }
+}
+#endif
 
 struct D3Gru {
   const bf16x8* Ai = nullptr;
diff --git a/egogen_amd/csrc/ppo.hip b/egogen_amd/csrc/ppo.hip
--- a/egogen_amd/csrc/ppo.hip
+++ b/egogen_amd/csrc/ppo.hip
@@ -1,6 +1,6 @@
 #include <algorithm>
 #include <cstring>
-#include "egx_common.h"
+#include "egx_nets.h"
 
 namespace {
 constexpr float LOG_SQRT_2PI = 0.91893853320467274178f;
@@ -21,8 +21,10 @@
                                                           float max_lv, float eps_clip, float vf_coef, float ent_coef, int n,
                                                           int stride ,
                                                           float* __restrict__ g_mu, float* __restrict__ g_logvar,
-                                                          float* __restrict__ g_value, float* __restrict__ out_terms) {
+                                                          float* __restrict__ g_value, float* __restrict__ out_terms,
+                                                          const int* __restrict__ cursor, int max_cursor) {
   __shared__ float sh[4][6];
+  if (cursor) out_terms += 6 * (size_t)min(max(*cursor, 0), max_cursor);
   const int lane = threadIdx.x & 63, wave = threadIdx.x >> 6;
   const float scale = scale_ptr[0];
   float acc[6] = {0.f, 0.f, 0.f, 0.f, 0.f, 0.f};
@@ -169,31 +171,7 @@
 }
 
 __global__ __launch_bounds__(256) void egx_adv_stats_kernel(const float* __restrict__ adv, int n, float* __restrict__ out) {
-  __shared__ double red[256];
-  __shared__ double s_mean;
-  double a = 0.0;
-  for (int i = threadIdx.x; i < n; i += 256) a += adv[i];
-  red[threadIdx.x] = a;
-  __syncthreads();
-  for (int st = 128; st > 0; st >>= 1) {
-    if (threadIdx.x < st) red[threadIdx.x] += red[threadIdx.x + st];
-    __syncthreads();
-  }
-  if (threadIdx.x == 0) s_mean = red[0] / n;
-  __syncthreads();
-  const double mean = s_mean;
-  double b = 0.0;
-  for (int i = threadIdx.x; i < n; i += 256) { const double d = adv[i] - mean; b += d * d; }
-  red[threadIdx.x] = b;
-  __syncthreads();
-  for (int st = 128; st > 0; st >>= 1) {
-    if (threadIdx.x < st) red[threadIdx.x] += red[threadIdx.x + st];
-    __syncthreads();
-  }
-  if (threadIdx.x == 0) {
-    out[0] = (float)mean;
-    out[1] = (n > 1) ? (float)sqrt(red[0] / (n - 1)) : nanf("");
-  }
+  egx_adv_stats_role(adv, n, out, EgxRowsIdentity());
 }
 
 __global__ __launch_bounds__(256) void egx_track_episode_kernel(const float* __restrict__ rew, const int* __restrict__ term, int A,
@@ -285,7 +263,8 @@
 
 __global__ __launch_bounds__(256) void egx_adamw_consts_kernel(const float* __restrict__ partials, int n_partials, int do_clip,
                                                                float max_norm, double lr, double b1, double b2,
-                                                               const float* __restrict__ step, float* __restrict__ consts) {
+                                                               const float* __restrict__ step, float* __restrict__ consts,
+                                                               int* __restrict__ cursor) {
   __shared__ double red[256];
   double a = 0.0;
   for (int i = threadIdx.x; i < n_partials; i += 256) a += partials[i];
@@ -303,6 +282,7 @@
     consts[0] = coef;
     consts[1] = (float)(lr / bc1);
     consts[2] = sqrtf(bc2);
+    if (cursor) *cursor += 1;
   }
 }
 
@@ -361,7 +341,7 @@
   hipLaunchKernelGGL(egx_zero_terms_kernel, dim3(1), dim3(64), 0, st, out_terms);
   hipLaunchKernelGGL(egx_ppo_loss_kernel, dim3(ppo_loss_blocks(num_rows)), dim3(256), 0, st, mu, logvar, value, act, adv, ret, logp_old,
                      adv_stats, scale, adv_eps, min_logvar, max_logvar, eps_clip, vf_coef, ent_coef, num_rows, 128, g_mu, g_logvar,
-                     g_value, out_terms);
+                     g_value, out_terms, nullptr, 0);
   EGX_HIP_CHECK(hipGetLastError());
   return EGX_OK;
 }
@@ -369,12 +349,12 @@
 int egx_ppo_loss_packed_precleared(const float* zp, const float* value, const float* act, const float* adv, const float* ret,
                                    const float* logp_old, const float* adv_stats, const float* scale, float adv_eps, float min_logvar,
                                    float max_logvar, float eps_clip, float vf_coef, float ent_coef, int num_rows, float* g_zp,
-                                   float* g_value, float* out_terms, void* stream_) {
+                                   float* g_value, float* out_terms, void* stream_, const int* cursor, int max_cursor) {
   EGX_REQUIRE(zp && value && act && adv && ret && logp_old && scale && g_zp && g_value && out_terms && num_rows > 0, "bad arguments");
   hipStream_t st = static_cast<hipStream_t>(stream_);
   hipLaunchKernelGGL(egx_ppo_loss_kernel, dim3(ppo_loss_blocks(num_rows)), dim3(256), 0, st, zp, zp + 128, value, act, adv, ret, logp_old, adv_stats,
                      scale, adv_eps, min_logvar, max_logvar, eps_clip, vf_coef, ent_coef, num_rows, 256, g_zp, g_zp + 128, g_value,
-                     out_terms);
+                     out_terms, cursor, max_cursor);
   EGX_HIP_CHECK(hipGetLastError());
   return EGX_OK;
 }
@@ -388,7 +368,7 @@
   hipLaunchKernelGGL(egx_zero_terms_kernel, dim3(1), dim3(64), 0, st, out_terms);
   hipLaunchKernelGGL(egx_ppo_loss_kernel, dim3(ppo_loss_blocks(num_rows)), dim3(256), 0, st, zp, zp + 128, value, act, adv, ret, logp_old, adv_stats,
                      scale, adv_eps, min_logvar, max_logvar, eps_clip, vf_coef, ent_coef, num_rows, 256, g_zp, g_zp + 128, g_value,
-                     out_terms);
+                     out_terms, nullptr, 0);
   EGX_HIP_CHECK(hipGetLastError());
   return EGX_OK;
 }
@@ -478,19 +458,33 @@
 
 extern "C" size_t egx_adamw_workspace_floats(void) { return 1024 + 8; }
 
-extern "C" int egx_adamw_clip_step(float* param, const float* grad, float* exp_avg, float* exp_avg_sq, size_t n, size_t n_clip,
-                                   float max_norm, double lr, double beta1, double beta2, double eps, double weight_decay,
-                                   float* step, float* workspace, void* stream_) {
+static int adamw_clip_step(float* param, const float* grad, float* exp_avg, float* exp_avg_sq, size_t n, size_t n_clip,
+                           float max_norm, double lr, double beta1, double beta2, double eps, double weight_decay,
+                           float* step, float* workspace, int* cursor, void* stream_) {
   EGX_REQUIRE(param && grad && exp_avg && exp_avg_sq && step && workspace && n > 0 && n_clip <= n, "bad arguments");
   hipStream_t st = static_cast<hipStream_t>(stream_);
   const int nb = 1024;
   const bool do_clip = max_norm > 0.f && n_clip > 0;
   hipLaunchKernelGGL(egx_sumsq_partial_kernel, dim3(nb), dim3(256), 0, st, grad, do_clip ? n_clip : (size_t)0, workspace, step);
   hipLaunchKernelGGL(egx_adamw_consts_kernel, dim3(1), dim3(256), 0, st, workspace, nb, do_clip ? 1 : 0, max_norm, lr, beta1, beta2,
-                     step, workspace + nb);
+                     step, workspace + nb, cursor);
   const size_t blocks = (n + 1023) / 1024;
   hipLaunchKernelGGL(egx_adamw_flat_kernel, dim3((unsigned)blocks), dim3(256), 0, st, param, grad, exp_avg, exp_avg_sq, n, n_clip,
                      workspace + nb, lr, beta1, beta2, eps, weight_decay);
   EGX_HIP_CHECK(hipGetLastError());
   return EGX_OK;
 }
+
+extern "C" int egx_adamw_clip_step(float* param, const float* grad, float* exp_avg, float* exp_avg_sq, size_t n, size_t n_clip,
+                                   float max_norm, double lr, double beta1, double beta2, double eps, double weight_decay,
+                                   float* step, float* workspace, void* stream_) {
+  return adamw_clip_step(param, grad, exp_avg, exp_avg_sq, n, n_clip, max_norm, lr, beta1, beta2, eps, weight_decay, step, workspace,
+                         nullptr, stream_);
+}
+
+extern "C" int egx_adamw_clip_step_cursor(float* param, const float* grad, float* exp_avg, float* exp_avg_sq, size_t n, size_t n_clip,
+                                          float max_norm, double lr, double beta1, double beta2, double eps, double weight_decay,
+                                          float* step, float* workspace, int32_t* cursor, void* stream_) {
+  return adamw_clip_step(param, grad, exp_avg, exp_avg_sq, n, n_clip, max_norm, lr, beta1, beta2, eps, weight_decay, step, workspace,
+                         cursor, stream_);
+}
diff --git a/egogen_amd/csrc/update3.hip b/egogen_amd/csrc/update3.hip
--- a/egogen_amd/csrc/update3.hip
+++ b/egogen_amd/csrc/update3.hip
@@ -33,6 +33,40 @@
   int S_total2;
 };
 
+template <class Rows>
+__device__ __forceinline__ void u3_pack_fragment(const PackEntry& e, const float* __restrict__ src, int frag, int lane, int nplanes,
+                                                 const Rows& rows) {
+  float x[8];
+  int rt, s;
+  if (!e.transpose) {
+    const int S = (e.cols + 31) >> 5;
+    rt = frag / S; s = frag % S;
+    const int row = rt * 16 + (lane & 15), k0 = s * 32 + 8 * (lane >> 4);
+    const size_t srow = row < e.red ? rows(row) : 0;
+#pragma unroll
+    for (int q = 0; q < 8; ++q) x[q] = (row < e.red && k0 + q < e.cols) ? src[srow * e.ld + e.col0 + k0 + q] : 0.f;
+  } else {
+    const int S = (e.red + 31) >> 5;
+    rt = frag / S; s = frag % S;
+    const int irow = rt * 16 + (lane & 15), k0 = s * 32 + 8 * (lane >> 4);
+#pragma unroll
+    for (int q = 0; q < 8; ++q) {
+      float v = 0.f;
+      if (k0 + q < e.red) {
+        if (irow < e.cols) v = src[rows(k0 + q) * e.ld + e.col0 + irow];
+        else if (irow == e.ones_row) v = 1.f;
+      }
+      x[q] = v;
+    }
+  }
+  bf16x8 pl[3];
+  u3_split(x, pl);
+  bf16x8* o = e.dst + ((size_t)rt * e.S_total + e.s0 + s) * 3 * 64 + lane;
+#pragma unroll
+  for (int p = 0; p < 3; ++p)
+    if (p < nplanes) o[p * 64] = pl[p];
+}
+
 __global__ __launch_bounds__(256) void egx_pack3_table_kernel(const PackEntry* __restrict__ tab, int n, int nplanes) {
   int frag = blockIdx.x * 4 + (threadIdx.x >> 6);
   const int lane = threadIdx.x & 63;
@@ -45,7 +79,6 @@
   const PackEntry e = tab[lo];
   frag -= lo > 0 ? tab[lo - 1].frag_end : 0;
   float x[8];
-  int rt, s;
   if (e.transpose == 2) {
     __shared__ float sblk[4][32][33];
     float (*sb)[33] = sblk[threadIdx.x >> 6];
@@ -86,32 +119,73 @@
     }
     return;
   }
-  if (!e.transpose) {
-    const int S = (e.cols + 31) >> 5;
-    rt = frag / S; s = frag % S;
-    const int row = rt * 16 + (lane & 15), k0 = s * 32 + 8 * (lane >> 4);
-#pragma unroll
-    for (int q = 0; q < 8; ++q) x[q] = (row < e.red && k0 + q < e.cols) ? e.src[(size_t)row * e.ld + e.col0 + k0 + q] : 0.f;
-  } else {
-    const int S = (e.red + 31) >> 5;
-    rt = frag / S; s = frag % S;
-    const int irow = rt * 16 + (lane & 15), k0 = s * 32 + 8 * (lane >> 4);
-#pragma unroll
-    for (int q = 0; q < 8; ++q) {
-      float v = 0.f;
-      if (k0 + q < e.red) {
-        if (irow < e.cols) v = e.src[(size_t)(k0 + q) * e.ld + e.col0 + irow];
-        else if (irow == e.ones_row) v = 1.f;
-      }
-      x[q] = v;
-    }
-  }
-  bf16x8 pl[3];
-  u3_split(x, pl);
-  bf16x8* o = e.dst + ((size_t)rt * e.S_total + e.s0 + s) * 3 * 64 + lane;
-#pragma unroll
-  for (int p = 0; p < 3; ++p)
-    if (p < nplanes) o[p * 64] = pl[p];
+  u3_pack_fragment(e, e.src, frag, lane, nplanes, EgxRowsIdentity());
+}
+
+struct HeadArgs {
+  const PackEntry* tab;
+  int n_tab, frags_tab, nplanes;
+  const float *state, *ego;
+  const long long* perm;
+  const int* cursor;
+  int max_cursor, n, num_src;
+  const float *dist, *time, *act, *adv, *ret, *logp;
+  float *act_c, *adv_c, *ret_c, *logp_c;
+  float* stats;
+  float* log;
+  float* pe_out;
+  int pe_ld;
+  bf16x8* pe3;
+  int S3, s0;
+  bf16x8* pe3T;
+  int S3T, col0T;
+  int b_pack, b_pe, b_gather;
+};
+__device__ __forceinline__ int head_cursor(const HeadArgs& a) {
+  const int k = a.cursor ? *a.cursor : 0;
+  return min(max(k, 0), a.max_cursor);
+}
+
+__global__ __launch_bounds__(256) void egx_update_head_kernel(HeadArgs a) {
+  const int k = head_cursor(a);
+  const EgxRowsGathered rows{a.perm + (size_t)k * a.n, a.num_src};
+  const int lane = threadIdx.x & 63;
+  int bid = blockIdx.x;
+  if (bid < a.b_pack) {
+    int frag = bid * 4 + (threadIdx.x >> 6);
+    const PackEntry* __restrict__ tab = a.tab;
+    if (frag >= a.frags_tab) return;
+    int lo = 0, hi = a.n_tab - 1;
+    while (lo < hi) {
+      const int mid = (lo + hi) >> 1;
+      if (frag >= tab[mid].frag_end) lo = mid + 1; else hi = mid;
+    }
+    const PackEntry e = tab[lo];
+    const float* __restrict__ src = (lo < (a.n_tab >> 1)) ? a.state : a.ego;
+    frag -= lo > 0 ? tab[lo - 1].frag_end : 0;
+    u3_pack_fragment(e, src, frag, lane, a.nplanes, rows);
+    return;
+  }
+  bid -= a.b_pack;
+  if (bid < a.b_pe) {
+    if (bid == 0 && threadIdx.x < 6) a.log[6 * (size_t)k + threadIdx.x] = 0.f;
+    egx_posenc3_role(a.dist, a.time, a.n, a.pe_out, a.pe_ld, a.pe3, a.S3, a.s0, a.pe3T, a.S3T, a.col0T, bid, rows,
+                     [](const float (&x)[8], bf16x8 (&pl)[3]) { u3_split(x, pl); });
+    return;
+  }
+  bid -= a.b_pe;
+  if (bid < a.b_gather) {
+    const int r = bid * 8 + (threadIdx.x >> 5), c4 = threadIdx.x & 31;
+    if (r >= a.n) return;
+    const size_t srow = rows(r);
+    reinterpret_cast<f32x4*>(a.act_c + (size_t)r * 128)[c4] = reinterpret_cast<const f32x4*>(a.act + srow * 128)[c4];
+    if (c4 == 0) a.adv_c[r] = a.adv[srow];
+    else if (c4 == 1) a.ret_c[r] = a.ret[srow];
+    else if (c4 == 2) a.logp_c[r] = a.logp[srow];
+    return;
+  }
+  if (!a.stats) return;
+  egx_adv_stats_role(a.adv, a.n, a.stats, rows);
 }
 
 inline int img_tiles(int rows) { return 2 * egx_ceil_div(rows, 32); }
@@ -397,6 +471,7 @@
     add(h->h_inputs, nullptr, n, d, 2 * d, d, En.xT, 2 * Sn, Sn, 1, d);
   }
   h->n_inputs = (int)h->h_inputs.size();
+  if ((rc = upload_table(h->h_inputs, &h->tab_inputs, &h->frags_inputs))) return fail(rc);
   std::vector<PackEntry> tl;
   for (int b = 0; b < 2; ++b) {
     Branch& B = h->br[b];
@@ -443,7 +518,7 @@
 
 extern "C" int egx_policy_train_bind(egx_policy_train* h, const float* state, const float* egosensing) {
   EGX_REQUIRE(h && state && egosensing, "null argument");
-  if (h->bound_state == state && h->bound_ego == egosensing && h->tab_inputs) return EGX_OK;
+  if (h->bound_state == state && h->bound_ego == egosensing) return EGX_OK;
   for (int i = 0; i < 4; ++i) h->h_inputs[i].src = state;
   for (int i = 4; i < 8; ++i) h->h_inputs[i].src = egosensing;
   int rc = upload_table(h->h_inputs, &h->tab_inputs, &h->frags_inputs);
@@ -455,7 +530,7 @@
 static int train_step_parts(egx_policy_train* h, const float* dist, const float* time, const float* act, const float* adv,
                             const float* ret, const float* logp_old, const float* adv_stats, const float* scale, float adv_eps,
                             float min_logvar, float max_logvar, float eps_clip, float vf_coef, float ent_coef, float* out_terms,
-                            void* stream_, int parts);
+                            void* stream_, int parts, const egx_update_head* hd = nullptr);
 
 extern "C" int egx_policy_train_step(egx_policy_train* h, const float* dist, const float* time, const float* act, const float* adv,
                                      const float* ret, const float* logp_old, const float* adv_stats, const float* scale,
@@ -472,6 +547,58 @@
   return train_step_parts(h, dist, time, act, adv, ret, logp_old, adv_stats, scale, adv_eps, min_logvar, max_logvar, eps_clip, vf_coef,
                           ent_coef, out_terms, stream_, 1);
 }
+static int head_args_ok(const egx_policy_train* h, const egx_update_head* a) {
+  EGX_REQUIRE(h && a, "null argument");
+  EGX_REQUIRE(a->perm && a->state && a->egosensing && a->dist && a->time && a->act && a->adv && a->ret && a->logp_old &&
+                  a->act_c && a->adv_c && a->ret_c && a->logp_old_c && a->stats && a->log, "null field in egx_update_head");
+  EGX_REQUIRE(h->n_inputs == 8 && h->tab_inputs, "the input table must hold four state entries followed by four egosensing entries");
+  EGX_REQUIRE(a->num_src_rows > 0 && a->max_cursor >= 0, "egx_update_head: num_src_rows must be positive, max_cursor non-negative");
+  return EGX_OK;
+}
+static void launch_head(egx_policy_train* h, const egx_update_head* a, hipStream_t st) {
+  constexpr int S_HD = HD / 32, S_CAT = CAT / 32;
+  const int n = h->n, Sn = h->Sn;
+  HeadArgs k;
+  k.tab = h->tab_inputs; k.n_tab = h->n_inputs; k.frags_tab = h->frags_inputs; k.nplanes = planes_of(h->prec);
+  k.state = a->state; k.ego = a->egosensing;
+  k.perm = reinterpret_cast<const long long*>(a->perm); k.cursor = a->cursor; k.max_cursor = a->max_cursor; k.n = n;
+  k.num_src = a->num_src_rows;
+  k.dist = a->dist; k.time = a->time; k.act = a->act; k.adv = a->adv; k.ret = a->ret; k.logp = a->logp_old;
+  k.act_c = a->act_c; k.adv_c = a->adv_c; k.ret_c = a->ret_c; k.logp_c = a->logp_old_c;
+  k.stats = a->compute_stats ? a->stats : nullptr;
+  k.log = a->log;
+  k.pe_out = h->catf + 2 * HD; k.pe_ld = CAT; k.pe3 = h->cat_r; k.S3 = S_CAT; k.s0 = 2 * S_HD;
+  k.pe3T = h->catT; k.S3T = Sn; k.col0T = 2 * HD;
+  k.b_pack = egx_ceil_div(h->frags_inputs, 4);
+  k.b_pe = egx_ceil_div(2 * Sn * 4 + 8 * Sn, 4);
+  k.b_gather = egx_ceil_div(n, 8);
+  const int blocks = k.b_pack + k.b_pe + k.b_gather + (k.stats ? 1 : 0);
+  hipLaunchKernelGGL(egx_update_head_kernel, dim3(blocks), dim3(256), 0, st, k);
+}
+
+extern "C" int egx_policy_train_head(egx_policy_train* h, const egx_update_head* head, void* stream_) {
+  int rc = head_args_ok(h, head);
+  if (rc) return rc;
+  launch_head(h, head, static_cast<hipStream_t>(stream_));
+  EGX_HIP_CHECK(hipGetLastError());
+  return EGX_OK;
+}
+extern "C" int egx_policy_train_step_cursor(egx_policy_train* h, const egx_update_head* head, const float* scale, float adv_eps,
+                                            float min_logvar, float max_logvar, float eps_clip, float vf_coef, float ent_coef,
+                                            void* stream_) {
+  int rc = head_args_ok(h, head);
+  if (rc) return rc;
+  return train_step_parts(h, head->dist, head->time, head->act_c, head->adv_c, head->ret_c, head->logp_old_c, head->stats, scale, adv_eps,
+                          min_logvar, max_logvar, eps_clip, vf_coef, ent_coef, head->log, stream_, 3, head);
+}
+extern "C" int egx_policy_train_step_heads_cursor(egx_policy_train* h, const egx_update_head* head, const float* scale, float adv_eps,
+                                                  float min_logvar, float max_logvar, float eps_clip, float vf_coef, float ent_coef,
+                                                  void* stream_) {
+  int rc = head_args_ok(h, head);
+  if (rc) return rc;
+  return train_step_parts(h, head->dist, head->time, head->act_c, head->adv_c, head->ret_c, head->logp_old_c, head->stats, scale, adv_eps,
+                          min_logvar, max_logvar, eps_clip, vf_coef, ent_coef, head->log, stream_, 1, head);
+}
 extern "C" int egx_policy_train_step_encoders(egx_policy_train* h, void* stream_) {
   EGX_REQUIRE(h, "null handle");
   return train_step_parts(h, nullptr, nullptr, nullptr, nullptr, nullptr, nullptr, nullptr, nullptr, 0.f, 0.f, 0.f, 0.f, 0.f, 0.f, nullptr,
@@ -481,9 +608,9 @@
 static int train_step_parts(egx_policy_train* h, const float* dist, const float* time, const float* act, const float* adv,
                             const float* ret, const float* logp_old, const float* adv_stats, const float* scale, float adv_eps,
                             float min_logvar, float max_logvar, float eps_clip, float vf_coef, float ent_coef, float* out_terms,
-                            void* stream_, int parts) {
+                            void* stream_, int parts, const egx_update_head* hd) {
   EGX_REQUIRE(h && (!(parts & 1) || (dist && time && act && adv && ret && logp_old && scale && out_terms)), "null argument");
-  EGX_REQUIRE(h->tab_inputs, "egx_policy_train_bind has not been called");
+  EGX_REQUIRE(hd || !(parts & 1) || h->bound_state, "egx_policy_train_bind has not been called");
   hipStream_t st = static_cast<hipStream_t>(stream_);
   const int n = h->n, Sn = h->Sn;
   constexpr int S_HD = HD / 32, S_CAT = CAT / 32, S_G = 3 * HD / 32;
@@ -500,8 +627,12 @@
 
   int rc = EGX_OK;
   if (parts & 1) {
-  run_table(st, h->tab_inputs, h->n_inputs, h->frags_inputs, planes_of(h->prec));
-  egx_launch_posenc3(st, dist, time, n, h->catf + 2 * HD, CAT, h->cat_r, S_CAT, 2 * S_HD, h->catT, Sn, 2 * HD, out_terms);
+  if (hd) {
+    launch_head(h, hd, st);
+  } else {
+    run_table(st, h->tab_inputs, h->n_inputs, h->frags_inputs, planes_of(h->prec));
+    egx_launch_posenc3(st, dist, time, n, h->catf + 2 * HD, CAT, h->cat_r, S_CAT, 2 * S_HD, h->catT, Sn, 2 * HD, out_terms);
+  }
   {
     D3Gru g[2];
     for (int e = 0; e < 2; ++e) {
@@ -558,7 +689,8 @@
     launch_n(st, L, 2);
   }
   rc = egx_ppo_loss_packed_precleared(h->br[0].head, h->br[1].head, act, adv, ret, logp_old, adv_stats, scale, adv_eps, min_logvar, max_logvar,
-                               eps_clip, vf_coef, ent_coef, n, h->br[0].ghead, h->br[1].ghead, out_terms, st);
+                               eps_clip, vf_coef, ent_coef, n, h->br[0].ghead, h->br[1].ghead, out_terms, st, hd ? hd->cursor : nullptr,
+                               hd ? hd->max_cursor : 0);
   if (rc) return rc;
   run_table(st, h->tab_loss, h->n_loss, h->frags_loss, planes_of(h->prec));
   hipStream_t sw = st;
diff --git a/egogen_amd/ppo_policy.py b/egogen_amd/ppo_policy.py
--- a/egogen_amd/ppo_policy.py
+++ b/egogen_amd/ppo_policy.py
@@ -112,6 +112,8 @@
         self._flat_opt_state = None
         self.world_size = dist.get_world_size() if dist.is_available() and dist.is_initialized() else 1
         self._dp = self.world_size > 1 or (os.environ.get("EGX_FORCE_DP_PATH") == "1" and dist.is_available() and dist.is_initialized())
+        self._img_key = None
+        self.refresh_counts = {"total": 0, "learn_top": 0, "learn_bottom": 0}
         self.update_paths: dict = {}
         self.allreduce_events: list = []
         self._allreduce_done: list = []
@@ -293,12 +295,16 @@
         _lib.check(lib.egx_policy_train_set_precision(h, _UPDATE_PREC[self.update_precision]), "egx_policy_train_set_precision")
         dev = self._flat_grad.device
         f = dict(dtype=torch.float32, device=dev)
-        bufs = [torch.empty(n, 804, **f), torch.empty(n, 64, **f), torch.empty(n, 1, **f), torch.empty(n, 1, **f),
+        head = os.environ.get("EGX_UPDATE_HEAD", "1") != "0"
+        bufs = [None if head else torch.empty(n, 804, **f), None if head else torch.empty(n, 64, **f),
+                None if head else torch.empty(n, 1, **f), None if head else torch.empty(n, 1, **f),
                 torch.empty(n, 128, **f), torch.empty(n, 1, **f), torch.empty(n, 1, **f), torch.empty(n, 1, **f)]
-        _lib.check(lib.egx_policy_train_bind(h, _lib.ptr(bufs[0]), _lib.ptr(bufs[1])), "egx_policy_train_bind")
+        if not head:
+            _lib.check(lib.egx_policy_train_bind(h, _lib.ptr(bufs[0]), _lib.ptr(bufs[1])), "egx_policy_train_bind")
         packed = _lib.PolicyPacked3()
         _lib.check(lib.egx_policy_train_packed(h, C.byref(packed)), "egx_policy_train_packed")
-        hs = {"h": h, "bufs": bufs, "stats": torch.zeros(2, **f), "key": (w.x_enc_w_ih, g.x_enc_w_ih), "packed": packed}
+        hs = {"h": h, "n": int(n), "bufs": bufs, "stats": torch.zeros(2, **f), "key": (w.x_enc_w_ih, g.x_enc_w_ih), "packed": packed,
+              "head": head}
         self._train_handles[n] = hs
         if len(self._train_handles) == 1:
             self._runner.adopt_packed(packed, refresh=self._refresh_images)
@@ -331,14 +337,27 @@
         except Exception:
             pass
 
+    def _prec_key(self):
+        return (int(_lib.load().egx_policy_get_precision()), self.update_precision)
+
+    def _img_key_now(self):
+        return (sum(int(p._version) for p in self.parameters()), self._prec_key())
+
     def _refresh_images(self):
         if not self._train_handles:
             return
         lib, st = _lib.load(), _lib.current_stream_ptr()
         for hs in self._train_handles.values():
             _lib.check(lib.egx_policy_train_refresh(hs["h"], st), "egx_policy_train_refresh")
-
-    def _fwd_bwd_train_step(self, hs, batch, idx, gstats, log_out, part: str = "all"):
+        self._img_key = self._img_key_now()
+        self.refresh_counts["total"] += 1
+
+    def _refresh_images_if_stale(self, who: str):
+        if self._train_handles and self._img_key != self._img_key_now():
+            self._refresh_images()
+            self.refresh_counts[who] += 1
+
+    def _fwd_bwd_train_step(self, hs, batch, idx, gstats, log_out, part: str = "all", cursor=None):
         from .fused_ops import gather_rows
         lib, st = _lib.load(), _lib.current_stream_ptr()
         if part == "encoders":
@@ -347,6 +366,35 @@
         N = batch.n * batch.A
         obs_all = batch.obs_flat()
         b = hs["bufs"]
+        if hs["head"]:
+            n = hs["n"]
+            idx = idx.contiguous()
+            rows = int(idx.numel()) // n
+            assert idx.dtype == torch.long and rows >= 1 and (cursor is not None or int(idx.numel()) == n), (idx.dtype, idx.shape, n)
+            assert log_out.is_contiguous() and log_out.dtype == torch.float32 and log_out.numel() >= 6 * rows, log_out.shape
+            srcs = (obs_all["state"], obs_all["egosensing"], obs_all["dist"], obs_all["time"], batch.act, batch.adv, batch.returns,
+                    batch.logp_old)
+            assert all(t.dtype == torch.float32 and t.is_contiguous() for t in srcs)
+            dev = b[4].device
+            if gstats is None:
+                scale = self._scale_cache.get((n, dev))
+                if scale is None:
+                    scale = torch.full((1,), 1.0 / n, dtype=torch.float32, device=dev)
+                    self._scale_cache[(n, dev)] = scale
+            else:
+                hs["stats"].copy_(torch.stack([gstats[0], gstats[1]]).float())
+                scale = (1.0 / gstats[2]).reshape(1).float()
+            hd = _lib.UpdateHead()
+            hd.perm, hd.cursor = idx.data_ptr(), (cursor.data_ptr() if cursor is not None else None)
+            hd.max_cursor, hd.num_src_rows = rows - 1, N
+            (hd.state, hd.egosensing, hd.dist, hd.time, hd.act, hd.adv, hd.ret, hd.logp_old) = (t.data_ptr() for t in srcs)
+            hd.act_c, hd.adv_c, hd.ret_c, hd.logp_old_c = (b[i].data_ptr() for i in (4, 5, 6, 7))
+            hd.stats, hd.compute_stats, hd.log = hs["stats"].data_ptr(), int(gstats is None), log_out.data_ptr()
+            fn = lib.egx_policy_train_step_heads_cursor if part == "heads" else lib.egx_policy_train_step_cursor
+            rc = fn(hs["h"], C.byref(hd), _lib.ptr(scale), float(_EPS), float(self.actor.min_logvar), float(self.actor.max_logvar),
+                    float(self._eps_clip), float(self._weight_vf), float(self._weight_ent), st)
+            _lib.check(rc, "egx_policy_train_step_cursor")
+            return
         gather_rows(idx, [obs_all["state"].reshape(N, 804), obs_all["egosensing"].reshape(N, 64), obs_all["dist"].reshape(N, 1),
                           obs_all["time"].reshape(N, 1), batch.act.reshape(N, 128), batch.adv.reshape(N, 1), batch.returns.reshape(N, 1),
                           batch.logp_old.reshape(N, 1)], out=b)
@@ -368,10 +416,12 @@
                 _lib.ptr(log_out), st)
         _lib.check(rc, "egx_policy_train_step")
 
-    def _fwd_bwd(self, batch, idx, gstats, log_out) -> str:
-        hs = self._train_handle(int(idx.shape[0])) if idx.is_cuda else None
+    def _fwd_bwd(self, batch, idx, gstats, log_out, cursor=None, n=None) -> str:
+        hs = self._train_handle(int(idx.shape[0]) if n is None else int(n)) if idx.is_cuda else None
+        if cursor is not None and (hs is None or not hs["head"]):
+            raise _lib.EgxError("a minibatch cursor needs the update chain with its head launch")
         if hs is not None:
-            self._fwd_bwd_train_step(hs, batch, idx, gstats, log_out)
+            self._fwd_bwd_train_step(hs, batch, idx, gstats, log_out, cursor=cursor)
             return "chain"
         obs, act, adv, ret, lpo = self._gather(batch, idx)
         v_s = batch.values[:batch.n].reshape(-1).index_select(0, idx) if self._value_clip else None
@@ -389,19 +439,24 @@
             log_out.copy_(torch.stack([terms[k].detach() for k in ("loss", "loss/clip", "loss/vf", "loss/ent", "loss/kld", "approx_kl")]))
         return "autograd"
 
-    def _clip_and_step(self):
+    def _clip_and_step(self, cursor=None):
         if self.use_flat_optimizer and self._flat_opt_state == "ready":
             g = self.optim.param_groups[0]
             lib = _lib.load()
             b1, b2 = g["betas"]
-            rc = lib.egx_adamw_clip_step(_lib.ptr(self._flat_p), _lib.ptr(self._flat_grad), _lib.ptr(self._flat_m), _lib.ptr(self._flat_v),
-                                         self._flat_p.numel(), self._n_clip, float(self._grad_norm or 0.0), float(g["lr"]), float(b1),
-                                         float(b2), float(g["eps"]), float(g["weight_decay"]), _lib.ptr(self._step_t),
-                                         _lib.ptr(self._adamw_ws), _lib.current_stream_ptr())
+            args = (_lib.ptr(self._flat_p), _lib.ptr(self._flat_grad), _lib.ptr(self._flat_m), _lib.ptr(self._flat_v),
+                    self._flat_p.numel(), self._n_clip, float(self._grad_norm or 0.0), float(g["lr"]), float(b1),
+                    float(b2), float(g["eps"]), float(g["weight_decay"]), _lib.ptr(self._step_t), _lib.ptr(self._adamw_ws))
+            if cursor is None:
+                rc = lib.egx_adamw_clip_step(*args, _lib.current_stream_ptr())
+            else:
+                rc = lib.egx_adamw_clip_step_cursor(*args, _lib.ptr(cursor), _lib.current_stream_ptr())
             _lib.check(rc, "egx_adamw_clip_step")
             self._runner.mark_dirty()
             self._refresh_images()
             return
+        if cursor is not None:
+            raise _lib.EgxError("a minibatch cursor needs the flat optimiser")
         if self._grad_norm:
             nn.utils.clip_grad_norm_(self._actor_critic.parameters(), max_norm=self._grad_norm)
         self.optim.step()
@@ -514,8 +569,18 @@
         if g is not None:
             return g
         dev = batch.act.device
-        st = {"idx": torch.zeros(local_bs, dtype=torch.long, device=dev), "log": torch.zeros(6, device=dev),
-              "gstats": torch.tensor([0.0, 1.0, float(local_bs * self.world_size)], device=dev), "use_gstats": self._dp}
+        st = {"gstats": torch.tensor([0.0, 1.0, float(local_bs * self.world_size)], device=dev), "use_gstats": self._dp}
+        hs0 = self._train_handle(local_bs) if dev.type == "cuda" else None
+        st["head"] = hs0 is not None and hs0["head"] and self.use_flat_optimizer and self._flat_opt_state == "ready"
+        if st["head"]:
+            rows = max(1, (batch.n * batch.A) // local_bs)
+            st.update(rows=rows, perm=torch.zeros(rows * local_bs, dtype=torch.long, device=dev), log=torch.zeros(rows, 6, device=dev),
+                      cursor=torch.zeros((), dtype=torch.int32, device=dev))
+            fb_args, fb_kw = (st["perm"], ), dict(cursor=st["cursor"], n=local_bs)
+        else:
+            st.update(idx=torch.zeros(local_bs, dtype=torch.long, device=dev), log=torch.zeros(6, device=dev))
+            fb_args, fb_kw = (st["idx"], ), {}
+        cur = st.get("cursor")
         gs = (lambda: (st["gstats"][0], st["gstats"][1], st["gstats"][2])) if st["use_gstats"] else (lambda: None)
         try:
             snap = {k: v.clone() for k, v in self.state_dict().items()}
@@ -525,31 +590,31 @@
             side.wait_stream(torch.cuda.current_stream())
             with torch.cuda.stream(side):
                 for _ in range(3):
-                    self._fwd_bwd(batch, st["idx"], gs(), st["log"])
-                    self._clip_and_step()
+                    self._fwd_bwd(batch, *fb_args, gs(), st["log"], **fb_kw)
+                    self._clip_and_step(cur)
             torch.cuda.current_stream().wait_stream(side)
             torch.cuda.synchronize()
             g1 = torch.cuda.CUDAGraph()
             g2 = None
             if not self._dp:
                 with torch.cuda.graph(g1):
-                    st["path"] = self._fwd_bwd(batch, st["idx"], gs(), st["log"])
-                    self._clip_and_step()
-            else:
-                hs = self._train_handle(local_bs) if st["idx"].is_cuda else None
+                    st["path"] = self._fwd_bwd(batch, *fb_args, gs(), st["log"], **fb_kw)
+                    self._clip_and_step(cur)
+            else:
+                hs = self._train_handle(local_bs) if dev.type == "cuda" else None
                 if hs is not None and len(self._grad_buckets()) == 2 and self.overlap_allreduce:
                     with torch.cuda.graph(g1):
-                        self._fwd_bwd_train_step(hs, batch, st["idx"], gs(), st["log"], part="heads")
+                        self._fwd_bwd_train_step(hs, batch, *fb_args, gs(), st["log"], part="heads", cursor=cur)
                     g1b = torch.cuda.CUDAGraph()
                     with torch.cuda.graph(g1b, pool=g1.pool()):
-                        self._fwd_bwd_train_step(hs, batch, st["idx"], gs(), st["log"], part="encoders")
+                        self._fwd_bwd_train_step(hs, batch, *fb_args, gs(), st["log"], part="encoders")
                     st["g1b"], st["path"] = g1b, "chain"
                 else:
                     with torch.cuda.graph(g1):
-                        st["path"] = self._fwd_bwd(batch, st["idx"], gs(), st["log"])
+                        st["path"] = self._fwd_bwd(batch, *fb_args, gs(), st["log"], **fb_kw)
                 g2 = torch.cuda.CUDAGraph()
                 with torch.cuda.graph(g2, pool=g1.pool()):
-                    self._clip_and_step()
+                    self._clip_and_step(cur)
             self.load_state_dict(snap)
             for p_ in params:
                 for k, v in self.optim.state.get(p_, {}).items():
@@ -557,6 +622,9 @@
                         old_v = osnap[id(p_)].get(k)
                         v.copy_(old_v) if old_v is not None else v.zero_()
             st["g1"], st["g2"] = g1, g2
+            st["prec_key"] = self._prec_key()
+            if cur is not None:
+                cur.zero_()
             self._refresh_images()
         except Exception as e:
             import warnings
@@ -610,7 +678,7 @@
         self._ensure_flat_grads()
         if self.use_flat_optimizer and batch.act.is_cuda:
             self._flat_optimizer_ready()
-        self._refresh_images()
+        self._refresh_images_if_stale("learn_top")
         ws = self.world_size
         dp = self._dp
         N = batch.n * batch.A
@@ -640,11 +708,21 @@
             last_log = None
             spans = [(s, bounds[i + 1] if i + 1 < len(bounds) else N) for i, s in enumerate(bounds)]
             gstats_all = self._global_adv_stats(batch, perm, spans) if dp else None
+            gst = self._graphs_for(batch, local_bs) if (use_graph and spans[0][1] - spans[0][0] == local_bs) else None
+            if gst is not None and gst.get("g1") is None:
+                gst = None
+            vsum = self._img_key_now()[0]
+            head = gst is not None and gst["head"]
+            n_replayed, first_log = 0, len(logs)
+            if head:
+                gst["perm"].copy_(perm[:gst["perm"].numel()])
+                gst["cursor"].zero_()
             for i, (s, e) in enumerate(spans):
                 idx = perm[s:e]
-                st = self._graphs_for(batch, local_bs) if (use_graph and e - s == local_bs) else None
-                if st is not None and st.get("g1") is not None:
-                    st["idx"].copy_(idx)
+                st = gst if e - s == local_bs else None
+                if st is not None:
+                    if not head:
+                        st["idx"].copy_(idx)
                     if dp:
                         st["gstats"].copy_(gstats_all[i])
                     st["g1"].replay()
@@ -663,7 +741,12 @@
                         else:
                             self._all_reduce_grad()
                         st["g2"].replay()
-                    last_log = st["log"].clone()
+                    self._img_key = (vsum, st["prec_key"])
+                    if head:
+                        last_log = None
+                        n_replayed += 1
+                    else:
+                        last_log = st["log"].clone()
                     self.update_paths[st["path"] + "+graph"] = self.update_paths.get(st["path"] + "+graph", 0) + 1
                 else:
                     gstats = None
@@ -676,10 +759,14 @@
                     self._clip_and_step()
                     last_log = log
                     self.update_paths[path] = self.update_paths.get(path, 0) + 1
-                logs.append(last_log[:5])
+                logs.append(last_log)
                 if self._after_minibatch is not None:
                     self._after_minibatch(len(logs) - 1)
                 kld_rows.append(idx)
+            if n_replayed:
+                snap = gst["log"][:n_replayed].clone()
+                logs[first_log:first_log + n_replayed] = list(snap)
+            last_log = logs[-1] if logs else None
             if repeat > 1 and last_log is not None:
                 kl = last_log[5].clone()
                 if dp:
@@ -687,9 +774,9 @@
                 if float(kl.item()) >= 0.02:
                     break
         self._runner.mark_dirty()
-        self._refresh_images()
+        self._refresh_images_if_stale("learn_bottom")
         if logs:
-            L = torch.stack(logs)
+            L = torch.stack(logs)[:, :5].contiguous()
             mu2 = batch.mu.reshape(N, -1).pow(2).mean(1)
             if len({int(r.shape[0]) for r in kld_rows}) == 1:
                 kld = 0.5 * mu2.index_select(0, torch.cat(kld_rows)).reshape(len(kld_rows), -1).mean(1)
diff --git a/include/egogen_hip.h b/include/egogen_hip.h
--- a/include/egogen_hip.h
+++ b/include/egogen_hip.h
@@ -237,6 +237,24 @@
                                 float min_logvar, float max_logvar, float eps_clip, float vf_coef, float ent_coef, float* out_terms,
                                 void* stream);
 int egx_policy_train_step_encoders(egx_policy_train* h, void* stream);
+typedef struct egx_update_head {
+  const int64_t* perm;
+  const int32_t* cursor;
+  int max_cursor;
+  int num_src_rows;
+  const float *state, *egosensing, *dist, *time;
+  const float *act, *adv, *ret, *logp_old;
+  float *act_c, *adv_c, *ret_c, *logp_old_c;
+  float* stats;
+  int compute_stats;
+  float* log;
+} egx_update_head;
+int egx_policy_train_head(egx_policy_train* h, const egx_update_head* head, void* stream);
+int egx_policy_train_step_cursor(egx_policy_train* h, const egx_update_head* head, const float* scale, float adv_eps,
+                                 float min_logvar, float max_logvar, float eps_clip, float vf_coef, float ent_coef, void* stream);
+int egx_policy_train_step_heads_cursor(egx_policy_train* h, const egx_update_head* head, const float* scale, float adv_eps,
+                                       float min_logvar, float max_logvar, float eps_clip, float vf_coef, float ent_coef,
+                                       void* stream);
 int egx_policy_train_set_precision(egx_policy_train* h, int prec);
 
 int egx_policy_set_precision(int bf16);
@@ -396,6 +414,9 @@
 int egx_adamw_clip_step(float* param, const float* grad, float* exp_avg, float* exp_avg_sq, size_t n, size_t n_clip,
                         float max_norm, double lr, double beta1, double beta2, double eps, double weight_decay, float* step,
                         float* workspace, void* stream);
+int egx_adamw_clip_step_cursor(float* param, const float* grad, float* exp_avg, float* exp_avg_sq, size_t n, size_t n_clip,
+                               float max_norm, double lr, double beta1, double beta2, double eps, double weight_decay, float* step,
+                               float* workspace, int32_t* cursor, void* stream);
 
 #ifdef __cplusplus
 }
```

Result: faster. 193,100 (median of 6 runs) (+1.3%).
